# KrishnaswamyLab/MELD

Hardware: AMD Instinct MI355X
Metric: cells/sec through MELD.fit_transform (kNN+Chebyshev) (higher is better)
Workload: dtype f64

## Files before the change

### include/meld_hip.h

```cpp
#ifndef MELD_HIP_H
#define MELD_HIP_H

#include <stddef.h>
#include <stdint.h>

#ifdef __cplusplus
extern "C" {
#endif

#define MELD_OK 0
#define MELD_ERR_INVALID (-1)
#define MELD_ERR_UNSUPPORTED (-2)
#define MELD_ERR_HIP (-3)

typedef void* meld_stream_t;

int meld_abi_version(void);
const char* meld_last_error(void);
int meld_device_count(void);


int meld_knn_padded_dim(int d);
int meld_knn_tile_refs(void);
int meld_knn_block_queries(void);
int meld_knn_row_capacity(int ksel);
double meld_knn_error_coef(int d);

int meld_col_sums_f64(const double* X, int64_t N, int d, double* sums, meld_stream_t stream);
size_t meld_col_stats_temp_bytes(int d);
int meld_col_stats_f64(const double* X, int64_t N, int d, double* sums, double* mins, double* maxs, void* temp, size_t temp_bytes,
                       meld_stream_t stream);

int meld_knn_prepare_refs(const double* X, int64_t N, int d, const double* mean, int KP, float* Rt,
                          float* norm2, float* norm2_max, meld_stream_t stream);
int meld_knn_prepare_queries(const double* X, int64_t N, int d, const double* mean, int KP,
                             int64_t q_begin, int64_t q_count, float* Q, meld_stream_t stream);

int meld_knn_topk(const float* Q, const float* Rt, int64_t n_ref, int KP, int64_t q_count, int ksel,
                  int32_t* cand_idx, float* cand_d2, int32_t* cand_cnt, meld_stream_t stream);

int meld_knn16_kblocks(int d);
int meld_knn16_tile_refs(void);
int meld_knn16_split_dims(int d);
int meld_frame_max_dims(void);
int meld_cov_sample_f64(const double* X, int64_t N, int d, const double* mean, int64_t stride, double* cov, meld_stream_t stream);
int meld_rotate_rows_f64(const double* X, int64_t N, int d, const double* mean, const double* At, double* out, meld_stream_t stream);
int meld_knn16_block_queries(void);
int meld_knn16_row_capacity(int ksel);
double meld_knn16_error_coef(int nprod, int d);
double meld_knn16_error_coef_const(int nprod, int d);
double meld_knn16_error_coef_lin(int nprod);
size_t meld_knn16_tile_bytes(int d);
size_t meld_knn16_query_bytes(int d);
int meld_knn16_prepare(const double* X, int64_t N, int d, const double* mean, int64_t q_begin,
                       int64_t q_count, void* Rt16, void* Q16, float* Qn, float* norm2, float* norm2_max,
                       float* scale_info, meld_stream_t stream);
int meld_knn16_prepare_scaled(const double* X, int64_t N, int d, const double* mean, const double* col_min, const double* col_max,
                              int64_t q_begin, int64_t q_count, void* Rt16, void* Q16, float* Qn, float* norm2, float* norm2_max,
                              float* scale_info, meld_stream_t stream);
size_t meld_knn16_bounds_bytes(int64_t n_ref, int64_t q_count);
size_t meld_knn16_bounds_temp_bytes(int64_t n_ref, int d, int64_t q_count);
int meld_knn16_bounds(const double* X, int64_t N, int d, const double* mean, const float* scale_info,
                      const float* norm2_max, const void* Rt16, int64_t q_begin, int64_t q_count,
                      const float* thr_seed, const float* q_norm2 ,
                      int nprod, void* temp, void* lb2, meld_stream_t stream);
int meld_knn16_tile_spheres(const double* X, int64_t N, int d, const double* mean, const float* scale_info, void* temp,
                            int64_t tile_begin, int64_t tile_count, meld_stream_t stream);
int meld_knn16_sphere_layout(int64_t n_ref, int d, int64_t* rows, int64_t* row_bytes);
int meld_knn16_bounds_from_spheres(const double* X, int64_t N, int d, const double* mean, const float* scale_info,
                      const float* norm2_max, const void* Rt16, int64_t q_begin, int64_t q_count,
                      const float* thr_seed, const float* q_norm2 ,
                      int nprod, void* temp, void* lb2, meld_stream_t stream);
int meld_knn16_prepare_cross(const double* X, int64_t n_refs, int64_t n_total, int d, const double* mean, int64_t q_begin,
                             int64_t q_count, void* Rt16, void* Q16, float* Qn, float* norm2, float* norm2_max,
                             float* scale_info, meld_stream_t stream);
int meld_knn16_prepare_rows(const double* X, int64_t N, int d, const double* mean, const float* scale_info,
                            int64_t q_begin, const int32_t* rows, int64_t n_rows, void* Q16, float* Qn,
                            meld_stream_t stream);
int meld_knn16_research_thresholds(const int32_t* rows, int64_t n_rows, int64_t q_begin, const int32_t* cand_cnt,
                                   const float* cand_d2, int cap, int ksel, const float* norm2, const float* norm2_max,
                                   double err_coef, double err_lin, double err3, const float* scale_info, float* thr,
                                   meld_stream_t stream);
int meld_knn16_seed_thresholds_mfma(const void* Q16, const float* Qn, const void* Rt16, const float* scale_info,
                                    const float* norm2_max, int64_t n_ref, int d, int64_t q_begin, int64_t q_count,
                                    int knn, double radius_factor, int nprod, int side_tiles, float* thr_init,
                                    meld_stream_t stream);
int meld_knn16_topk(const void* Q16, const float* Qn, const void* Rt16, const float* scale_info,
                    int64_t n_ref, int d, int64_t q_count, int ksel, int nprod, int n_slices, const void* lb2,
                    const float* norm2_max, int64_t q_begin, const float* thr_init, int knn, double radius_factor,
                    int32_t* cand_idx, float* cand_d2, int32_t* cand_cnt, float* cand_thr,
                    uint64_t* tiles_done ,
                    const int32_t* block_order ,
                    meld_stream_t stream);
int meld_knn16_block_work(const void* lb2, const float* thr_seed, int64_t n_ref, int d, int64_t q_count, int nprod,
                          const float* norm2_max, const float* scale_info, int32_t* work, meld_stream_t stream);
int meld_knn16_step_lists(const void* lb2, const float* thr_seed, int64_t n_ref, int d, int64_t q_count, int nprod,
                          const float* norm2_max, const float* scale_info, int64_t q_begin, uint32_t* list,
                          int64_t list_stride, int32_t* cnt, meld_stream_t stream);
size_t meld_knn16_list_scratch_bytes(int64_t n_ref);
int meld_knn16_step_lists_direct(const double* X, int64_t N, int d, const double* mean, const float* scale_info, const float* norm2_max,
                                 const void* Rt16, const float* thr_seed, const float* q_norm2, int nprod, void* temp, void* scratch,
                                 uint32_t* list, int64_t list_stride, int32_t* cnt, meld_stream_t stream);
int meld_knn16_step_lists_direct_lead(const double* X, int64_t N, int d, const double* mean, const float* scale_info, const float* norm2_max,
                                 const void* Rt16, const float* thr_seed, const float* q_norm2, int nprod, void* temp, void* scratch,
                                 uint32_t* list, int64_t list_stride, int32_t* cnt, int lead_only, meld_stream_t stream);
int meld_knn16_topk_listed(const void* Q16, const float* Qn, const void* Rt16, const float* scale_info, int64_t n_ref, int d,
                           int64_t q_count, int ksel, const uint32_t* step_list, const int32_t* step_cnt, int64_t list_stride,
                           const float* norm2_max, int64_t q_begin, const float* thr_init, int knn, double radius_factor,
                           int32_t* cand_idx, float* cand_d2, int32_t* cand_cnt, float* cand_thr, uint64_t* tiles_done,
                           const int32_t* block_order, int n_slices , meld_stream_t stream);
int meld_knn16_topk_listed_partial(const void* Q16, const float* Qn, const void* Rt16, const float* scale_info, int64_t n_ref,
                                   int d, int64_t q_count, int ksel, const uint32_t* step_list, const int32_t* step_cnt,
                                   int64_t list_stride, const float* norm2_max, int64_t q_begin, const float* thr_init, int knn,
                                   double radius_factor, int32_t* cand_idx, float* cand_d2, int32_t* cand_cnt, float* cand_thr,
                                   uint64_t* tiles_done, const int32_t* block_order, int n_slices, int partial_test,
                                   meld_stream_t stream);
int meld_knn16_partial_filter(const void* Q16, const float* Qn, const void* Rt16, const float* scale_info, const float* norm2_max, int d,
                              int64_t q_count, const float* thr_init, uint32_t* step_list, const int32_t* step_cnt, int64_t list_stride,
                              int32_t* cnt_out, uint64_t* tested, const int32_t* block_order , meld_stream_t stream);
int meld_knn16_resident_blocks(int d, int nprod);
int meld_knn16_max_slices(int ksel);
int meld_knn16_merge_slices(const int32_t* s_idx, const float* s_d2, const int32_t* s_cnt, int64_t q_count,
                            int ksel, int n_slices, int32_t* out_idx, float* out_d2, int32_t* out_cnt,
                            meld_stream_t stream);


int meld_knn_refine(const double* X, int64_t N, int d, int64_t q_begin, int64_t q_count,
                    const int32_t* cand_idx, const float* cand_d2, const int32_t* cand_cnt,
                    const float* cand_thr ,
                    int ksel, int cap , int knn, double decay, double thresh,
                    const float* norm2_max, double err_coef,
                    const float* norm2 , double err_coef_lin, double* bw,
                    double* cand_val, int32_t* keep_cnt, int32_t* flag_rows, int32_t* n_flag,
                    const int32_t* rows, int out_cap, int32_t* cand_idx_out,
                    double bw_scale ,
                    const double* bw_fixed ,
                    int max_rank ,
                    meld_stream_t stream);

int meld_knn_radius_exact(const double* X, int64_t N, int d, int64_t q_begin, const int32_t* flag_rows,
                          int32_t n_flag, const double* bw, int knn, double decay, double thresh,
                          int mode, int32_t* fb_cnt, const int64_t* fb_off, int32_t* fb_cursor,
                          int32_t* fb_col, double* fb_val, int32_t* err_flag,
                          double bw_scale ,
                          meld_stream_t stream);
int meld_knn_pair_distances(const double* X, int d, const int64_t* rows, const int64_t* cand, int64_t n, int kk, double* out,
                            meld_stream_t stream);

#define MELD_METRIC_L1 1
#define MELD_METRIC_LINF 2
int meld_metric_tile_rows(void);
int meld_metric_tile_boxes(const double* X, int64_t N, int d, double* box_lo, double* box_hi, meld_stream_t stream);
int meld_metric_topk(const double* X, int64_t N, int d, int metric, int ksel, const double* box_lo, const double* box_hi, int prune,
                     double* heap_d, int32_t* heap_i, int32_t* cand_idx, double* cand_d, int32_t* cand_cnt,
                     unsigned long long* tiles_done, meld_stream_t stream);
int meld_metric_refine(const int32_t* cand_idx, const double* cand_d, const int32_t* cand_cnt, int64_t N, int ksel, int knn,
                       double decay, double thresh, double* bw, double* cand_val, int32_t* keep_cnt, int32_t* flag_rows,
                       int32_t* n_flag, meld_stream_t stream);
int meld_metric_radius(const double* X, int64_t N, int d, int metric, const int32_t* flag_rows, int32_t n_flag, const double* bw,
                       double decay, double thresh, int mode, int32_t* fb_cnt, const int64_t* fb_off, int32_t* fb_cursor,
                       int32_t* fb_col, double* fb_val, meld_stream_t stream);


size_t meld_scan_temp_bytes(int64_t n);
int meld_exclusive_scan_i32_i64(const int32_t* in, int64_t* out, int64_t n, void* temp, size_t temp_bytes,
                                meld_stream_t stream);

int meld_coo_emit(int64_t q_begin, int64_t q_count, const int32_t* cand_idx, const double* cand_val,
                  const int32_t* cand_cnt, int ksel, int cap, const int64_t* keep_off, const int32_t* flag_rows,
                  int32_t n_flag, const int64_t* fb_off, const int32_t* fb_col, const double* fb_val,
                  int64_t fb_base, int64_t M, uint64_t* keys, double* vals, meld_stream_t stream);

size_t meld_sort_temp_bytes(int64_t n);
int meld_sort_pairs_u64_f64(const uint64_t* keys_in, uint64_t* keys_out, const double* vals_in,
                            double* vals_out, int64_t n, int end_bit, void* temp, size_t temp_bytes,
                            meld_stream_t stream);

size_t meld_merge_temp_bytes(int64_t n);
int meld_coo_merge(const uint64_t* keys_sorted, const double* vals_sorted, int64_t n, uint64_t* ukeys,
                   double* uvals, int64_t* n_unique, void* temp, size_t temp_bytes, meld_stream_t stream);

int meld_csr_from_keys(const uint64_t* ukeys, int64_t nnz, int64_t row_begin, int64_t n_rows,
                       int64_t* rowptr, int32_t* col, meld_stream_t stream);

int meld_coo_partition_remote(const uint64_t* keys, const double* vals, int64_t n, int64_t rows_per_rank, int world,
                              int self_rank, int64_t cap, int32_t* counts, int64_t* send, meld_stream_t stream);
int meld_coo_emit_scatter(int64_t q_count, const int32_t* cand_idx, const double* cand_val, int ksel, int cap,
                          const int32_t* keep_cnt, const int32_t* flag_rows, int32_t n_flag, const int64_t* fb_off,
                          const int32_t* fb_col, const double* fb_val, int64_t fb_total, int32_t* cursor, int32_t* tcol,
                          double* tval, meld_stream_t stream);
int meld_csr_bucket_slots(void);
int meld_coo_scatter_rows(const uint64_t* keys, const double* vals, int64_t n, int64_t row_begin, int64_t n_rows,
                          int32_t* cursor, int32_t* tcol, double* tval, meld_stream_t stream);
int meld_csr_rows_sort_merge(const int32_t* cursor, int64_t n_rows, int32_t* tcol, double* tval, int32_t* ucnt,
                             int32_t* flags,
                             int symm ,
                             double theta , meld_stream_t stream);
int meld_csr_compact_rows(const int64_t* rowptr, int64_t n_rows, const int32_t* tcol, const double* tval,
                          int32_t* col, double* val, meld_stream_t stream);
int meld_csr_compact_rows_sums(const int64_t* rowptr, int64_t n_rows, const int32_t* tcol, const double* tval, int32_t* col,
                               double* val, double diag, double* sums, meld_stream_t stream);

int meld_csr_row_sums(const int64_t* rowptr, const double* val, int64_t n_rows, double diag,
                      double* out, meld_stream_t stream);
int meld_csr_anisotropy(const int64_t* rowptr, const int32_t* col, double* val, int64_t n_rows,
                        const double* ksum_all, int64_t ksum_row_offset, double anisotropy,
                        meld_stream_t stream);
int meld_csr_anisotropy_degrees(const int64_t* rowptr, const int32_t* col, double* val, int64_t n_rows,
                                const double* ksum_all, int64_t ksum_row_offset, double anisotropy, double* dw,
                                meld_stream_t stream);


int meld_spmm_dot_slots(void);
int meld_cheby_step(const int64_t* rowptr, const int32_t* col, const double* val, const double* dw,
                    int64_t n_rows, int64_t nnz_hint, int p, const double* x_full, int64_t x_row_offset,
                    const double* z, double* y, double* r, double alpha, double beta, double gamma,
                    double coef, double* dots, meld_stream_t stream);

int meld_cheby_step_wide(const int64_t* rowptr, const int32_t* col, const double* val, const double* dw, int64_t n_rows, int p,
                         const double* x_full, int64_t x_row_offset, const double* z, double* y, double alpha, double beta,
                         double gamma, meld_stream_t stream);

int meld_lanczos_steps(const int64_t* rowptr, const int32_t* col, const double* val, const double* dw,
                       int64_t n_rows, int64_t nnz_hint, double* v0, double* v1, double* v2, double* state,
                       double* alphas, double* betas, int it_begin, int n_iter, double* scratch,
                       meld_stream_t stream);
int meld_lanczos_spmv(const int64_t* rowptr, const int32_t* col, const double* val, const double* dw, int64_t n_rows,
                      int64_t nnz_hint, const double* x_full, int64_t x_row_offset, const double* z_local,
                      double* y_local, const double* state, double* dots, meld_stream_t stream);
int meld_lanczos_alpha(double* state, const double* dots, double* nrm2, double* alphas, int it, meld_stream_t stream);
int meld_lanczos_axpy(const double* x_local, double* y_local, int64_t n_rows, const double* state, double* nrm2,
                      meld_stream_t stream);
int meld_lanczos_beta(double* state, const double* nrm2, double* dots, double* betas, int it, meld_stream_t stream);
int meld_lanczos_fold(double* state, double* acc, double* alphas, double* betas, int it, meld_stream_t stream);
int meld_lanczos_axpy3(double* y_local, const double* u_local, const double* u_prev_local, int64_t n_rows,
                       const double* state, double* nrm2, meld_stream_t stream);
int meld_scale_f64(const double* x, double a, double* r, int64_t n, meld_stream_t stream);
int meld_axpby_f64(double a, const double* x, double b, double* y, int64_t n, double* nrm2,
                   meld_stream_t stream);

typedef struct meld_pt_layout {
  const int32_t* blk_row;
  const int32_t* blk_ntile;
  const int32_t* blk_ndist;
  const int32_t* seg;
  const int32_t* list_cols;
  const double* pval;
  const uint32_t* pidx;
  int32_t nb;
  const float* pval32;
  int64_t stream_len;
  const uint16_t* cdesc;
} meld_pt_layout_t;
int meld_pt_geometry(int* consumer_waves, int* rows_max, int* tile_cols, int* tiles_max);
int meld_pt_num_blocks(int64_t n_rows);
int64_t meld_pt_seg_len(int nb);
int64_t meld_pt_stream_len(int64_t nnz, int nb);
int64_t meld_pt_desc_len(int nb);
int meld_pt_debug_ablate(int mask);
int meld_pt_debug_stamps(unsigned long long* buf);
int meld_pt_build(const int64_t* rowptr, const int32_t* col, const double* val, int64_t n_rows, int64_t n_cols,
                  int64_t col_base, int symmetric, const meld_pt_layout_t* layout,
                  uint32_t* codes , int32_t* status, meld_stream_t stream);
int meld_pt_cheby_step(const meld_pt_layout_t* layout, const int64_t* rowptr, const double* dw, int64_t n_rows, int p,
                       const double* x_full, int64_t x_row_offset, const double* z, double* y, double* r,
                       double alpha, double beta, double gamma, double coef, double* dots, meld_stream_t stream);
int meld_pt_cheby_run(const meld_pt_layout_t* layout, const int64_t* rowptr, const double* dw, int64_t n_rows, int p,
                      double* t_prev2, double* t_prev1, double* r, const double* coeffs, int n_coef, double alpha2, double beta2,
                      int* last, meld_stream_t stream);
int meld_pt_lanczos_steps(const meld_pt_layout_t* layout, const int64_t* rowptr, const double* dw, int64_t n_rows,
                          double* v0, double* v1, double* v2, double* state, double* alphas, double* betas,
                          int it_begin, int n_iter, double* scratch, const int32_t* stop, meld_stream_t stream);
int meld_pt_lanczos_spmv(const meld_pt_layout_t* layout, const int64_t* rowptr, const double* dw, int64_t n_rows,
                         const double* x_full, int64_t x_row_offset, const double* z_local, double* y_local,
                         const double* state, double* dots, meld_stream_t stream);

int meld_rccl_available(void);
int meld_rccl_unique_id(void* id_host);
int meld_rccl_comm_create(const void* id_host, int world, int rank, void** comm);
int meld_rccl_comm_destroy(void* comm);
// ... 56 lines not shown
```

### meld_amd/_lib.py

```python
from __future__ import annotations

from ._options import is_set, opt

import ctypes as C
import os

_HERE = os.path.dirname(os.path.abspath(__file__))
LIB_NAME = "libmeld_hip.so"
LIB_PATH = os.path.join(_HERE, LIB_NAME)

_i32, _i64, _f64, _sz, _ptr = C.c_int, C.c_int64, C.c_double, C.c_size_t, C.c_void_p

SIGNATURES = {
    "meld_abi_version": (_i32, []),
    "meld_last_error": (C.c_char_p, []),
    "meld_device_count": (_i32, []),
    "meld_knn_padded_dim": (_i32, [_i32]),
    "meld_knn_tile_refs": (_i32, []),
    "meld_knn_block_queries": (_i32, []),
    "meld_knn_row_capacity": (_i32, [_i32]),
    "meld_col_sums_f64": (_i32, [_ptr, _i64, _i32, _ptr, _ptr]),
    "meld_col_stats_temp_bytes": (_sz, [_i32]),
    "meld_col_stats_f64": (_i32, [_ptr, _i64, _i32, _ptr, _ptr, _ptr, _ptr, _sz, _ptr]),
    "meld_knn_prepare_refs": (_i32, [_ptr, _i64, _i32, _ptr, _i32, _ptr, _ptr, _ptr, _ptr]),
    "meld_knn_prepare_queries": (_i32, [_ptr, _i64, _i32, _ptr, _i32, _i64, _i64, _ptr, _ptr]),
    "meld_knn_topk": (_i32, [_ptr, _ptr, _i64, _i32, _i64, _i32, _ptr, _ptr, _ptr, _ptr]),
    "meld_knn_refine": (
        _i32,
        [_ptr, _i64, _i32, _i64, _i64, _ptr, _ptr, _ptr, _ptr, _i32, _i32, _i32, _f64, _f64, _ptr, _f64, _ptr, _f64, _ptr, _ptr, _ptr,
         _ptr, _ptr, _ptr, _i32, _ptr, _f64, _ptr, _i32, _ptr],
    ),
    "meld_knn_error_coef": (_f64, [_i32]),
    "meld_knn16_kblocks": (_i32, [_i32]),
    "meld_knn16_tile_refs": (_i32, []),
    "meld_knn16_split_dims": (_i32, [_i32]),
    "meld_knn16_block_queries": (_i32, []),
    "meld_knn16_row_capacity": (_i32, [_i32]),
    "meld_knn16_error_coef": (_f64, [_i32, _i32]),
    "meld_knn16_error_coef_const": (_f64, [_i32, _i32]),
    "meld_knn16_error_coef_lin": (_f64, [_i32]),
    "meld_knn16_resident_blocks": (_i32, [_i32, _i32]),
    "meld_knn16_tile_bytes": (_sz, [_i32]),
    "meld_knn16_query_bytes": (_sz, [_i32]),
    "meld_knn16_prepare": (_i32, [_ptr, _i64, _i32, _ptr, _i64, _i64, _ptr, _ptr, _ptr, _ptr, _ptr, _ptr, _ptr]),
    "meld_knn16_prepare_scaled": (_i32, [_ptr, _i64, _i32, _ptr, _ptr, _ptr, _i64, _i64, _ptr, _ptr, _ptr, _ptr, _ptr, _ptr, _ptr]),
    "meld_knn16_prepare_cross": (_i32, [_ptr, _i64, _i64, _i32, _ptr, _i64, _i64, _ptr, _ptr, _ptr, _ptr, _ptr, _ptr, _ptr]),
    "meld_knn16_prepare_rows": (_i32, [_ptr, _i64, _i32, _ptr, _ptr, _i64, _ptr, _i64, _ptr, _ptr, _ptr]),
    "meld_knn16_research_thresholds": (_i32, [_ptr, _i64, _i64, _ptr, _ptr, _i32, _i32, _ptr, _ptr, _f64, _f64, _f64, _ptr, _ptr, _ptr]),
    "meld_knn16_bounds_bytes": (_sz, [_i64, _i64]),
    "meld_knn16_bounds_temp_bytes": (_sz, [_i64, _i32, _i64]),
    "meld_knn16_bounds": (_i32, [_ptr, _i64, _i32, _ptr, _ptr, _ptr, _ptr, _i64, _i64, _ptr, _ptr, _i32, _ptr, _ptr, _ptr]),
    "meld_knn16_bounds_from_spheres": (_i32, [_ptr, _i64, _i32, _ptr, _ptr, _ptr, _ptr, _i64, _i64, _ptr, _ptr, _i32, _ptr, _ptr, _ptr]),
    "meld_knn16_tile_spheres": (_i32, [_ptr, _i64, _i32, _ptr, _ptr, _ptr, _i64, _i64, _ptr]),
    "meld_knn16_sphere_layout": (_i32, [_i64, _i32, _ptr, _ptr]),
    "meld_knn16_topk": (_i32, [_ptr, _ptr, _ptr, _ptr, _i64, _i32, _i64, _i32, _i32, _i32, _ptr, _ptr, _i64, _ptr, _i32, _f64, _ptr, _ptr, _ptr, _ptr, _ptr, _ptr, _ptr]),
    "meld_knn16_block_work": (_i32, [_ptr, _ptr, _i64, _i32, _i64, _i32, _ptr, _ptr, _ptr, _ptr]),
    "meld_knn16_step_lists": (_i32, [_ptr, _ptr, _i64, _i32, _i64, _i32, _ptr, _ptr, _i64, _ptr, _i64, _ptr, _ptr]),
    "meld_knn16_list_scratch_bytes": (_sz, [_i64]),
    "meld_knn16_step_lists_direct": (_i32, [_ptr, _i64, _i32, _ptr, _ptr, _ptr, _ptr, _ptr, _ptr, _i32, _ptr, _ptr, _ptr, _i64, _ptr, _ptr]),
    "meld_knn16_step_lists_direct_lead": (_i32, [_ptr, _i64, _i32, _ptr, _ptr, _ptr, _ptr, _ptr, _ptr, _i32, _ptr, _ptr, _ptr, _i64, _ptr, _i32, _ptr]),
    "meld_knn16_topk_listed": (_i32, [_ptr, _ptr, _ptr, _ptr, _i64, _i32, _i64, _i32, _ptr, _ptr, _i64, _ptr, _i64, _ptr, _i32, _f64, _ptr, _ptr, _ptr, _ptr, _ptr, _ptr, _i32, _ptr]),
    "meld_knn16_topk_listed_partial": (_i32, [_ptr, _ptr, _ptr, _ptr, _i64, _i32, _i64, _i32, _ptr, _ptr, _i64, _ptr, _i64, _ptr, _i32, _f64, _ptr, _ptr, _ptr, _ptr, _ptr, _ptr, _i32, _i32, _ptr]),
    "meld_knn16_partial_filter": (_i32, [_ptr, _ptr, _ptr, _ptr, _ptr, _i32, _i64, _ptr, _ptr, _ptr, _i64, _ptr, _ptr, _ptr, _ptr]),
    "meld_knn16_seed_thresholds_mfma": (_i32, [_ptr, _ptr, _ptr, _ptr, _ptr, _i64, _i32, _i64, _i64, _i32, _f64, _i32, _i32, _ptr, _ptr]),
    "meld_knn16_max_slices": (_i32, [_i32]),
    "meld_knn16_merge_slices": (_i32, [_ptr, _ptr, _ptr, _i64, _i32, _i32, _ptr, _ptr, _ptr, _ptr]),
    "meld_knn_radius_exact": (
        _i32,
        [_ptr, _i64, _i32, _i64, _ptr, _i32, _ptr, _i32, _f64, _f64, _i32, _ptr, _ptr, _ptr, _ptr, _ptr, _ptr, _f64, _ptr],
    ),
    "meld_knn_pair_distances": (_i32, [_ptr, _i32, _ptr, _ptr, _i64, _i32, _ptr, _ptr]),
    "meld_metric_tile_rows": (_i32, []),
    "meld_metric_tile_boxes": (_i32, [_ptr, _i64, _i32, _ptr, _ptr, _ptr]),
    "meld_metric_topk": (_i32, [_ptr, _i64, _i32, _i32, _i32, _ptr, _ptr, _i32, _ptr, _ptr, _ptr, _ptr, _ptr, _ptr, _ptr]),
    "meld_metric_refine": (_i32, [_ptr, _ptr, _ptr, _i64, _i32, _i32, _f64, _f64, _ptr, _ptr, _ptr, _ptr, _ptr, _ptr]),
    "meld_metric_radius": (_i32, [_ptr, _i64, _i32, _i32, _ptr, _i32, _ptr, _f64, _f64, _i32, _ptr, _ptr, _ptr, _ptr, _ptr, _ptr]),
    "meld_scan_temp_bytes": (_sz, [_i64]),
    "meld_exclusive_scan_i32_i64": (_i32, [_ptr, _ptr, _i64, _ptr, _sz, _ptr]),
    "meld_coo_emit": (
        _i32,
        [_i64, _i64, _ptr, _ptr, _ptr, _i32, _i32, _ptr, _ptr, _i32, _ptr, _ptr, _ptr, _i64, _i64, _ptr, _ptr, _ptr],
    ),
    "meld_sort_temp_bytes": (_sz, [_i64]),
    "meld_sort_pairs_u64_f64": (_i32, [_ptr, _ptr, _ptr, _ptr, _i64, _i32, _ptr, _sz, _ptr]),
    "meld_merge_temp_bytes": (_sz, [_i64]),
    "meld_coo_merge": (_i32, [_ptr, _ptr, _i64, _ptr, _ptr, _ptr, _ptr, _sz, _ptr]),
    "meld_csr_from_keys": (_i32, [_ptr, _i64, _i64, _i64, _ptr, _ptr, _ptr]),
    "meld_csr_seg_length": (_i32, []),
    "meld_csr_spmm_f64": (_i32, [_ptr, _ptr, _ptr, _i32, _i64, _ptr, _ptr, _i64, _ptr, _ptr, _i64, _ptr, _ptr, _i64, _i32, _ptr, _i64, _ptr]),
    "meld_csr_transpose_keys": (_i32, [_ptr, _ptr, _ptr, _i32, _i64, _ptr, _ptr, _ptr]),
    "meld_csr_rows_to_dense_f64": (_i32, [_ptr, _ptr, _ptr, _i32, _i64, _i64, _i64, _ptr, _i64, _ptr]),
    "meld_csr_bucket_slots": (_i32, []),
    "meld_coo_scatter_rows": (_i32, [_ptr, _ptr, _i64, _i64, _i64, _ptr, _ptr, _ptr, _ptr]),
    "meld_coo_emit_scatter": (_i32, [_i64, _ptr, _ptr, _i32, _i32, _ptr, _ptr, _i32, _ptr, _ptr, _ptr, _i64, _ptr, _ptr, _ptr, _ptr]),
    "meld_coo_partition_remote": (_i32, [_ptr, _ptr, _i64, _i64, _i32, _i32, _i64, _ptr, _ptr, _ptr]),
    "meld_csr_rows_sort_merge": (_i32, [_ptr, _i64, _ptr, _ptr, _ptr, _ptr, _i32, _f64, _ptr]),
    "meld_csr_compact_rows": (_i32, [_ptr, _i64, _ptr, _ptr, _ptr, _ptr, _ptr]),
    "meld_csr_compact_rows_sums": (_i32, [_ptr, _i64, _ptr, _ptr, _ptr, _ptr, _f64, _ptr, _ptr]),
    "meld_csr_row_sums": (_i32, [_ptr, _ptr, _i64, _f64, _ptr, _ptr]),
    "meld_csr_anisotropy": (_i32, [_ptr, _ptr, _ptr, _i64, _ptr, _i64, _f64, _ptr]),
    "meld_csr_anisotropy_degrees": (_i32, [_ptr, _ptr, _ptr, _i64, _ptr, _i64, _f64, _ptr, _ptr]),
    "meld_spmm_dot_slots": (_i32, []),
    "meld_cheby_step": (
        _i32,
        [_ptr, _ptr, _ptr, _ptr, _i64, _i64, _i32, _ptr, _i64, _ptr, _ptr, _ptr, _f64, _f64, _f64, _f64, _ptr, _ptr],
    ),
    "meld_lanczos_steps": (_i32, [_ptr, _ptr, _ptr, _ptr, _i64, _i64, _ptr, _ptr, _ptr, _ptr, _ptr, _ptr, _i32, _i32, _ptr, _ptr]),
    "meld_lanczos_spmv": (_i32, [_ptr, _ptr, _ptr, _ptr, _i64, _i64, _ptr, _i64, _ptr, _ptr, _ptr, _ptr, _ptr]),
    "meld_lanczos_alpha": (_i32, [_ptr, _ptr, _ptr, _ptr, _i32, _ptr]),
    "meld_lanczos_axpy": (_i32, [_ptr, _ptr, _i64, _ptr, _ptr, _ptr]),
    "meld_lanczos_beta": (_i32, [_ptr, _ptr, _ptr, _ptr, _i32, _ptr]),
    "meld_lanczos_fold": (_i32, [_ptr, _ptr, _ptr, _ptr, _i32, _ptr]),
    "meld_lanczos_axpy3": (_i32, [_ptr, _ptr, _ptr, _i64, _ptr, _ptr, _ptr]),
    "meld_pt_geometry": (_i32, [_ptr, _ptr, _ptr, _ptr]),
    "meld_pt_num_blocks": (_i32, [_i64]),
    "meld_pt_seg_len": (_i64, [_i32]),
    "meld_pt_debug_ablate": (_i32, [_i32]),
    "meld_pt_debug_stamps": (_i32, [_ptr]),
    "meld_pt_stream_len": (_i64, [_i64, _i32]),
    "meld_pt_desc_len": (_i64, [_i32]),
    "meld_pt_build": (_i32, [_ptr, _ptr, _ptr, _i64, _i64, _i64, _i32, _ptr, _ptr, _ptr, _ptr]),
    "meld_cheby_step_wide": (_i32, [_ptr, _ptr, _ptr, _ptr, _i64, _i32, _ptr, _i64, _ptr, _ptr, _f64, _f64, _f64, _ptr]),
    "meld_pt_cheby_step": (_i32, [_ptr, _ptr, _ptr, _i64, _i32, _ptr, _i64, _ptr, _ptr, _ptr, _f64, _f64, _f64, _f64, _ptr, _ptr]),
    "meld_pt_cheby_run": (_i32, [_ptr, _ptr, _ptr, _i64, _i32, _ptr, _ptr, _ptr, _ptr, _i32, _f64, _f64, _ptr, _ptr]),
    "meld_pt_lanczos_steps": (_i32, [_ptr, _ptr, _ptr, _i64, _ptr, _ptr, _ptr, _ptr, _ptr, _ptr, _i32, _i32, _ptr, _ptr, _ptr]),
    "meld_pt_lanczos_spmv": (_i32, [_ptr, _ptr, _ptr, _i64, _ptr, _i64, _ptr, _ptr, _ptr, _ptr, _ptr]),
    "meld_kmeans_max_blocks": (_i32, []),
    "meld_kmeans_assign": (_i32, [_ptr, _i64, _i32, _ptr, _i32, _ptr, _ptr, _ptr, _ptr, _i32, _ptr]),
    "meld_scale_f64": (_i32, [_ptr, _f64, _ptr, _i64, _ptr]),
    "meld_axpby_f64": (_i32, [_f64, _ptr, _f64, _ptr, _i64, _ptr, _ptr]),
    "meld_normalize_rows_l1": (_i32, [_ptr, _ptr, _i64, _i32, _ptr]),
    "meld_assign_nearest": (_i32, [_ptr, _i64, _i32, _ptr, _i32, _ptr, _ptr, _ptr, _ptr]),
    "meld_chain_order": (_i32, [_ptr, _i64, _i32, _i32, _ptr, _ptr]),
    "meld_gather_rows_f64": (_i32, [_ptr, _ptr, _i64, _i32, _ptr, _ptr]),
    "meld_frame_max_dims": (_i32, []),
    "meld_cov_sample_f64": (_i32, [_ptr, _i64, _i32, _ptr, _i64, _ptr, _ptr]),
    "meld_rotate_rows_f64": (_i32, [_ptr, _i64, _i32, _ptr, _ptr, _ptr, _ptr]),
    "meld_argsort_u32_temp_bytes": (_sz, [_i64]),
    "meld_argsort_u32": (_i32, [_ptr, _i64, _i32, _ptr, _ptr, _ptr, _sz, _ptr]),
    "meld_order_starts": (_i32, [_ptr, _i64, _i32, _ptr, _ptr]),
    "meld_order_pick_centroids": (_i32, [_ptr, _i64, _i32, _ptr, _ptr, _i32, _i32, _ptr, _ptr]),
    "meld_order_update_keys": (_i32, [_ptr, _ptr, _ptr, _i64, _i32, _ptr]),
    "meld_rccl_available": (_i32, []),
    "meld_rccl_unique_id": (_i32, [_ptr]),
    "meld_rccl_comm_create": (_i32, [_ptr, _i32, _i32, _ptr]),
    "meld_rccl_comm_destroy": (_i32, [_ptr]),
    "meld_rccl_all_gather": (_i32, [_ptr, _ptr, _ptr, _sz, _ptr]),
    "meld_rccl_all_reduce_sum_f64": (_i32, [_ptr, _ptr, _sz, _ptr]),
    "meld_cheby_run_sharded": (_i32, [_ptr, _ptr, _ptr, _ptr, _ptr, _ptr, _i64, _i64, _i64, _i64, _i32, _ptr, _ptr, _ptr, _ptr, _i32, _f64, _f64, _ptr, _ptr]),
    "meld_lanczos_steps_sharded": (_i32, [_ptr, _ptr, _ptr, _ptr, _ptr, _ptr, _i64, _i64, _i64, _i64, _ptr, _ptr, _ptr, _ptr, _ptr, _ptr, _ptr, _i32, _i32, _ptr]),
    "meld_factorize_max_groups": (_i32, []),
    "meld_factorize_max_words": (_i32, []),
    "meld_factorize_temp_bytes": (_sz, [_i64]),
    "meld_factorize_labels": (_i32, [_ptr, _i64, _i32, _ptr, _sz, _ptr, _ptr]),
    "meld_factorize_codes": (_i32, [_ptr, _i64, _ptr, _ptr, _ptr]),
    "meld_indicator_signal": (_i32, [_ptr, _ptr, _ptr, _i64, _i64, _i32, _ptr, _ptr]),
    "meld_scatter_rows_f64": (_i32, [_ptr, _ptr, _i64, _i32, _ptr, _ptr]),
}



class PtLayout(C.Structure):

    _fields_ = [("blk_row", _ptr), ("blk_ntile", _ptr), ("blk_ndist", _ptr), ("seg", _ptr), ("list_cols", _ptr),
                ("pval", _ptr), ("pidx", _ptr), ("nb", C.c_int32), ("pval32", _ptr), ("stream_len", C.c_int64), ("cdesc", _ptr)]


_lib = None


class MeldHipError(RuntimeError):
    """A libmeld_hip.so entry point returned a non-zero status."""


def get_lib():
    global _lib
    if _lib is not None:
        return _lib
    path = opt("MELD_HIP_LIB") or LIB_PATH
    if not os.path.exists(path):
# ... 23 lines not shown
```

### meld_amd/csrc/assemble.hip

```cpp
#include "common.hpp"

#include <rocprim/rocprim.hpp>

namespace meld {

__global__ __launch_bounds__(256) void coo_emit_rows_kernel(int64_t q_begin, int64_t q_count,
                                                            const int* __restrict__ cand_idx,
                                                            const double* __restrict__ cand_val, int ksel, int cap,
                                                            const int64_t* __restrict__ keep_off, int64_t M,
                                                            unsigned long long* __restrict__ keys,
                                                            double* __restrict__ vals) {
  const int lane = threadIdx.x & 63;
  const int64_t q = (int64_t)blockIdx.x * 4 + (threadIdx.x >> 6);
  if (q >= q_count) return;
  const int64_t base = keep_off[q];
  if (keep_off[q + 1] == base) return;
  const unsigned long long gi = (unsigned long long)(q_begin + q);
  int written = 0;
  for (int c0 = 0; c0 < ksel; c0 += 64) {
    const int c = c0 + lane;
    double v = 0.0;
    int j = 0;
    if (c < ksel) {
      v = cand_val[(size_t)q * ksel + c];
// ... 328 lines not shown
    int j = 0;
    if (c < ksel) {
      v = cand_val[(size_t)q * ksel + c];
      j = cand_idx[(size_t)q * cap + c];
    }
    const bool keep = v > 0.0;
    const unsigned long long b = __ballot(keep);
    if (keep) {
      const int pos = written + __popcll(b & ((1ull << lane) - 1ull));
      const double hv = 0.5 * v;
      tcol[q * CSR_BUCKET + pos] = j;
      tval[q * CSR_BUCKET + pos] = hv;
      const int slot = atomicAdd(cursor + j, 1);
      if (slot < CSR_BUCKET) {
        tcol[(int64_t)j * CSR_BUCKET + slot] = (int)q;
        tval[(int64_t)j * CSR_BUCKET + slot] = hv;
      }
    }
    written += __popcll(b);
  }
}
__global__ __launch_bounds__(256) void coo_emit_scatter_fallback_kernel(const int* __restrict__ flag_rows, int n_flag,
                                                                        const int64_t* __restrict__ fb_off,
                                                                        const int* __restrict__ fb_col,
                                                                        const double* __restrict__ fb_val, int64_t fb_total,
                                                                        int* __restrict__ cursor, int* __restrict__ tcol,
                                                                        double* __restrict__ tval) {
  const int64_t e = (int64_t)blockIdx.x * blockDim.x + threadIdx.x;
  if (e >= fb_total) return;
  int lo = 0, hi = n_flag - 1;
  while (lo < hi) {
    const int mid = (lo + hi + 1) >> 1;
    if (fb_off[mid] <= e) lo = mid; else hi = mid - 1;
  }
  const int64_t q = flag_rows[lo];
  const int64_t pos = e - fb_off[lo];
  const int j = fb_col[e];
  const double hv = 0.5 * fb_val[e];
  if (pos < CSR_BUCKET) {
    tcol[q * CSR_BUCKET + pos] = j;
    tval[q * CSR_BUCKET + pos] = hv;
  }
  const int slot = atomicAdd(cursor + j, 1);
  if (slot < CSR_BUCKET) {
    tcol[(int64_t)j * CSR_BUCKET + slot] = (int)q;
    tval[(int64_t)j * CSR_BUCKET + slot] = hv;
  }
}

template <int SL, typename K>
__device__ __forceinline__ void csr_bitonic_sort(K (&key)[SL], int lane) {
  constexpr int NE = 64 * SL;
#pragma unroll
  for (int k = 2; k <= NE; k <<= 1) {
#pragma unroll
    for (int j = k >> 1; j > 0; j >>= 1) {
      if (j >= 64) {
        const int je = j >> 6;
#pragma unroll
        for (int e = 0; e < SL; ++e) {
          if ((e & je) == 0) {
            const bool asc = ((64 * e + lane) & k) == 0;
            const K a = key[e], b = key[e | je];
            const bool sw = asc ? (b < a) : (a < b);
            key[e] = sw ? b : a;
            key[e | je] = sw ? a : b;
          }
        }
      } else {
#pragma unroll
        for (int e = 0; e < SL; ++e) {
          const int i = 64 * e + lane;
          const K o = __shfl_xor(key[e], j, 64);
          const bool keep_min = ((i & j) == 0) == ((i & k) == 0);
          key[e] = keep_min ? (o < key[e] ? o : key[e]) : (o < key[e] ? key[e] : o);
        }
      }
    }
  }
}

template <int SL>
__device__ __forceinline__ int csr_row_merge(int* __restrict__ tcol, double* __restrict__ tval, int64_t base, int n, int lane,
                                             bool* bad, int symm, double theta) {
  static_assert(CSR_BUCKET <= 256, "the slot shares a 32-bit key with a 24-bit column");
  unsigned cin[SL];
  bool wide = false;
#pragma unroll
  for (int e = 0; e < SL; ++e) {
    const int i = lane + 64 * e;
    cin[e] = i < n ? (unsigned)tcol[base + i] : 0u;
    wide |= cin[e] >= 0xFFFFFFu;
  }
  double v[SL];
  unsigned c[SL];
  if (!__any(wide)) {
    unsigned key[SL];
#pragma unroll
    for (int e = 0; e < SL; ++e) {
      const int i = lane + 64 * e;
      key[e] = i < n ? ((cin[e] << 8) | (unsigned)i) : ~0u;
    }
    csr_bitonic_sort<SL>(key, lane);
#pragma unroll
    for (int e = 0; e < SL; ++e) {
      const int i = lane + 64 * e;
      c[e] = i < n ? (key[e] >> 8) : 0xffffffffu;
      v[e] = i < n ? tval[base + (key[e] & 255u)] : 0.0;
    }
  } else {
    unsigned long long key[SL];
#pragma unroll
    for (int e = 0; e < SL; ++e) {
      const int i = lane + 64 * e;
      key[e] = i < n ? (((unsigned long long)cin[e] << 32) | (unsigned)i) : ~0ull;
    }
    csr_bitonic_sort<SL>(key, lane);
#pragma unroll
    for (int e = 0; e < SL; ++e) {
      const int i = lane + 64 * e;
      c[e] = (unsigned)(key[e] >> 32);
      v[e] = i < n ? tval[base + (unsigned)key[e]] : 0.0;
    }
  }
  int total = 0;
  bool any_bad = false;
  unsigned head_col[SL];
  double head_val[SL];
  int head_pos[SL];
  bool is_head[SL];
#pragma unroll
  for (int e = 0; e < SL; ++e) {
    const int i = lane + 64 * e;
    unsigned prev = __shfl_up(c[e], 1, 64);
    if (lane == 0) prev = 0xffffffffu;
    if (e > 0) {
      const unsigned pl = __shfl(c[e - 1], 63, 64);
      if (lane == 0) prev = pl;
    }
    unsigned n1 = __shfl_down(c[e], 1, 64), n2 = __shfl_down(c[e], 2, 64);
    double v1 = __shfl_down(v[e], 1, 64);
    if (e + 1 < SL) {
      const unsigned f0 = __shfl(c[e + 1], 0, 64), f1 = __shfl(c[e + 1], 1, 64);
      const double w0 = __shfl(v[e + 1], 0, 64);
      if (lane == 63) { n1 = f0; n2 = f1; v1 = w0; }
      if (lane == 62) n2 = f0;
    } else {
      if (lane == 63) { n1 = 0xffffffffu; n2 = 0xffffffffu; }
      if (lane == 62) n2 = 0xffffffffu;
    }
    const bool valid = i < n;
    const bool head = valid && (i == 0 || prev != c[e]);
    const bool pair = valid && (i + 1 < n) && n1 == c[e];
    const bool triple = valid && (i + 2 < n) && n2 == c[e];
    any_bad |= triple;
    double hv = pair ? v[e] + v1 : v[e];
    bool keep_head = head;
    if (symm == 1) {
      hv = pair ? 4.0 * v[e] * v1 : 0.0;
      keep_head = head && pair;
    } else if (symm == 2) {
      hv = pair ? 2.0 * (theta * fmin(v[e], v1) + (1.0 - theta) * fmax(v[e], v1)) : 2.0 * (1.0 - theta) * v[e];
      keep_head = head && hv != 0.0;
    }
    is_head[e] = keep_head;
    head_col[e] = c[e];
    head_val[e] = hv;
    const unsigned long long hb = __ballot(keep_head);
    head_pos[e] = total + __popcll(hb & ((1ull << lane) - 1ull));
    total += __popcll(hb);
  }
#pragma unroll
  for (int e = 0; e < SL; ++e) {
    if (is_head[e]) {
      tcol[base + head_pos[e]] = (int)head_col[e];
      tval[base + head_pos[e]] = head_val[e];
    }
  }
  if (__any(any_bad)) *bad = true;
  return total;
}

__global__ __launch_bounds__(256) void csr_rows_sort_merge_kernel(const int* __restrict__ cursor, int64_t n_rows,
                                                                  int* __restrict__ tcol, double* __restrict__ tval,
                                                                  int* __restrict__ ucnt, int* __restrict__ flags, int symm, double theta) {
  const int lane = threadIdx.x & 63;
  const int64_t r = (int64_t)blockIdx.x * 4 + (threadIdx.x >> 6);
  if (r >= n_rows) return;
  const int64_t base = r * CSR_BUCKET;
  const int n = cursor[r];
  if (n > CSR_BUCKET) {
    if (lane == 0) {
      atomicOr(flags, 1);
      ucnt[r] = 0;
    }
    return;
  }
  bool bad = false;
  int total;
  if (n <= 64)
    total = csr_row_merge<1>(tcol, tval, base, n, lane, &bad, symm, theta);
  else if (n <= 128)
    total = csr_row_merge<2>(tcol, tval, base, n, lane, &bad, symm, theta);
  else
    total = csr_row_merge<4>(tcol, tval, base, n, lane, &bad, symm, theta);
  if (lane == 0) {
    ucnt[r] = total;
    if (bad) atomicOr(flags, 2);
  }
}

__global__ __launch_bounds__(256) void csr_compact_rows_kernel(const int64_t* __restrict__ rowptr, int64_t n_rows,
                                                               const int* __restrict__ tcol, const double* __restrict__ tval,
                                                               int* __restrict__ col, double* __restrict__ val) {
  const int64_t r = ((int64_t)blockIdx.x * blockDim.x + threadIdx.x) >> 4;
  const int g = threadIdx.x & 15;
  if (r >= n_rows) return;
  const int64_t src = r * CSR_BUCKET, dst = rowptr[r];
  const int len = (int)(rowptr[r + 1] - dst);
  for (int k = g; k < len; k += 16) {
    col[dst + k] = tcol[src + k];
    val[dst + k] = tval[src + k];
  }
}

__global__ __launch_bounds__(256) void csr_compact_rows_sums_kernel(const int64_t* __restrict__ rowptr, int64_t n_rows,
                                                                    const int* __restrict__ tcol, const double* __restrict__ tval,
                                                                    int* __restrict__ col, double* __restrict__ val, double diag,
                                                                    double* __restrict__ sums) {
  const int64_t r = ((int64_t)blockIdx.x * blockDim.x + threadIdx.x) >> 3;
  const int g = threadIdx.x & 7;
  double s = 0.0;
  if (r < n_rows) {
    const int64_t src = r * CSR_BUCKET, dst = rowptr[r];
    const int len = (int)(rowptr[r + 1] - dst);
    for (int k = g; k < len; k += 8) {
      const double v = tval[src + k];
      col[dst + k] = tcol[src + k];
      val[dst + k] = v;
      s += v;
    }
  }
  s += __shfl_xor(s, 1, 64);
  s += __shfl_xor(s, 2, 64);
  s += __shfl_xor(s, 4, 64);
  if (r < n_rows && g == 0) sums[r] = diag + s;
}

extern "C" int meld_csr_bucket_slots(void) { return CSR_BUCKET; }

extern "C" int meld_coo_scatter_rows(const uint64_t* keys, const double* vals, int64_t n, int64_t row_begin, int64_t n_rows,
                                     int32_t* cursor, int32_t* tcol, double* tval, meld_stream_t stream) {
  MELD_CHECK_ARG(cursor && n_rows > 0 && n >= 0 && (n == 0 || (keys && vals && tcol && tval)),
                 "meld_coo_scatter_rows: bad arguments");
  MELD_HIP_CALL(hipMemsetAsync(cursor, 0, sizeof(int32_t) * (size_t)n_rows, S(stream)));
  if (n == 0) return MELD_OK;
  hipLaunchKernelGGL(coo_scatter_rows_kernel, dim3((unsigned)ceil_div(n, 256)), dim3(256), 0, S(stream),
                     reinterpret_cast<const unsigned long long*>(keys), vals, n, row_begin, n_rows, cursor, tcol, tval);
  MELD_LAUNCH_CHECK("coo_scatter_rows_kernel");
  return MELD_OK;
}

extern "C" int meld_coo_partition_remote(const uint64_t* keys, const double* vals, int64_t n, int64_t rows_per_rank, int world,
                                         int self_rank, int64_t cap, int32_t* counts, int64_t* send, meld_stream_t stream) {
  MELD_CHECK_ARG(counts && send && n >= 0 && (n == 0 || (keys && vals)) && rows_per_rank > 0 && world >= 1 && self_rank >= 0 &&
                     self_rank < world && cap >= 0,
                 "meld_coo_partition_remote: bad arguments");
  MELD_HIP_CALL(hipMemsetAsync(counts, 0, sizeof(int32_t) * (size_t)world, S(stream)));
  if (cap > 0) MELD_HIP_CALL(hipMemsetAsync(send, 0xFF, sizeof(int64_t) * 2 * (size_t)world * (size_t)cap, S(stream)));
  if (n == 0) return MELD_OK;
  MELD_CHECK_ARG(world <= PR_WORLD_MAX, "meld_coo_partition_remote: %d ranks (at most %d)", world, PR_WORLD_MAX);
  hipLaunchKernelGGL(coo_partition_remote_kernel, dim3((unsigned)ceil_div(n, 256 * PR_PER)), dim3(256), 0, S(stream),
                     reinterpret_cast<const unsigned long long*>(keys), vals, n, rows_per_rank, world, self_rank, cap, counts,
                     reinterpret_cast<long long*>(send));
  MELD_LAUNCH_CHECK("coo_partition_remote_kernel");
  return MELD_OK;
}

extern "C" int meld_coo_emit_scatter(int64_t q_count, const int32_t* cand_idx, const double* cand_val, int ksel, int cap,
                                     const int32_t* keep_cnt, const int32_t* flag_rows, int32_t n_flag, const int64_t* fb_off,
                                     const int32_t* fb_col, const double* fb_val, int64_t fb_total, int32_t* cursor, int32_t* tcol,
                                     double* tval, meld_stream_t stream) {
  MELD_CHECK_ARG(cand_idx && cand_val && keep_cnt && cursor && tcol && tval && q_count > 0, "meld_coo_emit_scatter: bad arguments");
  MELD_CHECK_ARG(cap >= ksel && ksel <= CSR_BUCKET, "meld_coo_emit_scatter: ksel=%d must fit a row bucket (%d) and the row stride cap=%d",
                 ksel, CSR_BUCKET, cap);
  hipLaunchKernelGGL(coo_emit_scatter_rows_kernel, dim3((unsigned)ceil_div(q_count, 4)), dim3(256), 0, S(stream), q_count, cand_idx,
                     cand_val, ksel, cap, keep_cnt, cursor, tcol, tval);
  MELD_LAUNCH_CHECK("coo_emit_scatter_rows_kernel");
  if (n_flag > 0 && fb_total > 0) {
    MELD_CHECK_ARG(flag_rows && fb_off && fb_col && fb_val, "meld_coo_emit_scatter: missing fallback arrays");
    hipLaunchKernelGGL(coo_emit_scatter_fallback_kernel, dim3((unsigned)ceil_div(fb_total, 256)), dim3(256), 0, S(stream), flag_rows,
                       n_flag, fb_off, fb_col, fb_val, fb_total, cursor, tcol, tval);
    MELD_LAUNCH_CHECK("coo_emit_scatter_fallback_kernel");
  }
  return MELD_OK;
}

extern "C" int meld_csr_rows_sort_merge(const int32_t* cursor, int64_t n_rows, int32_t* tcol, double* tval, int32_t* ucnt,
                                        int32_t* flags, int symm, double theta, meld_stream_t stream) {
  MELD_CHECK_ARG(cursor && tcol && tval && ucnt && flags && n_rows > 0, "meld_csr_rows_sort_merge: bad arguments");
  MELD_CHECK_ARG(symm >= 0 && symm <= 2 && (symm != 2 || (theta >= 0.0 && theta <= 1.0)),
                 "meld_csr_rows_sort_merge: symm must be 0 (+), 1 (*) or 2 (mnn, theta in [0, 1])");
  MELD_HIP_CALL(hipMemsetAsync(flags, 0, sizeof(int32_t), S(stream)));
  hipLaunchKernelGGL(csr_rows_sort_merge_kernel, dim3((unsigned)ceil_div(n_rows, 4)), dim3(256), 0, S(stream), cursor, n_rows,
                     tcol, tval, ucnt, flags, symm, theta);
  MELD_LAUNCH_CHECK("csr_rows_sort_merge_kernel");
  return MELD_OK;
}

extern "C" int meld_csr_compact_rows(const int64_t* rowptr, int64_t n_rows, const int32_t* tcol, const double* tval,
                                     int32_t* col, double* val, meld_stream_t stream) {
  MELD_CHECK_ARG(rowptr && n_rows > 0 && tcol && tval && col && val, "meld_csr_compact_rows: bad arguments");
  hipLaunchKernelGGL(csr_compact_rows_kernel, dim3((unsigned)ceil_div(n_rows * 16, 256)), dim3(256), 0, S(stream), rowptr,
                     n_rows, tcol, tval, col, val);
  MELD_LAUNCH_CHECK("csr_compact_rows_kernel");
  return MELD_OK;
}

extern "C" int meld_csr_compact_rows_sums(const int64_t* rowptr, int64_t n_rows, const int32_t* tcol, const double* tval, int32_t* col,
                                          double* val, double diag, double* sums, meld_stream_t stream) {
  MELD_CHECK_ARG(rowptr && n_rows > 0 && tcol && tval && col && val && sums, "meld_csr_compact_rows_sums: bad arguments");
  hipLaunchKernelGGL(csr_compact_rows_sums_kernel, dim3((unsigned)ceil_div(n_rows * 8, 256)), dim3(256), 0, S(stream), rowptr, n_rows, tcol,
                     tval, col, val, diag, sums);
  MELD_LAUNCH_CHECK("csr_compact_rows_sums_kernel");
  return MELD_OK;
}

extern "C" int meld_csr_row_sums(const int64_t* rowptr, const double* val, int64_t n_rows, double diag, double* out,
                                 meld_stream_t stream) {
  MELD_CHECK_ARG(rowptr && out && n_rows > 0, "meld_csr_row_sums: bad arguments");
  hipLaunchKernelGGL(csr_row_sums_kernel, dim3((unsigned)ceil_div(n_rows * 8, 256)), dim3(256), 0, S(stream), rowptr,
                     val, n_rows, diag, out);
  MELD_LAUNCH_CHECK("csr_row_sums_kernel");
  return MELD_OK;
}

extern "C" int meld_csr_anisotropy(const int64_t* rowptr, const int32_t* col, double* val, int64_t n_rows,
                                   const double* ksum_all, int64_t ksum_row_offset, double anisotropy,
                                   meld_stream_t stream) {
  MELD_CHECK_ARG(rowptr && ksum_all && n_rows > 0, "meld_csr_anisotropy: bad arguments");
  if (anisotropy == 0.0) return MELD_OK;
  hipLaunchKernelGGL(csr_anisotropy_kernel, dim3((unsigned)ceil_div(n_rows * 8, 256)), dim3(256), 0, S(stream),
                     rowptr, col, val, n_rows, ksum_all, ksum_row_offset, anisotropy, (double*)nullptr);
  MELD_LAUNCH_CHECK("csr_anisotropy_kernel");
  return MELD_OK;
}

extern "C" int meld_csr_anisotropy_degrees(const int64_t* rowptr, const int32_t* col, double* val, int64_t n_rows,
                                           const double* ksum_all, int64_t ksum_row_offset, double anisotropy, double* dw,
                                           meld_stream_t stream) {
  MELD_CHECK_ARG(rowptr && ksum_all && dw && n_rows > 0, "meld_csr_anisotropy_degrees: bad arguments");
  if (anisotropy == 0.0) return meld_csr_row_sums(rowptr, val, n_rows, 0.0, dw, stream);
  hipLaunchKernelGGL(csr_anisotropy_kernel, dim3((unsigned)ceil_div(n_rows * 8, 256)), dim3(256), 0, S(stream),
                     rowptr, col, val, n_rows, ksum_all, ksum_row_offset, anisotropy, dw);
  MELD_LAUNCH_CHECK("csr_anisotropy_kernel");
  return MELD_OK;
}
```

### meld_amd/csrc/knn16.hip

```cpp
#include "common.hpp"

#include <hip/hip_fp16.h>

#include <algorithm>

namespace meld {

constexpr int K16_TS = 64;
constexpr int K16_BQ = 256;
constexpr int K16_THREADS = 256;
constexpr int K16_NWAVE = K16_THREADS / 64;
constexpr int K16_SLACK = 128;
constexpr int K16_CAPMAX = 256;
constexpr int K16_BOUNDS_THREADS = 1024;
constexpr int K16_SLOTS = K16_CAPMAX / 64;
constexpr int K16_DMAX = 16 * 9 - 3;

constexpr int K16_SPLIT_DA = 13;
__host__ __device__ inline void k16_slot(int c, int d, int dA, int* coord, int* piece) {
  *coord = -1;
  *piece = -1;
  if (dA == 0) {
    if (c < d) *coord = c;
    else if (c < d + 3) *piece = 3 + (c - d);
// ... 984 lines not shown
}
template <int SL>
__device__ __forceinline__ void k16_finish_row(float* __restrict__ drow, int* __restrict__ irow, int n0, int half, int n_all, int n,
                                               float add, float out_scale, int lane) {
  unsigned long long key[SL];
#pragma unroll
  for (int e = 0; e < SL; ++e) {
    const int i = lane + 64 * e;
    const int p = i < n0 ? i : half + (i - n0);
    key[e] = ~0ull;
    if (i < n_all) key[e] = ((unsigned long long)ordered_bits(drow[p] + 0.0f) << 32) | (unsigned)irow[p];
  }
  k16_bitonic_sort<SL>(key, lane);
#pragma unroll
  for (int e = 0; e < SL; ++e) {
    const int i = 64 * e + lane;
    if (i < n) {
      drow[i] = (from_ordered_bits((unsigned)(key[e] >> 32)) + add) * out_scale;
      irow[i] = (int)(unsigned)key[e];
    }
  }
}
__global__ __launch_bounds__(256) void knn16_finish_rows_kernel(float* __restrict__ d2, int* __restrict__ idx,
                                                                int* __restrict__ cnt, const float* __restrict__ Qn,
                                                                const float* __restrict__ scale_info, int64_t n_rows,
                                                                int64_t q_pad, int cap, int ksel) {
  const int lane = threadIdx.x & 63;
  const int64_t row = (int64_t)blockIdx.x * 4 + (threadIdx.x >> 6);
  if (row >= n_rows) return;
  const int packed = cnt[row];
  const int n0 = packed & 0xffff, n1 = (packed >> 16) & 0xffff, half = cap >> 1;
  float* drow = d2 + (size_t)row * cap;
  int* irow = idx + (size_t)row * cap;
  const int n_all = n0 + n1, n = min(n_all, ksel);
  const float add = Qn[row % q_pad], out_scale = scale_info[1];
  if (n_all <= 64)
    k16_finish_row<1>(drow, irow, n0, half, n_all, n, add, out_scale, lane);
  else if (n_all <= 128)
    k16_finish_row<2>(drow, irow, n0, half, n_all, n, add, out_scale, lane);
  else
    k16_finish_row<K16_SLOTS>(drow, irow, n0, half, n_all, n, add, out_scale, lane);
  if (lane == 0) cnt[row] = n;
}

constexpr int K16_MERGE_MAX = 4096;
constexpr int K16_MERGE_SLOTS = K16_MERGE_MAX / 64;

__global__ __launch_bounds__(64) void knn16_merge_slices_kernel(const int* __restrict__ s_idx,
                                                                const float* __restrict__ s_d2,
                                                                const int* __restrict__ s_cnt, int q_count, int q_pad,
                                                                int ksel, int cap, int n_slices,
                                                                int* __restrict__ out_idx, float* __restrict__ out_d2,
                                                                int* __restrict__ out_cnt) {
  extern __shared__ __attribute__((aligned(16))) unsigned char merge_lds[];
  float* sd = reinterpret_cast<float*>(merge_lds);
  int* si = reinterpret_cast<int*>(merge_lds) + n_slices * ksel;
  const int lane = threadIdx.x;
  const int q = blockIdx.x;
  if (q >= q_count) return;
  int n = 0;
  for (int s = 0; s < n_slices; ++s) {
    const int row = s * q_pad + q;
    const int c = min(s_cnt[row], ksel);
    for (int e = lane; e < c; e += 64) {
      sd[n + e] = s_d2[(size_t)row * cap + e];
      si[n + e] = s_idx[(size_t)row * cap + e];
    }
    n += c;
  }
  __syncthreads();
  for (int p = lane; p < n; p += 64) {
    const float dp = sd[p];
    const int ip = si[p];
    int rk = 0;
    for (int e = 0; e < n; ++e) rk += (sd[e] < dp || (sd[e] == dp && si[e] < ip)) ? 1 : 0;
    if (rk < ksel) {
      out_d2[(size_t)q * cap + rk] = dp;
      out_idx[(size_t)q * cap + rk] = ip;
    }
  }
  if (lane == 0) out_cnt[q] = min(n, ksel);
}

__global__ __launch_bounds__(256) void tile_spheres_kernel(const double* __restrict__ X, int64_t N, int d,
                                                           const double* __restrict__ mean,
                                                           const float* __restrict__ scale_info, int KB,
                                                           _Float16* __restrict__ cent16, float* __restrict__ cent_n,
                                                           float* __restrict__ cent_r, int tile0, int dA) {
  extern __shared__ float xs_dyn[];
  const int ld = d | 1;
#define XS(r, k) xs_dyn[(r) * ld + (k)]
  __shared__ float cs[K16_DMAX + 19];
  const int tid = threadIdx.x;
  const int tile = tile0 + (int)blockIdx.x;
  const int64_t row0 = (int64_t)tile * K16_TS;
  const int cnt = (int)min((int64_t)K16_TS, N - row0);
  const float s = scale_info[0];
  for (int u = tid; u < K16_TS * d; u += 256) {
    const int r = u / d, k = u - r * d;
    const int64_t i = row0 + r;
    XS(r, k) = i < N ? s * (float)(X[i * d + k] - mean[k]) : 0.0f;
  }
  __syncthreads();
  if (tid < KB * 16) {
    float acc = 0.0f;
    if (tid < d)
      for (int r = 0; r < cnt; ++r) acc += XS(r, tid);
    cs[tid] = tid < d ? acc / (float)cnt : 0.0f;
  }
  __syncthreads();
  __shared__ float cb[K16_DMAX + 19];
  __shared__ float s_best_r2;
  if (tid < 64) {
    const int lane = tid;
    auto far2 = [&](int* who) {
      float r2 = -1.0f;
      if (lane < cnt) {
        r2 = 0.0f;
        int k = 0;
        for (; k + 8 <= d; k += 8) {
          float t[8];
#pragma unroll
          for (int u = 0; u < 8; ++u) t[u] = XS(lane, k + u) - cs[k + u];
#pragma unroll
          for (int u = 0; u < 8; ++u) r2 = fmaf(t[u], t[u], r2);
        }
        for (; k < d; ++k) {
          const float t = XS(lane, k) - cs[k];
          r2 = fmaf(t, t, r2);
        }
      }
      auto dppf = [](float old, float v, auto ctrl, auto rows) __attribute__((always_inline)) {
        return __int_as_float(__builtin_amdgcn_update_dpp(__float_as_int(old), __float_as_int(v), decltype(ctrl)::value, decltype(rows)::value, 0xF, false));
      };
      using std::integral_constant;
      float m = r2;
      m = fmaxf(m, dppf(m, m, integral_constant<int, 0xB1>{}, integral_constant<int, 0xF>{}));
      m = fmaxf(m, dppf(m, m, integral_constant<int, 0x4E>{}, integral_constant<int, 0xF>{}));
      m = fmaxf(m, dppf(m, m, integral_constant<int, 0x141>{}, integral_constant<int, 0xF>{}));
      m = fmaxf(m, dppf(m, m, integral_constant<int, 0x140>{}, integral_constant<int, 0xF>{}));
      m = fmaxf(m, dppf(m, m, integral_constant<int, 0x142>{}, integral_constant<int, 0xA>{}));
      m = fmaxf(m, dppf(m, m, integral_constant<int, 0x143>{}, integral_constant<int, 0xC>{}));
      m = __int_as_float(__builtin_amdgcn_readlane(__float_as_int(m), 63));
      *who = __ffsll((long long)__ballot(r2 == m)) - 1;
      return m;
    };
    float best = INFINITY;
    constexpr int MEB_STEPS = 24;
    for (int it = 1; it <= MEB_STEPS + 1; ++it) {
      int who;
      const float r2 = far2(&who);
      if (r2 < best) {
        best = r2;
        for (int k = lane; k < KB * 16; k += 64) cb[k] = cs[k];
      }
      if (it <= MEB_STEPS) {
        const float wgt = 1.0f / (float)(it + 1);
        for (int k = lane; k < d; k += 64) cs[k] = fmaf(wgt, XS(who, k) - cs[k], cs[k]);
      }
      __builtin_amdgcn_s_waitcnt(0xC07F);
      asm volatile("" ::: "memory");
    }
    for (int k = lane; k < KB * 16; k += 64) cs[k] = cb[k];
    if (lane == 0) s_best_r2 = best;
  }
  __syncthreads();
  if (tid < 64) {
    const float r2 = s_best_r2;
    float n = 0.0f;
    for (int k = 0; k < d; ++k) n = fmaf(cs[k], cs[k], n);
    if (tid == 0) {
      cent_r[tile] = sqrtf(r2) * 1.0001f + 1e-30f;
      cent_n[tile] = n;
    }
  } else if (tid - 64 < KB * 2) {
    const int g = tid - 64;
    f16x8 hi, lo;
#pragma unroll
    for (int e = 0; e < 8; ++e) {
      int cc, pc;
      k16_slot(g * 8 + e, d, dA, &cc, &pc);
      _Float16 h16 = (_Float16)0.0f, l16 = (_Float16)0.0f;
      if (cc >= 0) {
        h16 = (_Float16)cs[cc];
        l16 = (_Float16)(cs[cc] - (float)h16);
      } else if (pc >= 0) {
        h16 = (_Float16)1.0f;
      }
      hi[e] = h16;
      lo[e] = l16;
    }
    f16x8* qrow = reinterpret_cast<f16x8*>(cent16) + (size_t)tile * ((size_t)KB * 4);
    qrow[g * 2 + 0] = hi;
    qrow[g * 2 + 1] = lo;
  }
#undef XS
}

template <int KB, bool SEEDED, int BT, bool BITS = false, int KU = KB>
__global__ __launch_bounds__(BT) void knn16_tile_bounds_kernel(const _Float16* __restrict__ C16, const float* __restrict__ Cn,
                                                                const float* __restrict__ Cr,
                                                                const _Float16* __restrict__ Rt16, int n_tiles,
                                                                int first_tile, int n_blocks, float err_coef,
                                                                const float* __restrict__ norm2_max,
                                                                const float* __restrict__ scale_info,
                                                                const float* __restrict__ thr_seed, int64_t n_seed,
                                                                float seed_err_coef, int mark_sign,
                                                                const float* __restrict__ q_norm2, float err_c, float err_l,
                                                                __half* __restrict__ lb2, const float* __restrict__ wthr = nullptr,
                                                                unsigned long long* __restrict__ bits_a = nullptr,
                                                                unsigned long long* __restrict__ bits_b = nullptr, int wpr = 0, int dA = 0) {
  constexpr int TPB = 1;
  constexpr int HV = KU * 2 * K16_TS;
  constexpr int NS = (HV + BT - 1) / BT;
  __shared__ __attribute__((aligned(16))) float4 lds_a[2][HV];
  __shared__ __attribute__((aligned(16))) f16x8 lds_x[2][2 * K16_TS];
  const int tid = threadIdx.x, lane = tid & 63, wave = tid >> 6, jq = lane & 31, h = lane >> 5;
  const int c_base = blockIdx.x * BT + wave * 64;
  f16x8 bhi[2][KU];
  float cn[2], cr[2];
#pragma unroll
  for (int g = 0; g < 2; ++g) {
    const f16x8* qrow = reinterpret_cast<const f16x8*>(C16 + (size_t)(c_base + g * 32 + jq) * (KB * 32));
#pragma unroll
    for (int kb = 0; kb < KU; ++kb) bhi[g][kb] = qrow[(kb * 2 + h) * 2 + 0];
    cn[g] = Cn[c_base + g * 32 + jq];
    cr[g] = Cr[c_base + g * 32 + jq];
    if (KU < KB) {
      const f16x8 lo = qrow[(0 * 2 + h) * 2 + 1];
      float n = 0.0f;
#pragma unroll
      for (int e = 0; e < 8; ++e) {
        const float v = (8 * h + e < dA) ? (float)bhi[g][0][e] + (float)lo[e] : 0.0f;
        n = fmaf(v, v, n);
      }
      cn[g] = n + __shfl_xor(n, 32, 64);
    }
  }
  float wcol[2] = {-INFINITY, -INFINITY};
  if (BITS) {
#pragma unroll
    for (int g = 0; g < 2; ++g)
      if (c_base + g * 32 + jq < n_tiles) wcol[g] = wthr[c_base + g * 32 + jq];
  }
  const int c_l = c_base + lane;
  const float cn_l = h == 0 ? cn[0] : cn[1], cr_l = h == 0 ? cr[0] : cr[1], wcol_l = h == 0 ? wcol[0] : wcol[1];
  f16x8 bx[2];
#pragma unroll
  for (int g = 0; g < 2; ++g) {
#pragma unroll
    for (int e = 0; e < 8; ++e) bx[g][e] = (_Float16)0.0f;
    if (h == 0) {
      bx[g][0] = (_Float16)(-1.0f);
      bx[g][1] = (_Float16)(-__half2float(__float2half_ru(2.0f * cr[g])));
    }
  }
  const float err_abs = (err_coef + (KU < KB ? 1.9073486328125e-06f : 0.0f)) * norm2_max[0] * scale_info[0] * scale_info[0];
  const int b_lo = (int)((long long)n_blocks * blockIdx.y / gridDim.y);
  const int b_hi = (int)((long long)n_blocks * (blockIdx.y + 1) / gridDim.y);
  const int n_steps = (b_hi - b_lo) * TPB;
  const float4* R4 = reinterpret_cast<const float4*>(Rt16);
  float4 p[NS];
  float seed_v = 0.0f;
  const float nmax_s = norm2_max[0] * scale_info[0] * scale_info[0];
  const float seed_margin = seed_err_coef * nmax_s;
  float seed_nq = -1.0f;
  auto load = [&](int step) __attribute__((always_inline)) {
    const int t = first_tile + (b_lo * TPB + step);
#pragma unroll
    for (int u = 0; u < NS; ++u) {
      const int j = tid + BT * u;
      if (j < HV) p[u] = t < n_tiles ? R4[(size_t)t * (KB * 256) + ((j >> 6) << 7) + (j & 63)] : make_float4(0.f, 0.f, 0.f, 0.f);
    }
    if (SEEDED && tid < K16_TS) {
      const int64_t q = (int64_t)(b_lo * TPB + step) * K16_TS + tid;
      seed_v = q < n_seed ? thr_seed[q] : -1.0f;
      seed_nq = (q_norm2 != nullptr && q < n_seed) ? q_norm2[q] : -1.0f;
    }
  };
  auto store = [&](int buf) __attribute__((always_inline)) {
#pragma unroll
// ... 130 lines not shown
    if (IS_REF) {
      if (i < N) v = s * (float)(X[i * d + k] - mean[k]);
    } else {
      const int64_t qq = i < n_rows ? i : n_rows - 1;
      const int64_t src = q_begin + (rows ? (int64_t)rows[qq] : qq);
      v = s * (float)(X[src * d + k] - mean[k]);
    }
    xs[r][k] = v;
  }
  __syncthreads();
  const int r = tid & 63, part = tid >> 6;
  const int64_t i = row0 + r;
  const bool real = !IS_REF || i < N;
  float n = 0.0f;
  for (int k = 0; k < d; ++k) n = fmaf(xs[r][k], xs[r][k], n);
  if (!real) n = INFINITY;
  float nA = 0.0f, nB = n;
  if (IS_REF && dA > 0) {
    nB = 0.0f;
    for (int k = 0; k < dA; ++k) nA = fmaf(xs[r][k], xs[r][k], nA);
    for (int k = dA; k < d; ++k) nB = fmaf(xs[r][k], xs[r][k], nB);
    const float m_r = 1.03f * 0.0009765625f * nB + (float)d * 2.384185791015625e-07f;
    nA -= m_r;
    nB += m_r;
    if (!real) {
      nA = INFINITY;
      nB = 0.0f;
    }
  }
  _Float16 npc[6];
  {
    const float src2[2] = {nA, nB};
#pragma unroll
    for (int q = 0; q < 2; ++q) {
      const float nn = src2[q];
      const _Float16 n1 = (_Float16)nn;
      const float r1 = isinf(nn) ? 0.0f : nn - (float)n1;
      const _Float16 n2 = (_Float16)r1;
      npc[3 * q + 0] = n1;
      npc[3 * q + 1] = n2;
      npc[3 * q + 2] = (_Float16)(r1 - (float)n2);
    }
  }
  for (int g = part; g < KB * 2; g += 4) {
    f16x8 hi, lo;
#pragma unroll
    for (int e = 0; e < 8; ++e) {
      int cc, pc;
      k16_slot(g * 8 + e, d, dA, &cc, &pc);
      _Float16 h16 = (_Float16)0.0f, l16 = (_Float16)0.0f;
      if (cc >= 0) {
        const float v = IS_REF ? -2.0f * xs[r][cc] : xs[r][cc];
        h16 = (_Float16)v;
        l16 = (_Float16)(v - (float)h16);
      } else if (pc >= 0) {
        h16 = IS_REF ? npc[pc] : (_Float16)1.0f;
      }
      hi[e] = h16;
      lo[e] = l16;
    }
    if (IS_REF) {
      f16x8* tile = reinterpret_cast<f16x8*>(out16) + (size_t)blockIdx.x * ((size_t)KB * 2 * 2 * K16_TS);
      tile[(size_t)(g * 2 + 0) * K16_TS + r] = hi;
      tile[(size_t)(g * 2 + 1) * K16_TS + r] = lo;
    } else {
      f16x8* qrow = reinterpret_cast<f16x8*>(out16) + (size_t)i * ((size_t)KB * 4);
      qrow[g * 2 + 0] = hi;
      qrow[g * 2 + 1] = lo;
    }
  }
  if (part == 0) {
    if (IS_REF) {
      float n_orig = 0.0f;
      if (real) {
        n_orig = n * scale_info[1];
        out_norm[i] = n_orig;
      }
#pragma unroll
      for (int off = 32; off > 0; off >>= 1) n_orig = fmaxf(n_orig, __shfl_xor(n_orig, off, 64));
      if (r == 0) atomicMax(reinterpret_cast<int*>(norm2_max), __float_as_int(n_orig));
    } else {
      out_norm[i] = n;
    }
  }
}

constexpr int SEED_KMAX = 64;

constexpr int SEED_WAVES = 8;
template <int KB, int SEED_K>
__global__ __launch_bounds__(64 * SEED_WAVES) void knn16_seed_mfma_kernel(const _Float16* __restrict__ Q16, const float* __restrict__ Qn,
                                                              const _Float16* __restrict__ Rt16,
                                                              const float* __restrict__ scale_info,
                                                              const float* __restrict__ norm2_max, int n_tiles,
                                                              int first_tile, int side, int n_qwaves, int knn1, float rf2, float err_c, float err_l,
                                                              float* __restrict__ thr_init) {
  constexpr int HV = KB * 2 * K16_TS;
  constexpr int ST = 64 * SEED_WAVES;
  constexpr int NS = (HV + ST - 1) / ST;
  __shared__ __attribute__((aligned(16))) float4 lds_a[HV];
  const int tid = threadIdx.x, lane = tid & 63, wave = tid >> 6, jq = lane & 31, h = lane >> 5;
  const int q_base = (blockIdx.x * SEED_WAVES + wave) * 64;
  const bool has_q = blockIdx.x * SEED_WAVES + wave < n_qwaves;
  f16x8 bhi[2][KB];
  float nq[2];
#pragma unroll
  for (int g = 0; g < 2; ++g) {
    const f16x8* qrow = reinterpret_cast<const f16x8*>(Q16 + (size_t)((has_q ? q_base : 0) + g * 32 + jq) * (KB * 32));
#pragma unroll
    for (int kb = 0; kb < KB; ++kb) bhi[g][kb] = qrow[(kb * 2 + h) * 2 + 0];
    nq[g] = Qn[(has_q ? q_base : 0) + g * 32 + jq];
  }
  float best0[SEED_K], best1[SEED_K];
#pragma unroll
  for (int e = 0; e < SEED_K; ++e) best0[e] = best1[e] = INFINITY;
  auto insert = [&](float (&best)[SEED_K], float v) __attribute__((always_inline)) {
    if (v < best[SEED_K - 1]) {
#pragma unroll
      for (int e = SEED_K - 1; e > 0; --e) best[e] = __builtin_amdgcn_fmed3f(best[e - 1], v, best[e]);
      best[0] = fminf(best[0], v);
    }
  };
  const float4* R4 = reinterpret_cast<const float4*>(Rt16);
  const int t_own = first_tile + blockIdx.x * SEED_WAVES;
  const int t_lo = max(t_own - side, 0), t_hi = min(t_own + SEED_WAVES + side, n_tiles);
  float4 stage[NS];
  auto fetch = [&](int t) __attribute__((always_inline)) {
#pragma unroll
    for (int u = 0; u < NS; ++u) {
      const int j = tid + ST * u;
      if (j < HV) stage[u] = R4[(size_t)t * (KB * 256) + ((j >> 6) << 7) + (j & 63)];
    }
  };
  const int own_hi = min(t_own + SEED_WAVES, t_hi);
  int n_below = 0, n_above = 0, t_next;
  auto advance = [&](int t) __attribute__((always_inline)) {
    if (t >= t_own && t + 1 < own_hi) return t + 1;
    const bool more_below = t_own - 1 - n_below >= t_lo, more_above = own_hi + n_above < t_hi;
    if (more_below && (n_below <= n_above || !more_above)) return t_own - 1 - n_below++;
    if (more_above) return own_hi + n_above++;
    return t_hi;
  };
  t_next = t_own < own_hi ? t_own : advance(t_hi);
  if (t_next < t_hi) fetch(t_next);
  for (int t = t_next; t < t_hi; t = t_next) {
    __syncthreads();
#pragma unroll
    for (int u = 0; u < NS; ++u) {
      const int j = tid + ST * u;
      if (j < HV) lds_a[j] = stage[u];
    }
    __syncthreads();
    t_next = advance(t);
    if (t_next < t_hi) fetch(t_next);
    const f16x8* a8 = reinterpret_cast<const f16x8*>(lds_a);
#pragma unroll
    for (int sub = 0; sub < 2; ++sub) {
      f32x16 c0, c1;
#pragma unroll
      for (int r = 0; r < 16; ++r) c0[r] = c1[r] = 0.0f;
#pragma unroll
      for (int kb = 0; kb < KB; ++kb) {
        const f16x8 ahi = a8[(kb * 2 + h) * K16_TS + sub * 32 + jq];
        c0 = __builtin_amdgcn_mfma_f32_32x32x16_f16(ahi, bhi[0][kb], c0, 0, 0, 0);
        c1 = __builtin_amdgcn_mfma_f32_32x32x16_f16(ahi, bhi[1][kb], c1, 0, 0, 0);
      }
// ... 47 lines not shown
static int k16_dA(int d, int KB) { return (d > K16_SPLIT_DA && d + 6 <= 16 * KB) ? K16_SPLIT_DA : 0; }
extern "C" int meld_knn16_kblocks(int d);
extern "C" int meld_knn16_split_dims(int d) {
  const int kb = meld_knn16_kblocks(d);
  return kb < 0 ? 0 : k16_dA(d, kb);
}
extern "C" int meld_knn16_kblocks(int d) {
  if (d < 1) return MELD_ERR_INVALID;
  const int kb = (d + 3 + 15) / 16;
  if (kb > 9) {
    set_err("meld_knn16_kblocks: d=%d exceeds the largest instantiated distance kernel (d <= 141)", d);
    return MELD_ERR_UNSUPPORTED;
  }
  return kb;
}
extern "C" size_t meld_knn16_tile_bytes(int d) {
  const int kb = meld_knn16_kblocks(d);
  return kb < 0 ? 0 : (size_t)kb * 2 * 2 * K16_TS * 16;
}
extern "C" size_t meld_knn16_query_bytes(int d) {
  const int kb = meld_knn16_kblocks(d);
  return kb < 0 ? 0 : (size_t)kb * 64;
}
extern "C" int meld_knn16_tile_refs(void) { return K16_TS; }
extern "C" int meld_knn16_block_queries(void) { return K16_BQ; }
extern "C" int meld_knn16_row_capacity(int ksel) {
  if (ksel < 1 || ksel > K16_CAPMAX - K16_SLACK) {
    set_err("meld_knn16_row_capacity: ksel=%d outside [1, %d]", ksel, K16_CAPMAX - K16_SLACK);
    return MELD_ERR_UNSUPPORTED;
  }
  return ksel + K16_SLACK;
}
static double k16_const_coef(int nprod, int d) {
  const double T = (double)(nprod == 3 ? 3 * d : d) + 6.0;
  double c = 1.01 * T * 1.1920928955078125e-07 * 3.0
             + 4.76837158203125e-07
             + (double)(d + 2) * 5.9604644775390625e-08
             + 5.9604644775390625e-08
             + 2.98023223876953125e-07;
  if (nprod == 3) c += 9.5367431640625e-07 + 3.0 * 2.98023223876953125e-08 * sqrt((double)d) + 4.76837158203125e-07;
  return c;
}
extern "C" double meld_knn16_error_coef(int nprod, int d) {
  return k16_const_coef(nprod, d) + (nprod == 1 ? 0.001953125 : 0.0);
}
extern "C" double meld_knn16_error_coef_const(int nprod, int d) { return k16_const_coef(nprod, d); }
extern "C" double meld_knn16_error_coef_lin(int nprod) { return nprod == 1 ? 0.001953125 : 0.0; }

static int k16_prepare_impl(const double* X, int64_t N, int d, const double* mean, int64_t q_begin,
                                  int64_t q_count, void* Rt16, void* Q16, float* Qn, float* norm2, float* norm2_max,
                                  float* scale_info, meld_stream_t stream, const double* col_min, const double* col_max) {
  MELD_CHECK_ARG(X && mean && Rt16 && Q16 && Qn && norm2 && norm2_max && scale_info && N > 0,
                 "meld_knn16_prepare: null/empty argument");
  MELD_CHECK_ARG(q_count > 0 && q_begin >= 0 && q_begin + q_count <= N, "meld_knn16_prepare: bad query range");
  const int KB = meld_knn16_kblocks(d);
  if (KB < 0) return KB;
  hipStream_t st = S(stream);
  MELD_HIP_CALL(hipMemsetAsync(scale_info, 0, 4 * sizeof(float), st));
  MELD_HIP_CALL(hipMemsetAsync(norm2_max, 0, sizeof(float), st));
  if (col_min != nullptr && col_max != nullptr)
    hipLaunchKernelGGL(absmax_from_extremes_kernel, dim3(1), dim3(256), 0, st, mean, col_min, col_max, d, scale_info);
  else
    hipLaunchKernelGGL(absmax_centered_kernel, dim3(2048), dim3(256), 0, st, X, N * (int64_t)d, d, mean, scale_info);
  hipLaunchKernelGGL(finish_scale_kernel, dim3(1), dim3(1), 0, st, scale_info);
  const int64_t n_pad = ceil_div(N, K16_TS) * K16_TS;
  hipLaunchKernelGGL((prepare16_kernel<true>), dim3((unsigned)(n_pad / K16_TS)), dim3(256), 0, st, X, N, d, mean, scale_info,
                     KB, (int64_t)0, N, (const int*)nullptr, reinterpret_cast<_Float16*>(Rt16), norm2, norm2_max, k16_dA(d, KB));
  const int64_t q_pad = ceil_div(q_count, K16_BQ) * K16_BQ;
  hipLaunchKernelGGL((prepare16_kernel<false>), dim3((unsigned)(q_pad / K16_TS)), dim3(256), 0, st, X, N, d, mean, scale_info,
                     KB, q_begin, q_count, (const int*)nullptr, reinterpret_cast<_Float16*>(Q16), Qn, (float*)nullptr, k16_dA(d, KB));
  MELD_LAUNCH_CHECK("meld_knn16_prepare");
  return MELD_OK;
}
extern "C" int meld_knn16_prepare(const double* X, int64_t N, int d, const double* mean, int64_t q_begin,
                                  int64_t q_count, void* Rt16, void* Q16, float* Qn, float* norm2, float* norm2_max,
                                  float* scale_info, meld_stream_t stream) {
  return k16_prepare_impl(X, N, d, mean, q_begin, q_count, Rt16, Q16, Qn, norm2, norm2_max, scale_info, stream, nullptr, nullptr);
}
extern "C" int meld_knn16_prepare_scaled(const double* X, int64_t N, int d, const double* mean, const double* col_min, const double* col_max,
                                         int64_t q_begin, int64_t q_count, void* Rt16, void* Q16, float* Qn, float* norm2, float* norm2_max,
                                         float* scale_info, meld_stream_t stream) {
  MELD_CHECK_ARG(col_min && col_max, "meld_knn16_prepare_scaled: null column extremes");
  return k16_prepare_impl(X, N, d, mean, q_begin, q_count, Rt16, Q16, Qn, norm2, norm2_max, scale_info, stream, col_min, col_max);
}

extern "C" int meld_knn16_prepare_cross(const double* X, int64_t n_refs, int64_t n_total, int d, const double* mean,
                                        int64_t q_begin, int64_t q_count, void* Rt16, void* Q16, float* Qn, float* norm2,
                                        float* norm2_max, float* scale_info, meld_stream_t stream) {
  MELD_CHECK_ARG(X && mean && Rt16 && Q16 && Qn && norm2 && norm2_max && scale_info && n_refs > 0 && n_total >= n_refs,
                 "meld_knn16_prepare_cross: null/empty argument");
  MELD_CHECK_ARG(q_count > 0 && q_begin >= 0 && q_begin + q_count <= n_total, "meld_knn16_prepare_cross: bad query range");
  const int KB = meld_knn16_kblocks(d);
  if (KB < 0) return KB;
  hipStream_t st = S(stream);
  MELD_HIP_CALL(hipMemsetAsync(scale_info, 0, 4 * sizeof(float), st));
  MELD_HIP_CALL(hipMemsetAsync(norm2_max, 0, sizeof(float), st));
  hipLaunchKernelGGL(absmax_centered_kernel, dim3(2048), dim3(256), 0, st, X, n_total * (int64_t)d, d, mean, scale_info);
  hipLaunchKernelGGL(finish_scale_kernel, dim3(1), dim3(1), 0, st, scale_info);
  const int64_t n_pad = ceil_div(n_refs, K16_TS) * K16_TS;
  hipLaunchKernelGGL((prepare16_kernel<true>), dim3((unsigned)(n_pad / K16_TS)), dim3(256), 0, st, X, n_refs, d, mean, scale_info,
                     KB, (int64_t)0, n_refs, (const int*)nullptr, reinterpret_cast<_Float16*>(Rt16), norm2, norm2_max, k16_dA(d, KB));
  const int64_t q_pad = ceil_div(q_count, K16_BQ) * K16_BQ;
  hipLaunchKernelGGL((prepare16_kernel<false>), dim3((unsigned)(q_pad / K16_TS)), dim3(256), 0, st, X, n_total, d, mean, scale_info,
                     KB, q_begin, q_count, (const int*)nullptr, reinterpret_cast<_Float16*>(Q16), Qn, (float*)nullptr, k16_dA(d, KB));
  MELD_LAUNCH_CHECK("meld_knn16_prepare_cross");
  return MELD_OK;
}

extern "C" int meld_knn16_prepare_rows(const double* X, int64_t N, int d, const double* mean, const float* scale_info,
                                       int64_t q_begin, const int32_t* rows, int64_t n_rows, void* Q16, float* Qn,
                                       meld_stream_t stream) {
  MELD_CHECK_ARG(X && mean && scale_info && rows && Q16 && Qn && n_rows > 0 && N > 0,
                 "meld_knn16_prepare_rows: bad arguments");
  const int KB = meld_knn16_kblocks(d);
  if (KB < 0) return KB;
  const int64_t q_pad = ceil_div(n_rows, K16_BQ) * K16_BQ;
  hipLaunchKernelGGL((prepare16_kernel<false>), dim3((unsigned)(q_pad / K16_TS)), dim3(256), 0, S(stream), X, N, d, mean,
                     scale_info, KB, q_begin, n_rows, rows, reinterpret_cast<_Float16*>(Q16), Qn, (float*)nullptr, k16_dA(d, KB));
  MELD_LAUNCH_CHECK("meld_knn16_prepare_rows");
  return MELD_OK;
}

namespace meld {
__global__ __launch_bounds__(256) void knn16_research_thr_kernel(const int* __restrict__ rows, long long n_rows, long long q_pad,
                                                                 long long q_begin, const int* __restrict__ cand_cnt,
                                                                 const float* __restrict__ cand_d2, int cap, int ksel,
                                                                 const float* __restrict__ norm2, const float* __restrict__ nmax,
                                                                 double err_coef, double err_lin, double err3,
                                                                 const float* __restrict__ scale_info, float* __restrict__ thr) {
  const long long i = (long long)blockIdx.x * 256 + threadIdx.x;
  if (i >= q_pad) return;
  const long long r = rows[i < n_rows ? i : n_rows - 1];
  const int c = cand_cnt[r];
  const double tau = (double)cand_d2[r * cap + (c > 0 ? c - 1 : 0)];
  const double nmx = (double)nmax[0];
  const double e1 = err_coef * nmx + err_lin * sqrt((double)norm2[q_begin + r] * nmx);
  const double e3 = err3 * nmx;
  const double s = (double)scale_info[0];
  const float b = (float)((tau + e1 + e3) * (s * s) * (1.0 + 1e-5));
  thr[i] = c >= ksel ? b : INFINITY;
}
}

extern "C" int meld_knn16_research_thresholds(const int32_t* rows, int64_t n_rows, int64_t q_begin, const int32_t* cand_cnt,
                                              const float* cand_d2, int cap, int ksel, const float* norm2, const float* norm2_max,
                                              double err_coef, double err_lin, double err3, const float* scale_info, float* thr,
                                              meld_stream_t stream) {
  MELD_CHECK_ARG(rows && cand_cnt && cand_d2 && norm2 && norm2_max && scale_info && thr && n_rows > 0 && cap > 0,
                 "meld_knn16_research_thresholds: bad arguments");
  const int64_t q_pad = ceil_div(n_rows, K16_BQ) * K16_BQ;
  knn16_research_thr_kernel<<<(unsigned)ceil_div(q_pad, 256), 256, 0, S(stream)>>>(rows, n_rows, q_pad, q_begin, cand_cnt, cand_d2, cap, ksel,
                                                                                   norm2, norm2_max, err_coef, err_lin, err3, scale_info, thr);
  MELD_LAUNCH_CHECK("meld_knn16_research_thresholds");
  return MELD_OK;
}

namespace meld {
__global__ __launch_bounds__(256) void knn16_bounds_symmetrize_kernel(unsigned short* __restrict__ lb, int n, int ld) {
  __shared__ unsigned short ta[64][66], tb[64][66];
  const int nb = (n + 63) / 64;
  int bi = 0, rem = blockIdx.x;
  while (rem >= nb - bi) {
    rem -= nb - bi;
    ++bi;
  }
  const int bj = bi + rem;
// ... 221 lines not shown
  if (w >= n_rows) return;
  const int64_t q = (int64_t)w * 64 + lane;
  float sd = q < n_seed ? thr_seed[q] : -INFINITY;
#pragma unroll
  for (int off = 32; off > 0; off >>= 1) sd = fmaxf(sd, __shfl_xor(sd, off, 64));
  if (lane == 0) wthr[w] = sd + err_coef * norm2_max[0] * scale_info[0] * scale_info[0];
}

__global__ __launch_bounds__(256) void knn16_bits_transpose_and_kernel(const unsigned long long* __restrict__ bits_a,
                                                                       const unsigned long long* __restrict__ bits_b, int n_rows, int wpr,
                                                                       unsigned long long* __restrict__ live) {
  const int lane = threadIdx.x & 63;
  const int tile = blockIdx.x * 4 + (threadIdx.x >> 6);
  const int R = tile / wpr, C = tile % wpr;
  if (R >= (n_rows + 63) / 64) return;
  const int src_row = C * 64 + lane;
  const unsigned long long x = (src_row < n_rows && R < wpr) ? bits_b[(size_t)src_row * wpr + R] : 0ull;
  unsigned long long mine = 0ull;
#pragma unroll 8
  for (int j = 0; j < 64; ++j) {
    const unsigned long long t = __ballot((x >> j) & 1ull);
    if (lane == j) mine = t;
  }
  const int out_row = R * 64 + lane;
  if (out_row < n_rows) live[(size_t)out_row * wpr + C] = mine & bits_a[(size_t)out_row * wpr + C];
}

__global__ __launch_bounds__(256) void knn16_step_list_bits_kernel(const unsigned long long* __restrict__ live, int wpr, int n_tiles,
                                                                   int tile_origin, int two_sided, unsigned* __restrict__ list,
                                                                   long long stride, int* __restrict__ cnt) {
  __shared__ int wtot[2][K16_NWAVE];
  const int tid = threadIdx.x, lane = tid & 63, wave = tid >> 6;
  const int bx = blockIdx.x;
  const unsigned long long* row = live + (size_t)bx * K16_NWAVE * wpr;
  unsigned* out = list + (size_t)bx * (size_t)stride;
  const int t0 = (int)(((long long)tile_origin + (long long)bx * (K16_BQ / K16_TS)) % n_tiles);
  int base = 0, par = 0;
  for (int s0 = 0; s0 < n_tiles; s0 += 256, par ^= 1) {
    const int sidx = s0 + tid;
    unsigned mask = 0u;
    int t = 0;
    if (sidx < n_tiles) {
      t = k16_scan_tile(sidx, t0, n_tiles, two_sided);
      const int wd = t >> 6, bt = t & 63;
#pragma unroll
      for (int w = 0; w < K16_NWAVE; ++w) mask |= (unsigned)((row[(size_t)w * wpr + wd] >> bt) & 1ull) << w;
    }
    const bool keep = mask != 0u || sidx == 0;
    const unsigned long long bal = __ballot(keep);
    if (lane == 0) wtot[par][wave] = __popcll(bal);
    __syncthreads();
    int before = base;
    for (int w = 0; w < wave; ++w) before += wtot[par][w];
    if (keep) out[before + __popcll(bal & (((unsigned long long)1 << lane) - 1ull))] = (unsigned)t | (mask << 24);
    base += wtot[par][0] + wtot[par][1] + wtot[par][2] + wtot[par][3];
  }
  if (tid == 0) cnt[bx] = base;
}

extern "C" int meld_knn16_step_lists(const void* lb2, const float* thr_seed, int64_t n_ref, int d, int64_t q_count, int nprod,
                                     const float* norm2_max, const float* scale_info, int64_t q_begin, uint32_t* list,
                                     int64_t list_stride, int32_t* cnt, meld_stream_t stream) {
  MELD_CHECK_ARG(lb2 && norm2_max && scale_info && list && cnt && n_ref > 0 && q_count > 0 && (nprod == 1 || nprod == 3) && q_begin >= 0,
                 "meld_knn16_step_lists: bad arguments");
  static_assert(K16_NWAVE == 4 && K16_BQ == 256, "knn16_step_list_kernel is written for 4 waves of 64 queries");
  const int n_tiles = (int)ceil_div(n_ref, K16_TS);
  MELD_CHECK_ARG(n_tiles < (1 << 24) && list_stride >= n_tiles, "meld_knn16_step_lists: list_stride must hold the %d tiles of a block", n_tiles);
  const int tile_origin = (int)((q_begin / K16_TS) % n_tiles);
  hipLaunchKernelGGL(knn16_step_list_kernel, dim3((unsigned)ceil_div(q_count, K16_BQ)), dim3(256), 0, S(stream),
                     reinterpret_cast<const __half*>(lb2), thr_seed, n_tiles, (float)meld_knn16_error_coef(nprod, d), norm2_max, scale_info,
                     tile_origin, 1, list, (long long)list_stride, cnt);
  MELD_LAUNCH_CHECK("knn16_step_list_kernel");
  return MELD_OK;
}

extern "C" size_t meld_knn16_list_scratch_bytes(int64_t n_ref) {
  const size_t n_q = (size_t)ceil_div(n_ref, K16_BQ) * K16_NWAVE, wpr = (size_t)ceil_div(ceil_div(n_ref, K16_TS), 64);
  return ((n_q * sizeof(float) + 255) / 256) * 256 + 3 * n_q * wpr * sizeof(unsigned long long);
}

static int k16_step_lists_direct_impl(const double* X, int64_t N, int d, const double* mean, const float* scale_info,
                                      const float* norm2_max, const void* Rt16, const float* thr_seed, const float* q_norm2,
                                      int nprod, void* temp, void* scratch, uint32_t* list, int64_t list_stride, int32_t* cnt,
                                      int lead_only, meld_stream_t stream) {
  MELD_CHECK_ARG(nprod == 1 || nprod == 3, "meld_knn16_step_lists_direct: nprod must be 1 or 3");
  MELD_CHECK_ARG(X && mean && scale_info && norm2_max && Rt16 && thr_seed && q_norm2 && temp && scratch && list && cnt && N > 0,
                 "meld_knn16_step_lists_direct: bad arguments");
  const int KB = meld_knn16_kblocks(d);
  if (KB < 0) return KB;
  const int n_t = (int)ceil_div(N, K16_TS), n_q = (int)ceil_div(N, K16_BQ) * K16_NWAVE;
  MELD_CHECK_ARG(n_t < (1 << 24) && list_stride >= n_t, "meld_knn16_step_lists_direct: list_stride must hold the %d tiles of a block", n_t);
  const int wpr = (int)ceil_div(n_t, 64);
  const size_t n_c = (size_t)ceil_div(n_t, K16_BOUNDS_THREADS) * K16_BOUNDS_THREADS;
  hipStream_t st = S(stream);
  _Float16* c16 = reinterpret_cast<_Float16*>(temp);
  float* cn = reinterpret_cast<float*>(reinterpret_cast<char*>(temp) + n_c * (size_t)KB * 64);
  float* cr = cn + n_c;
  float* wthr = reinterpret_cast<float*>(scratch);
  unsigned long long* bits_a = reinterpret_cast<unsigned long long*>(reinterpret_cast<char*>(scratch) + (((size_t)n_q * sizeof(float) + 255) / 256) * 256);
  unsigned long long* bits_b = bits_a + (size_t)n_q * wpr;
  unsigned long long* live = bits_b + (size_t)n_q * wpr;
  MELD_HIP_CALL(hipMemsetAsync(temp, 0, n_c * ((size_t)KB * 64 + 2 * sizeof(float)), st));
  hipLaunchKernelGGL(tile_spheres_kernel, dim3(n_t), dim3(256), sizeof(float) * K16_TS * (size_t)(d | 1), st, X, N, d, mean, scale_info, KB, c16, cn, cr, 0, k16_dA(d, KB));
  const float es = (float)meld_knn16_error_coef(nprod, d);
  hipLaunchKernelGGL(knn16_wave_thresholds_kernel, dim3((unsigned)ceil_div(n_q, 4)), dim3(256), 0, st, thr_seed, N, n_q, es, norm2_max,
                     scale_info, wthr);
  MELD_HIP_CALL(hipMemsetAsync(bits_a, 0, 2 * (size_t)n_q * wpr * sizeof(unsigned long long), st));
  const int bt = KB <= 4 ? K16_BOUNDS_THREADS : K16_BOUNDS_THREADS / 2;
  const int gx = (int)(n_c / bt);
  const int gy = std::max(1, std::min(n_q, (int)ceil_div(2048, gx)));
  const float ec = (float)meld_knn16_error_coef(1, d);
  const int dA = k16_dA(d, KB);
  const bool lead = lead_only != 0 && dA > 0 && KB >= 2;
#define K16_BITS_LAUNCH(KBV, BTV)                                                                                          \
  if (lead)                                                                                                                \
    hipLaunchKernelGGL((knn16_tile_bounds_kernel<KBV, true, BTV, true, (KBV >= 2 ? 1 : KBV)>), dim3(gx, gy), dim3(BTV), 0, st, c16, cn, cr, \
                       reinterpret_cast<const _Float16*>(Rt16), n_t, 0, n_q, ec, norm2_max, scale_info, thr_seed, N, es, 1, q_norm2, \
                       (float)meld_knn16_error_coef_const(nprod, d), (float)meld_knn16_error_coef_lin(nprod), (__half*)nullptr, wthr,  \
                       bits_a, bits_b, wpr, dA);                                                                          \
  else                                                                                                                     \
  hipLaunchKernelGGL((knn16_tile_bounds_kernel<KBV, true, BTV, true>), dim3(gx, gy), dim3(BTV), 0, st, c16, cn, cr,        \
                     reinterpret_cast<const _Float16*>(Rt16), n_t, 0, n_q, ec, norm2_max, scale_info, thr_seed, N, es, 1, q_norm2, \
                     (float)meld_knn16_error_coef_const(nprod, d), (float)meld_knn16_error_coef_lin(nprod), (__half*)nullptr, wthr,  \
                     bits_a, bits_b, wpr)
#define K16_BITS_CASE(KBV) \
  case KBV:                \
    K16_BITS_LAUNCH(KBV, (KBV <= 4 ? K16_BOUNDS_THREADS : K16_BOUNDS_THREADS / 2)); \
    break;
  switch (KB) {
    K16_BITS_CASE(1)
    K16_BITS_CASE(2)
    K16_BITS_CASE(3)
    K16_BITS_CASE(4)
    K16_BITS_CASE(5)
    K16_BITS_CASE(6)
    K16_BITS_CASE(7)
    K16_BITS_CASE(8)
    K16_BITS_CASE(9)
    default:
      set_err("meld_knn16_step_lists_direct: no kernel for %d K blocks", KB);
      return MELD_ERR_UNSUPPORTED;
  }
#undef K16_BITS_CASE
#undef K16_BITS_LAUNCH
  MELD_LAUNCH_CHECK("knn16_tile_bounds_kernel(bits)");
  const int64_t n_tiles64 = (int64_t)ceil_div(n_q, 64) * wpr;
  hipLaunchKernelGGL(knn16_bits_transpose_and_kernel, dim3((unsigned)ceil_div(n_tiles64, 4)), dim3(256), 0, st, bits_a, bits_b, n_q, wpr, live);
  hipLaunchKernelGGL(knn16_step_list_bits_kernel, dim3((unsigned)ceil_div(N, K16_BQ)), dim3(256), 0, st, live, wpr, n_t, 0, 1, list,
                     (long long)list_stride, cnt);
  MELD_LAUNCH_CHECK("knn16_step_list_bits_kernel");
  return MELD_OK;
}

extern "C" int meld_knn16_step_lists_direct(const double* X, int64_t N, int d, const double* mean, const float* scale_info,
                                            const float* norm2_max, const void* Rt16, const float* thr_seed, const float* q_norm2,
                                            int nprod, void* temp, void* scratch, uint32_t* list, int64_t list_stride, int32_t* cnt,
                                            meld_stream_t stream) {
  return k16_step_lists_direct_impl(X, N, d, mean, scale_info, norm2_max, Rt16, thr_seed, q_norm2, nprod, temp, scratch, list, list_stride, cnt, 0,
                                    stream);
}
extern "C" int meld_knn16_step_lists_direct_lead(const double* X, int64_t N, int d, const double* mean, const float* scale_info,
                                                 const float* norm2_max, const void* Rt16, const float* thr_seed, const float* q_norm2,
                                                 int nprod, void* temp, void* scratch, uint32_t* list, int64_t list_stride, int32_t* cnt,
                                                 int lead_only, meld_stream_t stream) {
  return k16_step_lists_direct_impl(X, N, d, mean, scale_info, norm2_max, Rt16, thr_seed, q_norm2, nprod, temp, scratch, list, list_stride, cnt,
                                    lead_only, stream);
}

extern "C" int meld_knn16_seed_thresholds_mfma(const void* Q16, const float* Qn, const void* Rt16, const float* scale_info,
                                               const float* norm2_max, int64_t n_ref, int d, int64_t q_begin,
                                               int64_t q_count, int knn, double radius_factor, int nprod, int side_tiles,
                                               float* thr_init, meld_stream_t stream) {
  const int side = side_tiles > 0 ? side_tiles : (int)std::min<double>(64.0, std::max<double>(8.0, (double)n_ref / 12500.0));
  MELD_CHECK_ARG(Q16 && Qn && Rt16 && scale_info && norm2_max && thr_init && n_ref > 0 && q_count > 0 && q_begin >= 0,
                 "meld_knn16_seed_thresholds_mfma: bad arguments");
  MELD_CHECK_ARG(q_begin % K16_BQ == 0, "meld_knn16_seed_thresholds_mfma: q_begin must be a multiple of the query block (%d)", K16_BQ);
  MELD_CHECK_ARG(knn >= 1 && radius_factor >= 1.0 && (nprod == 1 || nprod == 3), "meld_knn16_seed_thresholds_mfma: bad kernel parameters");
  const int KB = meld_knn16_kblocks(d);
  if (KB < 0) return KB;
  const int n_b = (int)ceil_div(q_count, K16_BQ);
  hipStream_t st = S(stream);
  if (knn + 1 > SEED_KMAX) {
    MELD_HIP_CALL(hipMemsetD32Async(reinterpret_cast<hipDeviceptr_t>(thr_init), 0x7f800000, (size_t)n_b * K16_BQ, st));
    return MELD_OK;
  }
  const float rf2 = (float)(radius_factor * radius_factor * (1.0 + 1e-6));
  const int n_tiles = (int)ceil_div(n_ref, K16_TS);
  const float ec = (float)meld_knn16_error_coef_const(1, d), el = (float)meld_knn16_error_coef_lin(1);
  (void)nprod;
#define K16_SEEDM_LAUNCH(KBV, KV)                                                                                       \
  hipLaunchKernelGGL((knn16_seed_mfma_kernel<KBV, KV>), dim3((unsigned)ceil_div(n_b * K16_NWAVE, SEED_WAVES)),            \
                     dim3(64 * SEED_WAVES), 0, st, reinterpret_cast<const _Float16*>(Q16), Qn,                            \
                     reinterpret_cast<const _Float16*>(Rt16), scale_info, norm2_max, n_tiles, (int)(q_begin / K16_TS),   \
                     side, n_b * K16_NWAVE, knn + 1, rf2, ec, el, thr_init)
#define K16_SEEDM_CASE(KBV)          \
  case KBV:                          \
    if (knn + 1 <= 16)               \
      K16_SEEDM_LAUNCH(KBV, 16);     \
    else                             \
      K16_SEEDM_LAUNCH(KBV, 64);     \
    break;
  switch (KB) {
    K16_SEEDM_CASE(1)
    K16_SEEDM_CASE(2)
    K16_SEEDM_CASE(3)
    K16_SEEDM_CASE(4)
    K16_SEEDM_CASE(5)
    K16_SEEDM_CASE(6)
    K16_SEEDM_CASE(7)
    K16_SEEDM_CASE(8)
    K16_SEEDM_CASE(9)
    default:
      set_err("meld_knn16_seed_thresholds_mfma: no kernel for %d K blocks", KB);
      return MELD_ERR_UNSUPPORTED;
  }
#undef K16_SEEDM_CASE
#undef K16_SEEDM_LAUNCH
  MELD_LAUNCH_CHECK("knn16_seed_mfma_kernel");
  return MELD_OK;
}

template <int KB, int STATS>
static void k16_launch_topk(dim3 grid, hipStream_t st, const K16Args& ka, bool listed, bool ee, int nprod) {
  if (listed) {
    if constexpr (KB >= 2 && KB <= 7) {
      if (ee) {
        hipLaunchKernelGGL((knn16_topk_kernel<KB, STATS, 1, true, true>), grid, dim3(K16_THREADS), 0, st, ka);
        return;
      }
    }
    hipLaunchKernelGGL((knn16_topk_kernel<KB, STATS, 1, true>), grid, dim3(K16_THREADS), 0, st, ka);
  } else if (nprod == 1) {
    hipLaunchKernelGGL((knn16_topk_kernel<KB, STATS, 1>), grid, dim3(K16_THREADS), 0, st, ka);
  } else {
    hipLaunchKernelGGL((knn16_topk_kernel<KB, STATS, 3>), grid, dim3(K16_THREADS), 0, st, ka);
  }
}

static int k16_topk_impl(const void* Q16, const float* Qn, const void* Rt16, const float* scale_info,
                         int64_t n_ref, int d,
                         int64_t q_count, int ksel, int nprod, int n_slices, const void* lb2,
                         const float* norm2_max, int64_t q_begin, const float* thr_init, int knn,
                         double radius_factor, int32_t* cand_idx, float* cand_d2, int32_t* cand_cnt,
                         float* cand_thr, uint64_t* tiles_done, const int32_t* block_order, const uint32_t* step_list,
                         const int32_t* step_cnt, int64_t list_stride, meld_stream_t stream, int partial_test = 0, int two_counters = 0) {
  MELD_CHECK_ARG(nprod == 1 || nprod == 3, "meld_knn16_topk: nprod must be 1 or 3");
  MELD_CHECK_ARG(step_list == nullptr || (step_cnt != nullptr && nprod == 1 && lb2 == nullptr && thr_init != nullptr),
                 "meld_knn16_topk_listed: step lists go with the hi-only pass, start thresholds and no table");
  MELD_CHECK_ARG(n_slices >= 1 && n_slices * ksel <= K16_MERGE_MAX, "meld_knn16_topk: n_slices=%d must satisfy n_slices * ksel <= %d",
// ... 211 lines not shown
```

### meld_amd/graph.py

```python
from __future__ import annotations

from ._options import opt

import math
import time

from types import SimpleNamespace

import numpy as np
import torch

from ._lib import check, get_lib, ptr
from .knn_plan import SearchOptions, plan_knn_search, search_nprod, sphere_layout

__all__ = ["DeviceGraph", "build_knn_graph", "default_ksel", "EVENTS", "record_events"]

EVENTS = {"enabled": False, "pairs": []}


def record_events(enabled=True):
    EVENTS["enabled"] = bool(enabled)
    EVENTS["pairs"] = []


# ... 350 lines not shown

    def __init__(self, device=None, search=None, prune=None, nprod=None, spmm=None):
        self.lib = get_lib()
        self.spmm = spmm
        o = SearchOptions.from_env(search=search, prune=prune, nprod=nprod)
        self.search, self.nprod, self.prune, self.rotate, self.rotate_min_cells = o.search, o.nprod, o.prune, o.rotate, o.rotate_min_cells
        self.radius_cut, self.seed, self.seeded_bounds, self.block_order = o.radius_cut, o.seed, o.seeded_bounds, o.block_order
        if not torch.cuda.is_available():
            raise RuntimeError("meld_amd needs a ROCm GPU (MI355X); there is no CPU fallback")
        self.device = torch.device("cuda", torch.cuda.current_device()) if device is None else torch.device(device)

    def col_stats(self, X):
        N, d = int(X.shape[0]), int(X.shape[1])
        out = torch.empty(3, d, dtype=torch.float64, device=X.device)
        tb = self.lib.meld_col_stats_temp_bytes(d)
        tmp = torch.empty(tb, dtype=torch.uint8, device=X.device)
        check(self.lib.meld_col_stats_f64(ptr(X), N, d, ptr(out[0]), ptr(out[1]), ptr(out[2]), ptr(tmp), tb, _stream()), "meld_col_stats_f64")
        return out[0], out[1], out[2]

    def frame_axes_async(self, X, col_stats):
        lib = self.lib
        N, d = int(X.shape[0]), int(X.shape[1])
        if col_stats is None or d > int(lib.meld_frame_max_dims()) or not plan_knn_search(lib, N, d, 0, N, 1, 2, options=self).frame:
            return None
        st = _stream()
        mean = col_stats[0] / N
        cov = torch.zeros(d, d, dtype=torch.float64, device=X.device)
        check(lib.meld_cov_sample_f64(ptr(X), N, d, ptr(mean), max(1, N // 32768), ptr(cov), st), "meld_cov_sample_f64")
        host = torch.empty(d, d, dtype=torch.float64, pin_memory=True)
        host.copy_(cov, non_blocking=True)
        done = torch.cuda.Event()
        done.record()

        def finish(lead):
            done.synchronize()
            evals, evecs = _eigh_one_thread(host.numpy())
            tot = float(evals.sum())
            if not np.isfinite(tot) or tot <= 0.0 or float(evals[-lead:].sum()) < 0.5 * tot:
                return False
            At = np.zeros((d, int(lib.meld_frame_max_dims())))
            At[:, :d] = evecs[:, ::-1].T
            return torch.from_numpy(At).to(X.device, non_blocking=True)

        return finish

    def principal_frame(self, X, mean, lead, comm=None, axes=None):
        lib, st = self.lib, _stream()
        N, d = int(X.shape[0]), int(X.shape[1])
        if axes is not None and (comm is None or getattr(comm, "world", 1) == 1):
            At = axes(lead)
            if At is False:
                return None
            out = torch.empty_like(X)
            check(lib.meld_rotate_rows_f64(ptr(X), N, d, ptr(mean), ptr(At), ptr(out), st), "meld_rotate_rows_f64")
            return out
        wide = d > int(lib.meld_frame_max_dims())
        stride = max(1, N // 32768)
        if wide:
            Xs = X[::stride] - mean
            cov = torch.triu(Xs.T @ Xs)
            del Xs
        else:
            cov = torch.zeros(d, d, dtype=torch.float64, device=X.device)
            check(lib.meld_cov_sample_f64(ptr(X), N, d, ptr(mean), stride, ptr(cov), st), "meld_cov_sample_f64")
        if comm is not None and getattr(comm, "world", 1) > 1:
            if comm.rank != 0:
                cov.zero_()
            comm.all_reduce_sum(cov)
        evals, evecs = _eigh_one_thread(cov.cpu().numpy())
        tot = float(evals.sum())
        if not np.isfinite(tot) or tot <= 0.0 or float(evals[-lead:].sum()) < 0.5 * tot:
            return None
        if wide:
            V = torch.from_numpy(np.ascontiguousarray(evecs[:, ::-1])).to(X.device)
            return torch.addmm(-(mean @ V), X, V)
        At = np.zeros((d, int(lib.meld_frame_max_dims())))
        At[:, :d] = evecs[:, ::-1].T
        At = torch.from_numpy(At).to(X.device)
        out = torch.empty_like(X)
        check(lib.meld_rotate_rows_f64(ptr(X), N, d, ptr(mean), ptr(At), ptr(out), st), "meld_rotate_rows_f64")
        return out

    def directed_kernel_coo(self, X, q_begin, q_count, knn, decay, thresh, ksel, tm=None, force_fallback=False, n_refs=None, assemble=False, comm=None,
                            bw_scale=1.0, bw_fixed=None, col_stats=None, knn_max=None, symm=(0, 0.0), count_rows_ge=None, frame_axes=None):
        N = int(X.shape[0])
        NR = int(n_refs) if n_refs is not None else N
        if n_refs is not None and not (0 < NR <= q_begin and q_begin + q_count <= N):
            raise ValueError("cross search: the queries must lie behind the n_refs references")
        a = SimpleNamespace(X=X, N=N, d=int(X.shape[1]), NR=NR, cross=n_refs is not None, q_begin=q_begin, q_count=q_count, knn=knn, decay=decay,
                            thresh=thresh, bw_scale=bw_scale, bw_fixed=bw_fixed, knn_max=knn_max, force_fallback=force_fallback,
                            col_stats=col_stats, frame_axes=frame_axes, tm=tm or _Timer(False))
        r = self._search_and_refine(a, ksel, comm)
        retry_from = None
        if r.n_flag > max(1024, q_count // 100) and ksel < 128 and r.plan.search == "f16x3" and not force_fallback:
            retry_from, ksel = (ksel, r.n_flag), 128
            r = self._search_and_refine(a, ksel, None)
        s = self._exact_sweep(a, r, count_rows_ge)
        keys, vals, assembled = self._emit(a, r, s, ksel, assemble, symm)
        p, c = r.plan, r.cands
        info = dict(ksel=int(ksel), KP=int(c.KP), search=p.search, nprod=p.nprod, n_flagged_rows=r.n_flag,
                    prune=p.prune, radius_cut=p.radius_cut, seed=p.seed != "none", seeded_bounds=p.seeded_bounds, block_order=p.block_order != "none",
                    step_lists=p.lists != "none", principal_frame=p.frame, two_phase=p.two_pass, n_rows_bandwidth_recomputed=s.n_rebandwidth,
                    n_researched_rows=r.n_flag_stage1 if p.stage2 else 0, nnz_directed=r.m_main + s.fb_total,
                    wave_tiles_done=r.tiles_done_h, blocks_past_partial_test=r.blocks_on_h, pairs_past_filter=r.pairs_kept_h)
        if s.rows_at_least is not None:
            info["rows_with_at_least"] = s.rows_at_least
        if assembled is not None:
            info["assembled"] = assembled
        if retry_from is not None:
            info["ksel_retry_from"], info["n_flagged_rows_first_try"] = int(retry_from[0]), int(retry_from[1])
        return keys, vals, r.bw, info

    def _search_and_refine(self, a, ksel, comm):
        lib, dev = self.lib, a.X.device
        nprod = search_nprod(self.nprod, a.d)
        resident = lib.meld_knn16_resident_blocks(a.d, nprod) if lib.meld_knn16_kblocks(a.d) > 0 and nprod in (1, 3) else 0
        plan = plan_knn_search(lib, a.N, a.d, a.q_begin, a.q_count, a.knn, ksel, options=self, cross=a.cross, bandwidth=a.bw_fixed is not None,
                               world=getattr(comm, "world", 1) if comm is not None else 1, resident=resident)
        a.tm.start()
        col_min = col_max = None
        if a.col_stats is not None:
            sums, col_min, col_max = a.col_stats
            mean = sums / a.N
        elif a.d <= 256:
            sums, col_min, col_max = self.col_stats(a.X)
            mean = sums / a.N
        else:
            mean = a.X.mean(dim=0)
        norm2 = torch.empty(a.N, dtype=torch.float32, device=dev)
        nmax = torch.zeros(1, dtype=torch.float32, device=dev)
        if plan.search == "wide":
            c = self._candidates_wide(a, plan, ksel, mean, norm2, nmax)
        elif plan.search == "f32":
            c = self._candidates_f32(a, plan, ksel, mean, norm2, nmax)
        else:
            c = self._candidates_f16x3(a, plan, ksel, comm, mean, col_min, col_max, norm2, nmax)
        a.tm.stop("knn_topk")
        return self._refine(a, c, ksel)

    def _candidates_wide(self, a, plan, ksel, mean, norm2, nmax):
        dev, N, q_begin, q_count = a.X.device, a.N, a.q_begin, a.q_count
        cap = int(ksel)
        Xc = a.X - mean
        n2 = (Xc * Xc).sum(dim=1)
        norm2.copy_(n2.to(torch.float32))
        nmax.copy_(n2.max().to(torch.float32).reshape(1))
        a.tm.stop("prepare")
        kk = min(int(ksel), N)
        cand_idx = torch.zeros(q_count * cap, dtype=torch.int32, device=dev)
        cand_d2 = torch.full((q_count * cap,), float("inf"), dtype=torch.float32, device=dev)
        cand_cnt = torch.full((q_count,), kk, dtype=torch.int32, device=dev)
        QC, RC = 4096, 32768
        with _EventSpan("knn_topk", N=N, d=a.d, q=q_count):
            for q0 in range(0, q_count, QC):
                q1 = min(q_count, q0 + QC)
                Xq = Xc[q_begin + q0 : q_begin + q1]
                nq = n2[q_begin + q0 : q_begin + q1]
                best_d = torch.full((q1 - q0, 0), 0.0, dtype=torch.float64, device=dev)
                best_i = torch.zeros((q1 - q0, 0), dtype=torch.int64, device=dev)
                for r0 in range(0, N, RC):
                    r1 = min(N, r0 + RC)
                    D = nq[:, None] + n2[None, r0:r1] - 2.0 * (Xq @ Xc[r0:r1].T)
                    ids = torch.arange(r0, r1, device=dev, dtype=torch.int64)[None, :].expand(q1 - q0, -1)
                    D = torch.cat([best_d, D], dim=1)
                    ids = torch.cat([best_i, ids], dim=1)
                    best_d, sel = torch.topk(D, min(kk, D.shape[1]), dim=1, largest=False, sorted=True)
                    best_i = torch.gather(ids, 1, sel)
                rows = torch.arange(q0, q1, device=dev, dtype=torch.int64)[:, None] * cap + torch.arange(kk, device=dev)[None, :]
                cand_d2[rows.reshape(-1)] = best_d.clamp_(min=0.0).to(torch.float32).reshape(-1)
                cand_idx[rows.reshape(-1)] = best_i.to(torch.int32).reshape(-1)
        return SimpleNamespace(plan=plan, idx=cand_idx, d2=cand_d2, cnt=cand_cnt, thr=None, cap=cap, err_coef=1e-6, err_lin=0.0, KP=a.d,
                               norm2=norm2, nmax=nmax, tiles_done=None, research=None)

    def _candidates_f32(self, a, plan, ksel, mean, norm2, nmax):
        lib, st, dev, X, N, d = self.lib, _stream(), a.X.device, a.X, a.N, a.d
        KP = lib.meld_knn_padded_dim(d)
        if KP < 0:
            check(KP, "meld_knn_padded_dim")
        TS, BQ = lib.meld_knn_tile_refs(), lib.meld_knn_block_queries()
        cap = lib.meld_knn_row_capacity(ksel)
        if cap < 0:
            check(cap, "meld_knn_row_capacity")
        n_tiles = (N + TS - 1) // TS
        Rt = torch.empty(n_tiles * KP * TS, dtype=torch.float32, device=dev)
        check(lib.meld_knn_prepare_refs(ptr(X), N, d, ptr(mean), KP, ptr(Rt), ptr(norm2), ptr(nmax), st), "meld_knn_prepare_refs")
        q_pad = ((a.q_count + BQ - 1) // BQ) * BQ
        Q = torch.empty(q_pad * KP, dtype=torch.float32, device=dev)
        check(lib.meld_knn_prepare_queries(ptr(X), N, d, ptr(mean), KP, a.q_begin, a.q_count, ptr(Q), st), "meld_knn_prepare_queries")
        a.tm.stop("prepare")
        cand_idx = torch.empty(q_pad * cap, dtype=torch.int32, device=dev)
        cand_d2 = torch.empty(q_pad * cap, dtype=torch.float32, device=dev)
        cand_cnt = torch.empty(q_pad, dtype=torch.int32, device=dev)
        with _EventSpan("knn_topk", N=N, d=d, q=a.q_count):
            check(lib.meld_knn_topk(ptr(Q), ptr(Rt), N, KP, a.q_count, ksel, ptr(cand_idx), ptr(cand_d2), ptr(cand_cnt), st), "meld_knn_topk")
        return SimpleNamespace(plan=plan, idx=cand_idx, d2=cand_d2, cnt=cand_cnt, thr=None, cap=cap, err_coef=lib.meld_knn_error_coef(d), err_lin=0.0,
                               KP=KP, norm2=norm2, nmax=nmax, tiles_done=None, research=None)

    def _candidates_f16x3(self, a, plan, ksel, comm, mean, col_min, col_max, norm2, nmax):
        lib, dev = self.lib, a.X.device
        cap = lib.meld_knn16_row_capacity(ksel)
        if cap < 0:
            check(cap, "meld_knn16_row_capacity")
        plan, o, nmax = self._operands16(a, plan, comm, mean, col_min, col_max, norm2, nmax)
        c = SimpleNamespace(plan=plan, cap=cap, err_coef=lib.meld_knn16_error_coef_const(plan.nprod, a.d), err_lin=lib.meld_knn16_error_coef_lin(plan.nprod),
                            KP=16 * o.KB, norm2=norm2, nmax=nmax, research=o if plan.stage2 else None)
        c.idx = torch.empty(o.q_pad * cap, dtype=torch.int32, device=dev)
        c.d2 = torch.empty(o.q_pad * cap, dtype=torch.float32, device=dev)
        c.cnt = torch.empty(o.q_pad, dtype=torch.int32, device=dev)
        c.thr, rfac = None, 1.0
        if plan.radius_cut:
            c.thr = torch.full((o.q_pad,), float("inf"), dtype=torch.float32, device=dev)
            rfac = max(_radius_factor(a.decay, a.thresh) * float(a.bw_scale), 1.0)
        c.tiles_done = torch.zeros(4, dtype=torch.int64, device=dev)
        seeds = self._start_thresholds(a, plan, o, c, rfac)
        lists = self._step_lists(a, plan, o, seeds, nmax, comm)
        self._search16(a, plan, o, c, ksel, seeds, rfac, lists)
        return c

    def _operands16(self, a, plan, comm, mean, col_min, col_max, norm2, nmax):
        lib, st, dev, X, N, d = self.lib, _stream(), a.X.device, a.X, a.N, a.d
        KB, TS, BQ = lib.meld_knn16_kblocks(d), lib.meld_knn16_tile_refs(), lib.meld_knn16_block_queries()
        o = SimpleNamespace(X_s=X, mean_s=mean, KB=KB, BQ=BQ, n_tiles=(a.NR + TS - 1) // TS, q_pad=((a.q_count + BQ - 1) // BQ) * BQ)
        if plan.frame:
            X_s = self.principal_frame(X, mean, int(lib.meld_knn16_split_dims(d)), comm, axes=a.frame_axes)
            if X_s is None:
                plan = plan.without_frame()
            else:
                sums_s, col_min, col_max = self.col_stats(X_s)
                o.X_s, o.mean_s = X_s, sums_s / N
        o.Rt = torch.empty(o.n_tiles * lib.meld_knn16_tile_bytes(d), dtype=torch.uint8, device=dev)
        o.Q = torch.empty(o.q_pad * lib.meld_knn16_query_bytes(d), dtype=torch.uint8, device=dev)
        o.Qn = torch.empty(o.q_pad, dtype=torch.float32, device=dev)
        o.scale_info = torch.empty(4, dtype=torch.float32, device=dev)
        tail = (a.q_begin, a.q_count, ptr(o.Rt), ptr(o.Q), ptr(o.Qn), ptr(norm2), ptr(nmax), ptr(o.scale_info), st)
        if a.cross:
            check(lib.meld_knn16_prepare_cross(ptr(X), a.NR, N, d, ptr(mean), *tail), "meld_knn16_prepare_cross")
            norm2[a.q_begin : a.q_begin + a.q_count] = o.Qn[: a.q_count]
            nmax = torch.maximum(nmax, o.Qn[: a.q_count].max().reshape(1))
        elif col_min is not None:
            check(lib.meld_knn16_prepare_scaled(ptr(o.X_s), N, d, ptr(o.mean_s), ptr(col_min), ptr(col_max), *tail), "meld_knn16_prepare_scaled")
        else:
            check(lib.meld_knn16_prepare(ptr(o.X_s), N, d, ptr(o.mean_s), *tail), "meld_knn16_prepare")
        a.tm.stop("prepare")
        return plan, o, nmax

    def _start_thresholds(self, a, plan, o, c, rfac):
        lib, st, dev = self.lib, _stream(), a.X.device
        if plan.seed == "bandwidth":
            rad = (a.bw_fixed[a.q_begin : a.q_begin + a.q_count] * float(a.bw_scale)).clamp_(min=float(np.finfo(float).eps)) * _radius_factor(a.decay, a.thresh)
            nmx = c.nmax.to(torch.float64)
            e_row = float(c.err_coef) * nmx + float(c.err_lin) * torch.sqrt(c.norm2[a.q_begin : a.q_begin + a.q_count].to(torch.float64) * nmx)
            seeds = torch.full((o.q_pad,), float("inf"), dtype=torch.float32, device=dev)
            seeds[: a.q_count] = ((rad * rad + 1.01 * e_row) * o.scale_info[0].to(torch.float64) ** 2 * (1.0 + 1e-5)).to(torch.float32)
            if o.q_pad > a.q_count:
                seeds[a.q_count :] = seeds[a.q_count - 1]
            return seeds
        if plan.seed == "mfma":
            seeds = torch.empty(o.q_pad, dtype=torch.float32, device=dev)
            check(lib.meld_knn16_seed_thresholds_mfma(ptr(o.Q), ptr(o.Qn), ptr(o.Rt), ptr(o.scale_info), ptr(c.nmax), a.N, a.d, a.q_begin, a.q_count, a.knn,
                                                      rfac, plan.nprod, 0, ptr(seeds), st), "meld_knn16_seed_thresholds_mfma")
            a.tm.stop("seed")
            return seeds
        return None

    def _step_lists(self, a, plan, o, seeds, nmax, comm):
        if not plan.prune:
            return None, None, None, None
        lib, st, dev, N, d = self.lib, _stream(), a.X.device, a.N, a.d
        X_s, mean_s, n_tiles, n_blocks = o.X_s, o.mean_s, o.n_tiles, o.q_pad // o.BQ
        tmpb = torch.empty(lib.meld_knn16_bounds_temp_bytes(N, d, a.q_count), dtype=torch.uint8, device=dev)
        if plan.bounds == "bounds_from_spheres":
            rows_c, row_b = sphere_layout(lib, N, d)
            per = rows_c // comm.world
            t0s = min(comm.rank * per, n_tiles)
            t1s = min(t0s + per, n_tiles)
            tmpb.zero_()
            check(lib.meld_knn16_tile_spheres(ptr(X_s), N, d, ptr(mean_s), ptr(o.scale_info), ptr(tmpb), t0s, max(t1s - t0s, 0), st), "meld_knn16_tile_spheres")
            parts = (tmpb[: rows_c * row_b], tmpb[rows_c * row_b : rows_c * (row_b + 4)], tmpb[rows_c * (row_b + 4) : rows_c * (row_b + 8)])
            for arr, width in zip(parts, (row_b, 4, 4)):
                mine = arr[comm.rank * per * width : (comm.rank + 1) * per * width].clone()
                comm.all_gather_rows(arr, mine)
        lb2 = step_list = step_cnt = None
        if plan.lists == "direct":
            step_list = torch.empty(n_blocks * n_tiles, dtype=torch.int32, device=dev)
            step_cnt = torch.empty(n_blocks, dtype=torch.int32, device=dev)
            scratch = torch.empty(lib.meld_knn16_list_scratch_bytes(N), dtype=torch.uint8, device=dev)
            check(lib.meld_knn16_step_lists_direct_lead(ptr(X_s), N, d, ptr(mean_s), ptr(o.scale_info), ptr(nmax), ptr(o.Rt), ptr(seeds), ptr(o.Qn), plan.nprod,
                                                        ptr(tmpb), ptr(scratch), ptr(step_list), n_tiles, ptr(step_cnt), int(plan.lead_bounds), st),
                  "meld_knn16_step_lists_direct")
            del scratch
        else:
            sb = plan.seeded_bounds
            lb2 = torch.empty(lib.meld_knn16_bounds_bytes(N, a.q_count), dtype=torch.uint8, device=dev)
            check((lib.meld_knn16_bounds_from_spheres if plan.bounds == "bounds_from_spheres" else lib.meld_knn16_bounds)(
                ptr(X_s), N, d, ptr(mean_s), ptr(o.scale_info), ptr(nmax), ptr(o.Rt), a.q_begin, a.q_count, ptr(seeds) if sb else None,
                ptr(o.Qn) if sb else None, plan.nprod, ptr(tmpb), ptr(lb2), st), "meld_knn16_bounds")
            if plan.lists == "table":
                step_list = torch.empty(n_blocks * n_tiles, dtype=torch.int32, device=dev)
                step_cnt = torch.empty(n_blocks, dtype=torch.int32, device=dev)
                check(lib.meld_knn16_step_lists(ptr(lb2), ptr(seeds), N, d, a.q_count, plan.nprod, ptr(nmax), ptr(o.scale_info), a.q_begin,
                                                ptr(step_list), n_tiles, ptr(step_cnt), st), "meld_knn16_step_lists")
        work = step_cnt
        if plan.block_order == "work":
            work = torch.empty(n_blocks, dtype=torch.int32, device=dev)
            check(lib.meld_knn16_block_work(ptr(lb2), ptr(seeds), N, d, a.q_count, plan.nprod, ptr(nmax), ptr(o.scale_info), ptr(work), st), "meld_knn16_block_work")
        block_order = torch.argsort(work, descending=True, stable=True).to(torch.int32) if plan.block_order != "none" else None
        a.tm.stop("bounds")
        return lb2, step_list, step_cnt, block_order

    def _search16(self, a, plan, o, c, ksel, seeds, rfac, lists):
        lib, st, dev, d, q_count, q_pad, cap = self.lib, _stream(), a.X.device, a.d, a.q_count, o.q_pad, c.cap
        lb2, step_list, step_cnt, block_order = lists
        q0 = 0 if a.cross else a.q_begin
        tiles_b = c.tiles_done
        if plan.two_pass:
            with _EventSpan("knn_filter", N=a.N, d=d, q=q_count):
                check(lib.meld_knn16_partial_filter(ptr(o.Q), ptr(o.Qn), ptr(o.Rt), ptr(o.scale_info), ptr(c.nmax), d, q_count, ptr(seeds), ptr(step_list),
                                                    ptr(step_cnt), o.n_tiles, ptr(step_cnt), ptr(c.tiles_done), ptr(block_order), st), "meld_knn16_partial_filter")
                if block_order is not None:
                    block_order = torch.argsort(step_cnt, descending=True, stable=True).to(torch.int32)
            tiles_b = c.tiles_done[1:]
            a.tm.stop("knn_filter")
        S = plan.main_slices
        with _EventSpan("knn_topk", N=a.N, d=d, q=q_count):
            if S > 1:
                out = (torch.empty(S * q_pad * cap, dtype=torch.int32, device=dev), torch.empty(S * q_pad * cap, dtype=torch.float32, device=dev),
                       torch.empty(S * q_pad, dtype=torch.int32, device=dev), torch.full((S, q_pad), float("inf"), dtype=torch.float32, device=dev))
            else:
                out = (c.idx, c.d2, c.cnt, c.thr)
            if step_list is not None:
                check(lib.meld_knn16_topk_listed_partial(ptr(o.Q), ptr(o.Qn), ptr(o.Rt), ptr(o.scale_info), a.NR, d, q_count, ksel, ptr(step_list), ptr(step_cnt),
                                                         o.n_tiles, ptr(c.nmax), q0, ptr(seeds), plan.knn_cut, rfac, *map(ptr, out), ptr(tiles_b), ptr(block_order),
                                                         S, int(plan.partial_in_search), st), "meld_knn16_topk_listed")
            else:
                check(lib.meld_knn16_topk(ptr(o.Q), ptr(o.Qn), ptr(o.Rt), ptr(o.scale_info), a.NR, d, q_count, ksel, plan.nprod, S, ptr(lb2), ptr(c.nmax), q0,
                                          ptr(seeds), plan.knn_cut, rfac, *map(ptr, out), ptr(c.tiles_done), ptr(block_order), st), "meld_knn16_topk")
            if S > 1:
                check(lib.meld_knn16_merge_slices(*map(ptr, out[:3]), q_count, ksel, S, ptr(c.idx), ptr(c.d2), ptr(c.cnt), st), "meld_knn16_merge_slices")
                c.thr.copy_(out[3].amin(0))
            del out
            while _WHILE_SEARCHING:
                _WHILE_SEARCHING.pop()()
        del o.Q

    def _refine(self, a, c, ksel):
        lib, st, dev, q_count = self.lib, _stream(), a.X.device, a.q_count
        r = SimpleNamespace(plan=c.plan, cands=c)
        max_rank = 0 if a.knn_max is None else int(a.knn_max) + 1
        r.bw = torch.empty(q_count, dtype=torch.float64, device=dev)
        r.cand_val = torch.empty(q_count * ksel, dtype=torch.float64, device=dev)
        r.keep_cnt = torch.empty(q_count, dtype=torch.int32, device=dev)
        r.flag_rows = torch.empty(q_count, dtype=torch.int32, device=dev)
        n_flag = torch.zeros(1, dtype=torch.int32, device=dev)
        nmax_used = c.nmax
        if a.force_fallback:
            nmax_used = torch.full((1,), float("inf"), dtype=torch.float32, device=dev)
        check(
            lib.meld_knn_refine(
                ptr(a.X), a.N, a.d, a.q_begin, q_count, ptr(c.idx), ptr(c.d2), ptr(c.cnt), ptr(c.thr), ksel, c.cap, a.knn, float(a.decay),
                float(a.thresh), ptr(nmax_used), float(c.err_coef), ptr(c.norm2), float(c.err_lin), ptr(r.bw), ptr(r.cand_val), ptr(r.keep_cnt),
                ptr(r.flag_rows), ptr(n_flag), None, 0, None, float(a.bw_scale), ptr(a.bw_fixed), max_rank, st,
            ),
            "meld_knn_refine",
        )
        r.n_flag = r.n_flag_stage1 = int(n_flag.item())
        a.tm.stop("refine")
        stage2 = c.research is not None and r.n_flag > 0 and not a.force_fallback
        if stage2:
            self._stage2(a, c, r, ksel, n_flag, max_rank)
        c.research = None
        r.keep_off = _scan_i32(lib, r.keep_cnt, st)
        td, p = c.tiles_done, c.plan
        heads = [n_flag[0].to(torch.int64), r.keep_off[q_count]] + ([td[0], td[2] if p.two_pass else td[1], td[1]] if td is not None else [])
        heads_h = torch.stack(heads).tolist()
        if stage2:
            r.n_flag = int(heads_h[0])
        r.m_main = int(heads_h[1])
# ... 23 lines not shown
                                                 ptr(o.scale_info), ptr(thr2), st), "meld_knn16_research_thresholds")
        c2_idx = torch.empty(n_slices * q2_pad * cap, dtype=torch.int32, device=dev)
        c2_d2 = torch.empty(n_slices * q2_pad * cap, dtype=torch.float32, device=dev)
        c2_cnt = torch.empty(n_slices * q2_pad, dtype=torch.int32, device=dev)
        with _EventSpan("knn_topk_stage2", N=a.N, d=d, q=n_flag_h):
            check(lib.meld_knn16_topk(ptr(Q2), ptr(Qn2), ptr(o.Rt), ptr(o.scale_info), a.NR, d, n_flag_h, ksel, 3, n_slices, None, ptr(c.nmax), 0, ptr(thr2), 0, 1.0,
                                      ptr(c2_idx), ptr(c2_d2), ptr(c2_cnt), None, None, None, st), "meld_knn16_topk(stage 2)")
            if n_slices > 1:
                m_idx = torch.empty(q2_pad * cap, dtype=torch.int32, device=dev)
                m_d2 = torch.empty(q2_pad * cap, dtype=torch.float32, device=dev)
                m_cnt = torch.empty(q2_pad, dtype=torch.int32, device=dev)
                check(lib.meld_knn16_merge_slices(ptr(c2_idx), ptr(c2_d2), ptr(c2_cnt), n_flag_h, ksel, n_slices, ptr(m_idx), ptr(m_d2), ptr(m_cnt), st), "meld_knn16_merge_slices")
                c2_idx, c2_d2, c2_cnt = m_idx, m_d2, m_cnt
        n_flag.zero_()
        check(
            lib.meld_knn_refine(
                ptr(a.X), a.N, d, a.q_begin, n_flag_h, ptr(c2_idx), ptr(c2_d2), ptr(c2_cnt), None, ksel, cap, a.knn, float(a.decay),
                float(a.thresh), ptr(c.nmax), float(lib.meld_knn16_error_coef(3, d)), None, 0.0, ptr(r.bw), ptr(r.cand_val), ptr(r.keep_cnt),
                ptr(r.flag_rows), ptr(n_flag), ptr(rows2), cap, ptr(c.idx), float(a.bw_scale), ptr(a.bw_fixed), max_rank, st,
            ),
            "meld_knn_refine(stage 2)",
        )
        a.tm.stop("knn_stage2")

    def _exact_sweep(self, a, r, count_rows_ge):
        lib, st, dev, q_count, n_flag_h = self.lib, _stream(), a.X.device, a.q_count, r.n_flag
        knn_chk = a.knn if a.bw_fixed is None else 2**31 - 1
        s = SimpleNamespace(n_rebandwidth=0, fb_total=0, fb_off=None, fb_col=None, fb_val=None, fb_cnt=None, rows_at_least=None)
        if n_flag_h > 0:
            r.flag_rows = flag_rows = torch.sort(r.flag_rows[:n_flag_h]).values.contiguous()
            fb_cnt = torch.empty(n_flag_h, dtype=torch.int32, device=dev)
            err = torch.zeros(1, dtype=torch.int32, device=dev)
            cursor = torch.zeros(n_flag_h, dtype=torch.int32, device=dev)

            def sweep(fill, what, fb_cnt=None, fb_off=None, fb_col=None, fb_val=None, err=None):
                check(lib.meld_knn_radius_exact(ptr(a.X), a.NR, a.d, a.q_begin, ptr(flag_rows), n_flag_h, ptr(r.bw), knn_chk, float(a.decay), float(a.thresh), fill,
                                                ptr(fb_cnt), ptr(fb_off), ptr(cursor), ptr(fb_col), ptr(fb_val), ptr(err), float(a.bw_scale), st), what)

            sweep(0, "meld_knn_radius_exact(count)", fb_cnt=fb_cnt, err=err)
            if int(err.item()) != 0:
                bad = torch.nonzero(fb_cnt < 0).reshape(-1)
                rows_bad = flag_rows[bad].to(torch.int64)
                r.bw[rows_bad] = _exact_bandwidth(a.X, a.q_begin + rows_bad, a.knn, n_refs=a.NR)
                fb_cnt.zero_()
                cursor.zero_()
                err.zero_()
                sweep(0, "meld_knn_radius_exact(recount)", fb_cnt=fb_cnt, err=err)
                if int(err.item()) != 0:
                    raise NotImplementedError(
                        "degenerate neighbourhoods: the exact sweep could not settle the bandwidth of {} rows".format(int((fb_cnt < 0).sum())))
                s.n_rebandwidth = int(bad.shape[0])
            fb_off = _scan_i32(lib, fb_cnt, st)
            fb_total = int(fb_off[n_flag_h].item())
            need = 12 * fb_total + 32 * (r.m_main + fb_total)
            if need > torch.cuda.get_device_properties(dev).total_memory:
                raise MemoryError(
                    "the kernel radius covers {:.3g} neighbours per cell on average: the graph would hold {:.3g} entries ({:.0f} GB to "
                    "assemble) -- raise decay or thresh".format((r.m_main + fb_total) / max(q_count, 1), float(r.m_main + fb_total), need / 1e9))
            fb_col = torch.empty(max(fb_total, 1), dtype=torch.int32, device=dev)
            fb_val = torch.empty(max(fb_total, 1), dtype=torch.float64, device=dev)
            sweep(1, "meld_knn_radius_exact(fill)", fb_off=fb_off, fb_col=fb_col, fb_val=fb_val)
            if a.knn_max is not None and fb_total > 0 and int(fb_cnt.max()) > int(a.knn_max):
                rows_e = torch.repeat_interleave(torch.arange(n_flag_h, device=dev), fb_cnt.to(torch.int64))
                o = torch.argsort(fb_col[:fb_total].to(torch.int64), stable=True)
                o = o[torch.argsort(-fb_val[:fb_total][o], stable=True)]
                o = o[torch.argsort(rows_e[o], stable=True)]
                rank = torch.arange(fb_total, device=dev) - fb_off[:n_flag_h][rows_e[o]]
                keep = o[rank < int(a.knn_max)]
                keep = keep[torch.argsort(rows_e[keep], stable=True)]
                fb_col, fb_val = fb_col[keep].contiguous(), fb_val[keep].contiguous()
                fb_cnt = torch.clamp(fb_cnt, max=int(a.knn_max))
                fb_off = _scan_i32(lib, fb_cnt, st)
                fb_total = int(fb_off[n_flag_h].item())
            s.fb_total, s.fb_off, s.fb_col, s.fb_val, s.fb_cnt = fb_total, fb_off, fb_col, fb_val, fb_cnt
        a.tm.stop("radius_exact")
        if count_rows_ge is not None:
            tot = r.keep_cnt.to(torch.int64)
            if n_flag_h > 0 and s.fb_total > 0:
                tot = tot.clone()
                tot[r.flag_rows[:n_flag_h].to(torch.int64)] = s.fb_cnt.to(torch.int64)
            s.rows_at_least = int(((tot + 1) >= int(count_rows_ge)).sum())
        return s

    def _emit(self, a, r, s, ksel, assemble, symm):
        lib, st, dev, q_count, n_flag_h, c = self.lib, _stream(), a.X.device, a.q_count, r.n_flag, r.cands
        M = r.m_main + s.fb_total
        assembled = None
        if assemble and M > 0 and a.q_begin == 0 and q_count == a.NR and not a.cross and opt("MELD_ASSEMBLE", "bucket") == "bucket" \
                and opt("MELD_ASSEMBLE_FUSED", "1") != "0":
            B = int(lib.meld_csr_bucket_slots())
            if ksel <= B and q_count * B * 12 <= torch.cuda.mem_get_info(dev)[0] // 4:
                cursor = r.keep_cnt.clone()
                if n_flag_h > 0 and s.fb_total > 0:
                    cursor[r.flag_rows[:n_flag_h].to(torch.int64)] = s.fb_cnt
                tcol = torch.empty(q_count * B, dtype=torch.int32, device=dev)
                tval = torch.empty(q_count * B, dtype=torch.float64, device=dev)
                check(lib.meld_coo_emit_scatter(q_count, ptr(c.idx), ptr(r.cand_val), ksel, c.cap, ptr(r.keep_cnt), ptr(r.flag_rows), n_flag_h,
                                                ptr(s.fb_off), ptr(s.fb_col), ptr(s.fb_val), s.fb_total, ptr(cursor), ptr(tcol), ptr(tval), st),
                      "meld_coo_emit_scatter")
                a.tm.stop("coo_emit")
                assembled = self._finish_buckets(cursor, tcol, tval, q_count, sums_diag=1.0, symm=symm)
                if assembled is not None and self.last_row_sums is not None:
                    assembled = assembled + (self.last_row_sums[1],)
                a.tm.stop("symmetrize")
                del cursor, tcol, tval
        keys = vals = None
        if assembled is None:
            keys = torch.empty(2 * M, dtype=torch.int64, device=dev)
            vals = torch.empty(2 * M, dtype=torch.float64, device=dev)
            if M > 0:
                check(
                    lib.meld_coo_emit(
                        a.q_begin, q_count, ptr(c.idx), ptr(r.cand_val), ptr(c.cnt), ksel, c.cap, ptr(r.keep_off), ptr(r.flag_rows),
                        n_flag_h, ptr(s.fb_off), ptr(s.fb_col), ptr(s.fb_val), r.m_main, M, ptr(keys), ptr(vals), st,
                    ),
                    "meld_coo_emit",
                )
        a.tm.stop("coo_emit")
        return keys, vals, assembled

    def sort_pairs(self, keys, vals, N):
        lib, st = self.lib, _stream()
        n = int(keys.shape[0])
        keys2 = torch.empty_like(keys)
        vals2 = torch.empty_like(vals)
        if n == 0:
            return keys2, vals2
        tb = lib.meld_sort_temp_bytes(n)
        tmp = torch.empty(tb, dtype=torch.uint8, device=keys.device)
        end_bit = 32 + max(1, int(N - 1).bit_length())
        check(lib.meld_sort_pairs_u64_f64(ptr(keys), ptr(keys2), ptr(vals), ptr(vals2), n, end_bit, ptr(tmp), tb, st), "meld_sort_pairs_u64_f64")
        return keys2, vals2

    def partition_remote(self, keys, vals, rows_per_rank, world, rank, cap):
        dev = keys.device
        counts = torch.empty(world, dtype=torch.int32, device=dev)
        send = torch.empty(world * 2 * cap, dtype=torch.int64, device=dev)
        check(self.lib.meld_coo_partition_remote(ptr(keys), ptr(vals), int(keys.shape[0]), int(rows_per_rank), int(world), int(rank),
                                                 int(cap), ptr(counts), ptr(send), _stream()), "meld_coo_partition_remote")
        return send, counts

    def _finish_buckets(self, cursor, tcol, tval, n_rows, sums_diag=None, symm=(0, 0.0)):
        lib, st, dev = self.lib, _stream(), cursor.device
        i32 = dict(dtype=torch.int32, device=dev)
        ucnt = torch.empty(n_rows, **i32)
        flags = torch.empty(1, **i32)
        check(lib.meld_csr_rows_sort_merge(ptr(cursor), n_rows, ptr(tcol), ptr(tval), ptr(ucnt), ptr(flags), int(symm[0]), float(symm[1]), st), "meld_csr_rows_sort_merge")
        rowptr = _scan_i32(lib, ucnt, st)
        nnz, flag = (int(v) for v in torch.stack([rowptr[n_rows], flags[0].to(torch.int64)]).tolist())
        if flag != 0:
            return None
        col = torch.empty(nnz, **i32)
        val = torch.empty(nnz, dtype=torch.float64, device=dev)
        self.last_row_sums = None
        if nnz > 0 and sums_diag is not None:
            sums = torch.empty(n_rows, dtype=torch.float64, device=dev)
            check(lib.meld_csr_compact_rows_sums(ptr(rowptr), n_rows, ptr(tcol), ptr(tval), ptr(col), ptr(val), float(sums_diag), ptr(sums), st),
                  "meld_csr_compact_rows_sums")
            self.last_row_sums = (sums_diag, sums)
        elif nnz > 0:
            check(lib.meld_csr_compact_rows(ptr(rowptr), n_rows, ptr(tcol), ptr(tval), ptr(col), ptr(val), st), "meld_csr_compact_rows")
        self.last_assemble = "bucket"
        return rowptr, col, val

    def assemble_rows(self, keys, vals, row_begin, n_rows, N, foreign=False, symm=(0, 0.0)):
        lib, st, dev = self.lib, _stream(), keys.device
        n = int(keys.shape[0])
        B = int(lib.meld_csr_bucket_slots())
        bucket_bytes = n_rows * B * 12
        fits = bucket_bytes <= torch.cuda.mem_get_info(dev)[0] // 4 if n_rows > 0 else True
        if n > 0 and n_rows > 0 and fits and opt("MELD_ASSEMBLE", "bucket") != "sort":
            i32 = dict(dtype=torch.int32, device=dev)
            cursor = torch.empty(n_rows, **i32)
            tcol = torch.empty(n_rows * B, **i32)
            tval = torch.empty(n_rows * B, dtype=torch.float64, device=dev)
            check(lib.meld_coo_scatter_rows(ptr(keys), ptr(vals), n, row_begin, n_rows, ptr(cursor), ptr(tcol), ptr(tval), st), "meld_coo_scatter_rows")
            done = self._finish_buckets(cursor, tcol, tval, n_rows, symm=symm)
            if done is not None:
                return done
            del cursor, tcol, tval
        self.last_assemble = "sort" if n > 0 else "empty"
        if foreign and n > 0:
            rows = keys >> 32
            own = (rows >= row_begin) & (rows < row_begin + n_rows)
            keys, vals = keys[own].contiguous(), vals[own].contiguous()
            n = int(keys.shape[0])
        keys2, vals2 = self.sort_pairs(keys, vals, N)
        if symm[0] != 0 and n > 0:
            first = torch.ones(n, dtype=torch.bool, device=dev)
            first[1:] = keys2[1:] != keys2[:-1]
            seg = torch.cumsum(first, 0) - 1
            nseg = int(seg[-1].item()) + 1
            cnt = torch.bincount(seg, minlength=nseg)
            if int(cnt.max().item()) > 2:
                raise NotImplementedError("kernel_symm other than '+': an entry of the kernel occurs more than once per direction")
            hi = torch.zeros(nseg, dtype=torch.float64, device=dev).scatter_reduce_(0, seg, vals2, "amax", include_self=False)
            lo = torch.zeros(nseg, dtype=torch.float64, device=dev).scatter_reduce_(0, seg, vals2, "amin", include_self=False)
            lo = torch.where(cnt == 2, lo, torch.zeros_like(lo))
            if symm[0] == 1:
                v, keep = 4.0 * hi * lo, cnt == 2
            else:
                v = 2.0 * (float(symm[1]) * lo + (1.0 - float(symm[1])) * hi)
                keep = v != 0.0
            ukeys, uvals = keys2[first][keep].contiguous(), v[keep].contiguous()
            nnz = int(ukeys.shape[0])
        else:
            tb = lib.meld_merge_temp_bytes(max(n, 1))
            tmp = torch.empty(tb, dtype=torch.uint8, device=dev)
            n_unique = torch.zeros(1, dtype=torch.int64, device=dev)
            ukeys = torch.empty_like(keys2)
            uvals = torch.empty_like(vals2)
            check(lib.meld_coo_merge(ptr(keys2), ptr(vals2), n, ptr(ukeys), ptr(uvals), ptr(n_unique), ptr(tmp), tb, st), "meld_coo_merge")
            nnz = int(n_unique.item())
        rowptr = torch.empty(n_rows + 1, dtype=torch.int64, device=dev)
        col = torch.empty(nnz, dtype=torch.int32, device=dev)
        check(lib.meld_csr_from_keys(ptr(ukeys), nnz, row_begin, n_rows, ptr(rowptr), ptr(col), st), "meld_csr_from_keys")
        return rowptr, col, uvals[:nnz].clone()

    def gather_rows(self, X, perm):
        X = X.contiguous()
        perm = perm.to(torch.int64).contiguous()
        out = torch.empty((int(perm.shape[0]), int(X.shape[1])), dtype=torch.float64, device=X.device)
        check(self.lib.meld_gather_rows_f64(ptr(X), ptr(perm), int(perm.shape[0]), int(X.shape[1]), ptr(out), _stream()), "meld_gather_rows_f64")
        return out

    def row_sums(self, rowptr, val, n_rows, diag):
        out = torch.empty(n_rows, dtype=torch.float64, device=rowptr.device)
        check(self.lib.meld_csr_row_sums(ptr(rowptr), ptr(val), n_rows, float(diag), ptr(out), _stream()), "meld_csr_row_sums")
        return out

    def anisotropy(self, rowptr, col, val, n_rows, ksum_all, row_off, a):
        check(self.lib.meld_csr_anisotropy(ptr(rowptr), ptr(col), ptr(val), n_rows, ptr(ksum_all), row_off, float(a), _stream()), "meld_csr_anisotropy")

    def anisotropy_degrees(self, rowptr, col, val, n_rows, ksum_all, row_off, a):
        dw = torch.empty(n_rows, dtype=torch.float64, device=val.device)
        check(self.lib.meld_csr_anisotropy_degrees(ptr(rowptr), ptr(col), ptr(val), n_rows, ptr(ksum_all), row_off, float(a), ptr(dw), _stream()),
              "meld_csr_anisotropy_degrees")
        return dw
# ... 272 lines not shown
def resolve_graph_params(N, knn, thresh, ksel):
    if N < 3:
        raise ValueError("need at least 3 points to build a kNN graph, got {}".format(N))
    if knn > N - 2:
        knn = N - 2
    thresh = float(max(thresh, np.finfo(float).eps))
    if ksel is None:
        ksel = default_ksel(knn)
    if ksel < knn + 2:
        raise NotImplementedError(
            "knn={} needs a candidate list of at least knn+2 entries but the search kernel holds at most 128".format(knn)
        )
    return int(knn), thresh, int(ksel)


def symm_code(kernel_symm, theta):
    if kernel_symm == "+":
        return (0, 0.0)
    if kernel_symm == "*":
        return (1, 0.0)
    if kernel_symm == "mnn":
        if theta is None:
            theta = 1.0
        if not isinstance(theta, (int, float)) or theta < 0 or theta > 1:
            raise ValueError("theta {} not recognized. Expected a float between 0 and 1".format(theta))
        return (2, float(theta))
    if kernel_symm is None:
        raise NotImplementedError("kernel_symm=None (a directed kernel) is not implemented: the filter needs a symmetric Laplacian")
    raise ValueError("kernel_symm '{}' not recognized. Choose from '+', '*', 'mnn', or 'none'.".format(kernel_symm))


def build_knn_graph(X, knn=5, decay=40, thresh=1e-4, anisotropy=1, ksel=None, profile=False, force_fallback=False,
                    reorder=True, bandwidth=None, bandwidth_scale=1.0, col_stats=None, knn_max=None, kernel_symm="+", theta=None, ops=None):
    if not (isinstance(X, torch.Tensor) and X.is_cuda and X.dtype == torch.float64 and X.dim() == 2):
        raise TypeError("build_knn_graph expects a CUDA float64 tensor [N, d]")
    X = X.contiguous()
    N, d = int(X.shape[0]), int(X.shape[1])
    ops = ops if ops is not None else HipOps(X.device)
    tm = _Timer(profile)
    knn, thresh, ksel = resolve_graph_params(N, knn, thresh, ksel)
    bw_scale = float(bandwidth_scale)
    if not (bw_scale > 0 and math.isfinite(bw_scale)):
        raise ValueError("bandwidth_scale must be positive and finite, got {!r}".format(bandwidth_scale))
    symm = symm_code(kernel_symm, theta)
    if knn_max is not None:
        knn_max = int(knn_max)
        if knn_max < knn:
            raise ValueError("`knn_max` must be greater than or equal to `knn`")
        if knn_max + 2 > ksel:
            ksel = min(128, ((knn_max + 2 + 31) // 32) * 32)
            if knn_max + 2 > ksel:
                raise NotImplementedError("knn_max={} needs a candidate list beyond the 128 entries the search kernel holds".format(knn_max))
    bw_fixed = None
    if bandwidth is not None:
        if callable(bandwidth):
            raise NotImplementedError("a callable bandwidth is not implemented by the MI355X graph builder")
        b = torch.as_tensor(np.asarray(bandwidth, dtype=np.float64)).to(X.device)
        if b.dim() == 0:
            b = b.expand(N)
        if tuple(b.shape) != (N,):
            raise ValueError("bandwidth must be a number or have one entry per cell ({}), got shape {}".format(N, tuple(b.shape)))
        if not bool(torch.isfinite(b).all()) or bool((b < 0).any()):
            raise ValueError("bandwidth must be finite and non-negative")
        bw_fixed = b.contiguous().clone()

    frame_axes = ops.frame_axes_async(X, col_stats) if (bw_fixed is None and hasattr(ops, "frame_axes_async")) else None
    perm = None
    if reorder:
        from .reorder import locality_permutation

        tm.start()
        perm = locality_permutation(X)
        if perm is not None:
            X = ops.gather_rows(X, perm)
            if bw_fixed is not None:
                bw_fixed = bw_fixed.index_select(0, perm).contiguous()
        tm.stop("reorder")

    k1 = knn + 1
    info = None
    if knn_max is not None and decay is not None and math.isfinite(decay) and 36 * k1 < min(knn_max + 1, N):
        trial = ops.directed_kernel_coo(X, 0, N, knn, decay, thresh, ksel, tm=tm, force_fallback=force_fallback, assemble=True,
                                        bw_scale=bw_scale, bw_fixed=bw_fixed, col_stats=col_stats, knn_max=None, symm=symm, count_rows_ge=6 * k1,
                                        frame_axes=frame_axes)
        if trial[3]["rows_with_at_least"] <= N // 10 or 36 * k1 >= N / 2:
            keys, vals, bw, info = trial
            info["knn_max_uncapped_as_upstream"] = True
            knn_max = None
        del trial
    if info is None:
        keys, vals, bw, info = ops.directed_kernel_coo(X, 0, N, knn, decay, thresh, ksel, tm=tm, force_fallback=force_fallback, assemble=True,
                                                       bw_scale=bw_scale, bw_fixed=bw_fixed, col_stats=col_stats, knn_max=knn_max, symm=symm,
                                                       frame_axes=frame_axes)
    if bw_scale != 1.0:
        bw = (bw * bw_scale).clamp_(min=float(np.finfo(float).eps))
    if info.get("nnz_directed", 0) == 0:
        raise ValueError("the kernel has no off-diagonal entries; cannot build a graph")
    tm.start()
    ksum = None
    if info.get("assembled") is not None:
        asm = info.pop("assembled")
        rowptr, col, val = asm[:3]
        ksum = asm[3] if len(asm) > 3 else None
    else:
        rowptr, col, val = ops.assemble_rows(keys, vals, 0, N, N, symm=symm)
    del keys, vals
    tm.stop("symmetrize")
    if ksum is None:
        ksum = ops.row_sums(rowptr, val, N, 1.0)
    dw = ops.anisotropy_degrees(rowptr, col, val, N, ksum, 0, anisotropy)
    tm.stop("anisotropy_degree")

    nnz = int(col.shape[0])
    info.update(N=N, d=d, knn=knn, nnz=nnz, mean_degree=nnz / N, stage_seconds=dict(tm.t), assemble=getattr(ops, "last_assemble", None))
    G = DeviceGraph(rowptr, col, val, dw, ksum=ksum, anisotropy=anisotropy, info=info)
    G.bandwidth = bw
    G.perm = perm
    G.ops = ops
    return G
```

### meld_amd/knn_plan.py

```python
from __future__ import annotations

import ctypes
import dataclasses
from dataclasses import dataclass
from typing import Optional

from ._lib import check
from ._options import opt


@dataclass(frozen=True)
class SearchOptions:

    search: str = "f16x3"
    nprod: int = 1
    prune: bool = True
    radius_cut: bool = True
    seed: bool = True
    seeded_bounds: bool = True
    block_order: bool = True
    rotate: bool = True
    rotate_min_cells: int = 262144

    @classmethod
    def from_env(cls, search=None, prune=None, nprod=None):
        out = cls(search=search or opt("MELD_KNN_SEARCH", "f16x3"), nprod=1 if nprod is None else int(nprod),
                  prune=(opt("MELD_KNN_PRUNE", "1") != "0") if prune is None else bool(prune),
                  rotate=opt("MELD_KNN_ROTATE", "1") != "0", rotate_min_cells=int(opt("MELD_KNN_ROTATE_MIN", "262144")))
        if out.search not in ("f16x3", "f32"):
            raise ValueError("unknown search kernel {!r}".format(out.search))
        return out


@dataclass(frozen=True)
class KnnPlan:
    search: str
    nprod: int
    frame: bool
    radius_cut: bool
    prune: bool
    seed: str
    knn_cut: int
    bounds: str
    seeded_bounds: bool
    lists: str
    block_order: str
    main_slices: int
    two_pass: bool
    partial_in_search: bool
    stage2: bool
    lead_bounds: Optional[bool] = None
    partial_forced: bool = False

    def __post_init__(self):
        if self.lead_bounds is None:
            object.__setattr__(self, "lead_bounds", self.lists == "direct" and self.frame)

    def without_frame(self):
        return dataclasses.replace(self, frame=False, two_pass=False, lead_bounds=False,
                                   partial_in_search=self.partial_in_search and self.partial_forced)


def search_nprod(nprod, d):
    return 3 if (nprod == 1 and d <= 6) else nprod


def sphere_layout(lib, N, d):
    rows, row_bytes = ctypes.c_int64(0), ctypes.c_int64(0)
    check(lib.meld_knn16_sphere_layout(N, d, ctypes.byref(rows), ctypes.byref(row_bytes)), "meld_knn16_sphere_layout")
    return int(rows.value), int(row_bytes.value)


def plan_knn_search(lib, N, d, q_begin, q_count, knn, ksel, *, options, cross=False, bandwidth=False, world=1, resident=0):
    search = options.search
    if search == "f16x3" and lib.meld_knn16_kblocks(d) < 0:
        search = "wide"
    if cross and search != "f16x3":
        raise NotImplementedError("the search between two point sets runs on the split-fp16 MFMA kernel only (d <= 141)")
    if search != "f16x3":
        return KnnPlan(search, options.nprod, False, False, False, "none", knn, "none", False, "none", "none", 1, False, False, False)
    nprod = search_nprod(options.nprod, d)
    TS, BQ = lib.meld_knn16_tile_refs(), lib.meld_knn16_block_queries()
    n_blocks, n_tiles = -(-q_count // BQ), -(-N // TS)
    radius_cut = bool(options.radius_cut) and knn < ksel
    frame = bool(options.rotate and lib.meld_knn16_split_dims(d) > 0 and nprod == 1 and not cross and options.prune and options.seed
                 and N >= max(16384, options.rotate_min_cells) and q_begin % BQ == 0 and not bandwidth)
    prune = bool(options.prune) and q_begin % TS == 0 and N >= 16384 and not cross
    seed = "none"
    if bandwidth and radius_cut:
        seed = "bandwidth"
    elif options.seed and radius_cut and q_begin % BQ == 0 and not cross:
        seed = "mfma"
    bounds, lists, block_order, seeded_bounds, main_slices = "none", "none", "none", False, 1
    if prune:
        seeded_bounds = seed != "none" and bool(options.seeded_bounds)
        shared = world > 1 and sphere_layout(lib, N, d)[0] % world == 0
        want_lists = seed != "none" and radius_cut and nprod == 1
        if want_lists and seeded_bounds and not shared and q_begin == 0 and q_count == N and opt("MELD_KNN_LIST_DIRECT", "1") != "0":
            lists = "direct"
        else:
            bounds = "bounds_from_spheres" if shared else "bounds"
            lists = "table" if want_lists else "none"
        if options.block_order and n_blocks > 1:
            block_order = "lists" if lists != "none" else "work"
        if radius_cut and resident > 0 and n_blocks < 2 * resident:
            main_slices = int(max(1, min(4, lib.meld_knn16_max_slices(ksel), -(-2 * resident // n_blocks), n_tiles // 64)))
    ee = opt("MELD_KNN16_EE")
    partial = frame if ee is None else ee != "0"
    two = opt("MELD_KNN_TWO_PHASE", "1")
    two_pass = lists != "none" and frame and (main_slices == 1 or two == "2") and two != "0" and ee is None
    lead_bounds = lists == "direct" and frame and opt("MELD_KNN16_LEAD_BOUNDS", "1") != "0"
    return KnnPlan(search, nprod, frame, radius_cut, prune, seed, 0 if seed == "bandwidth" else knn, bounds, seeded_bounds, lists,
                   block_order, main_slices, two_pass, partial, nprod == 1, lead_bounds, ee is not None)
```

Baseline: 27.99 million.

## Fuse kNN operand prep with tile spheres and fold anisotropy into CSR assembly

```diff
diff --git a/include/meld_hip.h b/include/meld_hip.h
--- a/include/meld_hip.h
+++ b/include/meld_hip.h
@@ -58,6 +58,9 @@
 int meld_knn16_prepare_scaled(const double* X, int64_t N, int d, const double* mean, const double* col_min, const double* col_max,
                               int64_t q_begin, int64_t q_count, void* Rt16, void* Q16, float* Qn, float* norm2, float* norm2_max,
                               float* scale_info, meld_stream_t stream);
+int meld_knn16_prepare_fused(const double* X, int64_t N, int d, const double* mean, const double* col_min, const double* col_max,
+                             void* Rt16, void* Q16, float* Qn, float* norm2, float* norm2_max, float* scale_info, void* temp,
+                             meld_stream_t stream);
 size_t meld_knn16_bounds_bytes(int64_t n_ref, int64_t q_count);
 size_t meld_knn16_bounds_temp_bytes(int64_t n_ref, int d, int64_t q_count);
 int meld_knn16_bounds(const double* X, int64_t N, int d, const double* mean, const float* scale_info,
@@ -104,6 +107,9 @@
 int meld_knn16_step_lists_direct_lead(const double* X, int64_t N, int d, const double* mean, const float* scale_info, const float* norm2_max,
                                  const void* Rt16, const float* thr_seed, const float* q_norm2, int nprod, void* temp, void* scratch,
                                  uint32_t* list, int64_t list_stride, int32_t* cnt, int lead_only, meld_stream_t stream);
+int meld_knn16_step_lists_direct_spheres(const double* X, int64_t N, int d, const double* mean, const float* scale_info, const float* norm2_max,
+                                 const void* Rt16, const float* thr_seed, const float* q_norm2, int nprod, void* temp, void* scratch,
+                                 uint32_t* list, int64_t list_stride, int32_t* cnt, int lead_only, meld_stream_t stream);
 int meld_knn16_topk_listed(const void* Q16, const float* Qn, const void* Rt16, const float* scale_info, int64_t n_ref, int d,
                            int64_t q_count, int ksel, const uint32_t* step_list, const int32_t* step_cnt, int64_t list_stride,
                            const float* norm2_max, int64_t q_begin, const float* thr_init, int knn, double radius_factor,
@@ -196,6 +202,10 @@
                              int32_t* flags,
                              int symm ,
                              double theta , meld_stream_t stream);
+int meld_csr_rows_sort_merge_sums(const int32_t* cursor, int64_t n_rows, int32_t* tcol, double* tval, int32_t* ucnt, int32_t* flags,
+                                  int symm, double theta, double diag, double* sums, meld_stream_t stream);
+int meld_csr_compact_rows_anisotropy(const int64_t* rowptr, int64_t n_rows, const int32_t* tcol, const double* tval, int32_t* col,
+                                     double* val, const double* ksum, double anisotropy, double* dw, meld_stream_t stream);
 int meld_csr_compact_rows(const int64_t* rowptr, int64_t n_rows, const int32_t* tcol, const double* tval,
                           int32_t* col, double* val, meld_stream_t stream);
 int meld_csr_compact_rows_sums(const int64_t* rowptr, int64_t n_rows, const int32_t* tcol, const double* tval, int32_t* col,
diff --git a/meld_amd/_lib.py b/meld_amd/_lib.py
--- a/meld_amd/_lib.py
+++ b/meld_amd/_lib.py
@@ -58,6 +58,8 @@
     "meld_knn16_step_lists": (_i32, [_ptr, _ptr, _i64, _i32, _i64, _i32, _ptr, _ptr, _i64, _ptr, _i64, _ptr, _ptr]),
     "meld_knn16_list_scratch_bytes": (_sz, [_i64]),
     "meld_knn16_step_lists_direct": (_i32, [_ptr, _i64, _i32, _ptr, _ptr, _ptr, _ptr, _ptr, _ptr, _i32, _ptr, _ptr, _ptr, _i64, _ptr, _ptr]),
+    "meld_knn16_prepare_fused": (_i32, [_ptr, _i64, _i32, _ptr, _ptr, _ptr, _ptr, _ptr, _ptr, _ptr, _ptr, _ptr, _ptr, _ptr]),
+    "meld_knn16_step_lists_direct_spheres": (_i32, [_ptr, _i64, _i32, _ptr, _ptr, _ptr, _ptr, _ptr, _ptr, _i32, _ptr, _ptr, _ptr, _i64, _ptr, _i32, _ptr]),
     "meld_knn16_step_lists_direct_lead": (_i32, [_ptr, _i64, _i32, _ptr, _ptr, _ptr, _ptr, _ptr, _ptr, _i32, _ptr, _ptr, _ptr, _i64, _ptr, _i32, _ptr]),
     "meld_knn16_topk_listed": (_i32, [_ptr, _ptr, _ptr, _ptr, _i64, _i32, _i64, _i32, _ptr, _ptr, _i64, _ptr, _i64, _ptr, _i32, _f64, _ptr, _ptr, _ptr, _ptr, _ptr, _ptr, _i32, _ptr]),
     "meld_knn16_topk_listed_partial": (_i32, [_ptr, _ptr, _ptr, _ptr, _i64, _i32, _i64, _i32, _ptr, _ptr, _i64, _ptr, _i64, _ptr, _i32, _f64, _ptr, _ptr, _ptr, _ptr, _ptr, _ptr, _i32, _i32, _ptr]),
@@ -96,6 +98,8 @@
     "meld_coo_partition_remote": (_i32, [_ptr, _ptr, _i64, _i64, _i32, _i32, _i64, _ptr, _ptr, _ptr]),
     "meld_csr_rows_sort_merge": (_i32, [_ptr, _i64, _ptr, _ptr, _ptr, _ptr, _i32, _f64, _ptr]),
     "meld_csr_compact_rows": (_i32, [_ptr, _i64, _ptr, _ptr, _ptr, _ptr, _ptr]),
+    "meld_csr_rows_sort_merge_sums": (_i32, [_ptr, _i64, _ptr, _ptr, _ptr, _ptr, _i32, _f64, _f64, _ptr, _ptr]),
+    "meld_csr_compact_rows_anisotropy": (_i32, [_ptr, _i64, _ptr, _ptr, _ptr, _ptr, _ptr, _f64, _ptr, _ptr]),
     "meld_csr_compact_rows_sums": (_i32, [_ptr, _i64, _ptr, _ptr, _ptr, _ptr, _f64, _ptr, _ptr]),
     "meld_csr_row_sums": (_i32, [_ptr, _ptr, _i64, _f64, _ptr, _ptr]),
     "meld_csr_anisotropy": (_i32, [_ptr, _ptr, _ptr, _i64, _ptr, _i64, _f64, _ptr]),
diff --git a/meld_amd/csrc/assemble.hip b/meld_amd/csrc/assemble.hip
--- a/meld_amd/csrc/assemble.hip
+++ b/meld_amd/csrc/assemble.hip
@@ -434,7 +434,7 @@
 
 template <int SL>
 __device__ __forceinline__ int csr_row_merge(int* __restrict__ tcol, double* __restrict__ tval, int64_t base, int n, int lane,
-                                             bool* bad, int symm, double theta) {
+                                             bool* bad, int symm, double theta, double* srow) {
   static_assert(CSR_BUCKET <= 256, "the slot shares a 32-bit key with a 24-bit column");
   unsigned cin[SL];
   bool wide = false;
@@ -527,6 +527,7 @@
     if (is_head[e]) {
       tcol[base + head_pos[e]] = (int)head_col[e];
       tval[base + head_pos[e]] = head_val[e];
+      if (srow != nullptr) srow[head_pos[e]] = head_val[e];
     }
   }
   if (__any(any_bad)) *bad = true;
@@ -535,7 +536,10 @@
 
 __global__ __launch_bounds__(256) void csr_rows_sort_merge_kernel(const int* __restrict__ cursor, int64_t n_rows,
                                                                   int* __restrict__ tcol, double* __restrict__ tval,
-                                                                  int* __restrict__ ucnt, int* __restrict__ flags, int symm, double theta) {
+                                                                  int* __restrict__ ucnt, int* __restrict__ flags, int symm, double theta,
+                                                                  double diag, double* __restrict__ sums) {
+  __shared__ double s_rows[4][CSR_BUCKET];
+  double* srow = sums != nullptr ? s_rows[threadIdx.x >> 6] : nullptr;
   const int lane = threadIdx.x & 63;
   const int64_t r = (int64_t)blockIdx.x * 4 + (threadIdx.x >> 6);
   if (r >= n_rows) return;
@@ -551,14 +555,24 @@
   bool bad = false;
   int total;
   if (n <= 64)
-    total = csr_row_merge<1>(tcol, tval, base, n, lane, &bad, symm, theta);
+    total = csr_row_merge<1>(tcol, tval, base, n, lane, &bad, symm, theta, srow);
   else if (n <= 128)
-    total = csr_row_merge<2>(tcol, tval, base, n, lane, &bad, symm, theta);
+    total = csr_row_merge<2>(tcol, tval, base, n, lane, &bad, symm, theta, srow);
   else
-    total = csr_row_merge<4>(tcol, tval, base, n, lane, &bad, symm, theta);
+    total = csr_row_merge<4>(tcol, tval, base, n, lane, &bad, symm, theta, srow);
   if (lane == 0) {
     ucnt[r] = total;
     if (bad) atomicOr(flags, 2);
+  }
+  if (sums != nullptr) {
+    __builtin_amdgcn_fence(__ATOMIC_ACQ_REL, "workgroup");
+    double s = 0.0;
+    if (lane < 8)
+      for (int k = lane; k < total; k += 8) s += srow[k];
+    s += __shfl_xor(s, 1, 64);
+    s += __shfl_xor(s, 2, 64);
+    s += __shfl_xor(s, 4, 64);
+    if (lane == 0) sums[r] = diag + s;
   }
 }
 
@@ -599,6 +613,49 @@
   if (r < n_rows && g == 0) sums[r] = diag + s;
 }
 
+__global__ __launch_bounds__(256) void csr_compact_rows_anisotropy_kernel(const int64_t* __restrict__ rowptr, int64_t n_rows,
+                                                                          const int* __restrict__ tcol, const double* __restrict__ tval,
+                                                                          int* __restrict__ col, double* __restrict__ val,
+                                                                          const double* __restrict__ ksum, double anisotropy,
+                                                                          double* __restrict__ dw) {
+  const int64_t r = ((int64_t)blockIdx.x * blockDim.x + threadIdx.x) >> 3;
+  const int g = threadIdx.x & 7;
+  double s = 0.0;
+  if (r < n_rows) {
+    const double di = ksum[r];
+    const int64_t src = r * CSR_BUCKET, dst = rowptr[r];
+    const int len = (int)(rowptr[r + 1] - dst);
+    constexpr int U = 4;
+    for (int k0 = g; k0 < len; k0 += 8 * U) {
+      int c[U];
+      double v[U], kj[U];
+#pragma unroll
+      for (int u = 0; u < U; ++u) {
+        const int k = k0 + 8 * u;
+        c[u] = k < len ? tcol[src + k] : 0;
+        v[u] = k < len ? tval[src + k] : 0.0;
+      }
+#pragma unroll
+      for (int u = 0; u < U; ++u) kj[u] = ksum[c[u]];
+#pragma unroll
+      for (int u = 0; u < U; ++u) {
+        const int k = k0 + 8 * u;
+        if (k < len) {
+          const double dd = di * kj[u];
+          const double w = (anisotropy == 0.0) ? v[u] : (anisotropy == 1.0) ? v[u] / dd : v[u] / pow(dd, anisotropy);
+          col[dst + k] = c[u];
+          val[dst + k] = w;
+          s += w;
+        }
+      }
+    }
+  }
+  s += __shfl_xor(s, 1, 64);
+  s += __shfl_xor(s, 2, 64);
+  s += __shfl_xor(s, 4, 64);
+  if (r < n_rows && g == 0) dw[r] = 0.0 + s;
+}
+
 extern "C" int meld_csr_bucket_slots(void) { return CSR_BUCKET; }
 
 extern "C" int meld_coo_scatter_rows(const uint64_t* keys, const double* vals, int64_t n, int64_t row_begin, int64_t n_rows,
@@ -655,8 +712,30 @@
                  "meld_csr_rows_sort_merge: symm must be 0 (+), 1 (*) or 2 (mnn, theta in [0, 1])");
   MELD_HIP_CALL(hipMemsetAsync(flags, 0, sizeof(int32_t), S(stream)));
   hipLaunchKernelGGL(csr_rows_sort_merge_kernel, dim3((unsigned)ceil_div(n_rows, 4)), dim3(256), 0, S(stream), cursor, n_rows,
-                     tcol, tval, ucnt, flags, symm, theta);
+                     tcol, tval, ucnt, flags, symm, theta, 0.0, (double*)nullptr);
   MELD_LAUNCH_CHECK("csr_rows_sort_merge_kernel");
+  return MELD_OK;
+}
+
+extern "C" int meld_csr_rows_sort_merge_sums(const int32_t* cursor, int64_t n_rows, int32_t* tcol, double* tval, int32_t* ucnt,
+                                             int32_t* flags, int symm, double theta, double diag, double* sums, meld_stream_t stream) {
+  MELD_CHECK_ARG(cursor && tcol && tval && ucnt && flags && sums && n_rows > 0, "meld_csr_rows_sort_merge_sums: bad arguments");
+  MELD_CHECK_ARG(symm >= 0 && symm <= 2 && (symm != 2 || (theta >= 0.0 && theta <= 1.0)),
+                 "meld_csr_rows_sort_merge_sums: symm must be 0 (+), 1 (*) or 2 (mnn, theta in [0, 1])");
+  MELD_HIP_CALL(hipMemsetAsync(flags, 0, sizeof(int32_t), S(stream)));
+  hipLaunchKernelGGL(csr_rows_sort_merge_kernel, dim3((unsigned)ceil_div(n_rows, 4)), dim3(256), 0, S(stream), cursor, n_rows,
+                     tcol, tval, ucnt, flags, symm, theta, diag, sums);
+  MELD_LAUNCH_CHECK("csr_rows_sort_merge_kernel");
+  return MELD_OK;
+}
+
+extern "C" int meld_csr_compact_rows_anisotropy(const int64_t* rowptr, int64_t n_rows, const int32_t* tcol, const double* tval,
+                                                int32_t* col, double* val, const double* ksum, double anisotropy, double* dw,
+                                                meld_stream_t stream) {
+  MELD_CHECK_ARG(rowptr && n_rows > 0 && tcol && tval && col && val && ksum && dw, "meld_csr_compact_rows_anisotropy: bad arguments");
+  hipLaunchKernelGGL(csr_compact_rows_anisotropy_kernel, dim3((unsigned)ceil_div(n_rows * 8, 256)), dim3(256), 0, S(stream), rowptr, n_rows,
+                     tcol, tval, col, val, ksum, anisotropy, dw);
+  MELD_LAUNCH_CHECK("csr_compact_rows_anisotropy_kernel");
   return MELD_OK;
 }
 
diff --git a/meld_amd/csrc/knn16.hip b/meld_amd/csrc/knn16.hip
--- a/meld_amd/csrc/knn16.hip
+++ b/meld_amd/csrc/knn16.hip
@@ -1090,26 +1090,11 @@
   if (lane == 0) out_cnt[q] = min(n, ksel);
 }
 
-__global__ __launch_bounds__(256) void tile_spheres_kernel(const double* __restrict__ X, int64_t N, int d,
-                                                           const double* __restrict__ mean,
-                                                           const float* __restrict__ scale_info, int KB,
-                                                           _Float16* __restrict__ cent16, float* __restrict__ cent_n,
-                                                           float* __restrict__ cent_r, int tile0, int dA) {
-  extern __shared__ float xs_dyn[];
-  const int ld = d | 1;
+__device__ __forceinline__ void k16_tile_sphere(const float* xs_dyn, int ld, int cnt, int d, int KB, int dA, int tile,
+                                                _Float16* __restrict__ cent16, float* __restrict__ cent_n, float* __restrict__ cent_r) {
 #define XS(r, k) xs_dyn[(r) * ld + (k)]
   __shared__ float cs[K16_DMAX + 19];
   const int tid = threadIdx.x;
-  const int tile = tile0 + (int)blockIdx.x;
-  const int64_t row0 = (int64_t)tile * K16_TS;
-  const int cnt = (int)min((int64_t)K16_TS, N - row0);
-  const float s = scale_info[0];
-  for (int u = tid; u < K16_TS * d; u += 256) {
-    const int r = u / d, k = u - r * d;
-    const int64_t i = row0 + r;
-    XS(r, k) = i < N ? s * (float)(X[i * d + k] - mean[k]) : 0.0f;
-  }
-  __syncthreads();
   if (tid < KB * 16) {
     float acc = 0.0f;
     if (tid < d)
@@ -1205,6 +1190,27 @@
 #undef XS
 }
 
+__global__ __launch_bounds__(256) void tile_spheres_kernel(const double* __restrict__ X, int64_t N, int d,
+                                                           const double* __restrict__ mean,
+                                                           const float* __restrict__ scale_info, int KB,
+                                                           _Float16* __restrict__ cent16, float* __restrict__ cent_n,
+                                                           float* __restrict__ cent_r, int tile0, int dA) {
+  extern __shared__ float xs_dyn[];
+  const int ld = d | 1;
+  const int tid = threadIdx.x;
+  const int tile = tile0 + (int)blockIdx.x;
+  const int64_t row0 = (int64_t)tile * K16_TS;
+  const int cnt = (int)min((int64_t)K16_TS, N - row0);
+  const float s = scale_info[0];
+  for (int u = tid; u < K16_TS * d; u += 256) {
+    const int r = u / d, k = u - r * d;
+    const int64_t i = row0 + r;
+    xs_dyn[r * ld + k] = i < N ? s * (float)(X[i * d + k] - mean[k]) : 0.0f;
+  }
+  __syncthreads();
+  k16_tile_sphere(xs_dyn, ld, cnt, d, KB, dA, tile, cent16, cent_n, cent_r);
+}
+
 template <int KB, bool SEEDED, int BT, bool BITS = false, int KU = KB>
 __global__ __launch_bounds__(BT) void knn16_tile_bounds_kernel(const _Float16* __restrict__ C16, const float* __restrict__ Cn,
                                                                 const float* __restrict__ Cr,
@@ -1501,6 +1507,112 @@
     } else {
       out_norm[i] = n;
     }
+  }
+}
+
+__global__ __launch_bounds__(256) void prepare16_fused_kernel(const double* __restrict__ X, int64_t N, int d,
+                                                              const double* __restrict__ mean,
+                                                              const float* __restrict__ scale_info, int KB,
+                                                              _Float16* __restrict__ Rt16, _Float16* __restrict__ Q16,
+                                                              float* __restrict__ Qn, float* __restrict__ norm2,
+                                                              float* __restrict__ norm2_max, _Float16* __restrict__ cent16,
+                                                              float* __restrict__ cent_n, float* __restrict__ cent_r, int n_t, int dA) {
+  extern __shared__ float xs_dyn[];
+  const int ld = d | 1;
+#define XS(r, k) xs_dyn[(r) * ld + (k)]
+  const int tid = threadIdx.x;
+  const int64_t row0 = (int64_t)blockIdx.x * K16_TS;
+  const float s = scale_info[0];
+  for (int u = tid; u < K16_TS * d; u += 256) {
+    const int r = u / d, k = u - r * d;
+    const int64_t src = row0 + r < N ? row0 + r : N - 1;
+    XS(r, k) = s * (float)(X[src * d + k] - mean[k]);
+  }
+  __syncthreads();
+  const int r = tid & 63, part = tid >> 6;
+  const int64_t i = row0 + r;
+  const bool is_tile = (int)blockIdx.x < n_t;
+  const bool real = i < N;
+  float n = 0.0f;
+  for (int k = 0; k < d; ++k) n = fmaf(XS(r, k), XS(r, k), n);
+  float nA = 0.0f, nB = real ? n : INFINITY;
+  if (is_tile && dA > 0) {
+    nB = 0.0f;
+    for (int k = 0; k < dA; ++k) nA = fmaf(XS(r, k), XS(r, k), nA);
+    for (int k = dA; k < d; ++k) nB = fmaf(XS(r, k), XS(r, k), nB);
+    const float m_r = 1.03f * 0.0009765625f * nB + (float)d * 2.384185791015625e-07f;
+    nA -= m_r;
+    nB += m_r;
+    if (!real) {
+      nA = INFINITY;
+      nB = 0.0f;
+    }
+  }
+  _Float16 npc[6];
+  {
+    const float src2[2] = {nA, nB};
+#pragma unroll
+    for (int q = 0; q < 2; ++q) {
+      const float nn = src2[q];
+      const _Float16 n1 = (_Float16)nn;
+      const float r1 = isinf(nn) ? 0.0f : nn - (float)n1;
+      const _Float16 n2 = (_Float16)r1;
+      npc[3 * q + 0] = n1;
+      npc[3 * q + 1] = n2;
+      npc[3 * q + 2] = (_Float16)(r1 - (float)n2);
+    }
+  }
+  for (int g = part; g < KB * 2; g += 4) {
+    f16x8 qhi, qlo, rhi, rlo;
+#pragma unroll
+    for (int e = 0; e < 8; ++e) {
+      int cc, pc;
+      k16_slot(g * 8 + e, d, dA, &cc, &pc);
+      _Float16 qh = (_Float16)0.0f, ql = (_Float16)0.0f, rh = (_Float16)0.0f, rl = (_Float16)0.0f;
+      if (cc >= 0) {
+        const float vq = XS(r, cc);
+        qh = (_Float16)vq;
+        ql = (_Float16)(vq - (float)qh);
+        float xr = real ? vq : 0.0f;
+        asm volatile("" : "+v"(xr));
+        const float vr = -2.0f * xr;
+        rh = (_Float16)vr;
+        rl = (_Float16)(vr - (float)rh);
+      } else if (pc >= 0) {
+        qh = (_Float16)1.0f;
+        rh = npc[pc];
+      }
+      qhi[e] = qh;
+      qlo[e] = ql;
+      rhi[e] = rh;
+      rlo[e] = rl;
+    }
+    f16x8* qrow = reinterpret_cast<f16x8*>(Q16) + (size_t)i * ((size_t)KB * 4);
+    qrow[g * 2 + 0] = qhi;
+    qrow[g * 2 + 1] = qlo;
+    if (is_tile) {
+      f16x8* tile = reinterpret_cast<f16x8*>(Rt16) + (size_t)blockIdx.x * ((size_t)KB * 2 * 2 * K16_TS);
+      tile[(size_t)(g * 2 + 0) * K16_TS + r] = rhi;
+      tile[(size_t)(g * 2 + 1) * K16_TS + r] = rlo;
+    }
+  }
+  if (part == 0) {
+    Qn[i] = n;
+    if (is_tile) {
+      float n_orig = 0.0f;
+      if (real) {
+        n_orig = n * scale_info[1];
+        norm2[i] = n_orig;
+      }
+#pragma unroll
+      for (int off = 32; off > 0; off >>= 1) n_orig = fmaxf(n_orig, __shfl_xor(n_orig, off, 64));
+      if (r == 0) atomicMax(reinterpret_cast<int*>(norm2_max), __float_as_int(n_orig));
+    }
+  }
+#undef XS
+  if (is_tile) {
+    const int cnt = (int)min((int64_t)K16_TS, N - row0);
+    k16_tile_sphere(xs_dyn, ld, cnt, d, KB, dA, (int)blockIdx.x, cent16, cent_n, cent_r);
   }
 }
 
@@ -1714,6 +1826,36 @@
                                          float* scale_info, meld_stream_t stream) {
   MELD_CHECK_ARG(col_min && col_max, "meld_knn16_prepare_scaled: null column extremes");
   return k16_prepare_impl(X, N, d, mean, q_begin, q_count, Rt16, Q16, Qn, norm2, norm2_max, scale_info, stream, col_min, col_max);
+}
+
+extern "C" int meld_knn16_prepare_fused(const double* X, int64_t N, int d, const double* mean, const double* col_min, const double* col_max,
+                                        void* Rt16, void* Q16, float* Qn, float* norm2, float* norm2_max, float* scale_info, void* temp,
+                                        meld_stream_t stream) {
+  MELD_CHECK_ARG(X && mean && Rt16 && Q16 && Qn && norm2 && norm2_max && scale_info && temp && N > 0,
+                 "meld_knn16_prepare_fused: null/empty argument");
+  MELD_CHECK_ARG((col_min == nullptr) == (col_max == nullptr), "meld_knn16_prepare_fused: column minima and maxima go together");
+  const int KB = meld_knn16_kblocks(d);
+  if (KB < 0) return KB;
+  hipStream_t st = S(stream);
+  MELD_HIP_CALL(hipMemsetAsync(scale_info, 0, 4 * sizeof(float), st));
+  MELD_HIP_CALL(hipMemsetAsync(norm2_max, 0, sizeof(float), st));
+  if (col_min != nullptr)
+    hipLaunchKernelGGL(absmax_from_extremes_kernel, dim3(1), dim3(256), 0, st, mean, col_min, col_max, d, scale_info);
+  else
+    hipLaunchKernelGGL(absmax_centered_kernel, dim3(2048), dim3(256), 0, st, X, N * (int64_t)d, d, mean, scale_info);
+  hipLaunchKernelGGL(finish_scale_kernel, dim3(1), dim3(1), 0, st, scale_info);
+  const int n_t = (int)ceil_div(N, K16_TS);
+  const size_t n_c = (size_t)ceil_div(n_t, K16_BOUNDS_THREADS) * K16_BOUNDS_THREADS;
+  _Float16* c16 = reinterpret_cast<_Float16*>(temp);
+  float* cn = reinterpret_cast<float*>(reinterpret_cast<char*>(temp) + n_c * (size_t)KB * 64);
+  float* cr = cn + n_c;
+  MELD_HIP_CALL(hipMemsetAsync(temp, 0, n_c * ((size_t)KB * 64 + 2 * sizeof(float)), st));
+  const int64_t q_pad = ceil_div(N, K16_BQ) * K16_BQ;
+  hipLaunchKernelGGL(prepare16_fused_kernel, dim3((unsigned)(q_pad / K16_TS)), dim3(256), sizeof(float) * K16_TS * (size_t)(d | 1), st, X, N, d,
+                     mean, scale_info, KB, reinterpret_cast<_Float16*>(Rt16), reinterpret_cast<_Float16*>(Q16), Qn, norm2, norm2_max, c16, cn, cr,
+                     n_t, k16_dA(d, KB));
+  MELD_LAUNCH_CHECK("meld_knn16_prepare_fused");
+  return MELD_OK;
 }
 
 extern "C" int meld_knn16_prepare_cross(const double* X, int64_t n_refs, int64_t n_total, int d, const double* mean,
@@ -2101,7 +2243,7 @@
 static int k16_step_lists_direct_impl(const double* X, int64_t N, int d, const double* mean, const float* scale_info,
                                       const float* norm2_max, const void* Rt16, const float* thr_seed, const float* q_norm2,
                                       int nprod, void* temp, void* scratch, uint32_t* list, int64_t list_stride, int32_t* cnt,
-                                      int lead_only, meld_stream_t stream) {
+                                      int lead_only, meld_stream_t stream, bool spheres_ready = false) {
   MELD_CHECK_ARG(nprod == 1 || nprod == 3, "meld_knn16_step_lists_direct: nprod must be 1 or 3");
   MELD_CHECK_ARG(X && mean && scale_info && norm2_max && Rt16 && thr_seed && q_norm2 && temp && scratch && list && cnt && N > 0,
                  "meld_knn16_step_lists_direct: bad arguments");
@@ -2119,8 +2261,10 @@
   unsigned long long* bits_a = reinterpret_cast<unsigned long long*>(reinterpret_cast<char*>(scratch) + (((size_t)n_q * sizeof(float) + 255) / 256) * 256);
   unsigned long long* bits_b = bits_a + (size_t)n_q * wpr;
   unsigned long long* live = bits_b + (size_t)n_q * wpr;
-  MELD_HIP_CALL(hipMemsetAsync(temp, 0, n_c * ((size_t)KB * 64 + 2 * sizeof(float)), st));
-  hipLaunchKernelGGL(tile_spheres_kernel, dim3(n_t), dim3(256), sizeof(float) * K16_TS * (size_t)(d | 1), st, X, N, d, mean, scale_info, KB, c16, cn, cr, 0, k16_dA(d, KB));
+  if (!spheres_ready) {
+    MELD_HIP_CALL(hipMemsetAsync(temp, 0, n_c * ((size_t)KB * 64 + 2 * sizeof(float)), st));
+    hipLaunchKernelGGL(tile_spheres_kernel, dim3(n_t), dim3(256), sizeof(float) * K16_TS * (size_t)(d | 1), st, X, N, d, mean, scale_info, KB, c16, cn, cr, 0, k16_dA(d, KB));
+  }
   const float es = (float)meld_knn16_error_coef(nprod, d);
   hipLaunchKernelGGL(knn16_wave_thresholds_kernel, dim3((unsigned)ceil_div(n_q, 4)), dim3(256), 0, st, thr_seed, N, n_q, es, norm2_max,
                      scale_info, wthr);
@@ -2184,6 +2328,14 @@
                                                  int lead_only, meld_stream_t stream) {
   return k16_step_lists_direct_impl(X, N, d, mean, scale_info, norm2_max, Rt16, thr_seed, q_norm2, nprod, temp, scratch, list, list_stride, cnt,
                                     lead_only, stream);
+}
+
+extern "C" int meld_knn16_step_lists_direct_spheres(const double* X, int64_t N, int d, const double* mean, const float* scale_info,
+                                                    const float* norm2_max, const void* Rt16, const float* thr_seed, const float* q_norm2,
+                                                    int nprod, void* temp, void* scratch, uint32_t* list, int64_t list_stride, int32_t* cnt,
+                                                    int lead_only, meld_stream_t stream) {
+  return k16_step_lists_direct_impl(X, N, d, mean, scale_info, norm2_max, Rt16, thr_seed, q_norm2, nprod, temp, scratch, list, list_stride, cnt,
+                                    lead_only, stream, true);
 }
 
 extern "C" int meld_knn16_seed_thresholds_mfma(const void* Q16, const float* Qn, const void* Rt16, const float* scale_info,
diff --git a/meld_amd/graph.py b/meld_amd/graph.py
--- a/meld_amd/graph.py
+++ b/meld_amd/graph.py
@@ -456,7 +456,8 @@
         return out
 
     def directed_kernel_coo(self, X, q_begin, q_count, knn, decay, thresh, ksel, tm=None, force_fallback=False, n_refs=None, assemble=False, comm=None,
-                            bw_scale=1.0, bw_fixed=None, col_stats=None, knn_max=None, symm=(0, 0.0), count_rows_ge=None, frame_axes=None):
+                            bw_scale=1.0, bw_fixed=None, col_stats=None, knn_max=None, symm=(0, 0.0), count_rows_ge=None, frame_axes=None,
+                            anisotropy=None):
         N = int(X.shape[0])
         NR = int(n_refs) if n_refs is not None else N
         if n_refs is not None and not (0 < NR <= q_begin and q_begin + q_count <= N):
@@ -470,7 +471,7 @@
             retry_from, ksel = (ksel, r.n_flag), 128
             r = self._search_and_refine(a, ksel, None)
         s = self._exact_sweep(a, r, count_rows_ge)
-        keys, vals, assembled = self._emit(a, r, s, ksel, assemble, symm)
+        keys, vals, assembled = self._emit(a, r, s, ksel, assemble, symm, anisotropy)
         p, c = r.plan, r.cands
         info = dict(ksel=int(ksel), KP=int(c.KP), search=p.search, nprod=p.nprod, n_flagged_rows=r.n_flag,
                     prune=p.prune, radius_cut=p.radius_cut, seed=p.seed != "none", seeded_bounds=p.seeded_bounds, block_order=p.block_order != "none",
@@ -611,6 +612,10 @@
             check(lib.meld_knn16_prepare_cross(ptr(X), a.NR, N, d, ptr(mean), *tail), "meld_knn16_prepare_cross")
             norm2[a.q_begin : a.q_begin + a.q_count] = o.Qn[: a.q_count]
             nmax = torch.maximum(nmax, o.Qn[: a.q_count].max().reshape(1))
+        elif plan.fused_operands:
+            o.spheres = torch.empty(lib.meld_knn16_bounds_temp_bytes(N, d, a.q_count), dtype=torch.uint8, device=dev)
+            check(lib.meld_knn16_prepare_fused(ptr(o.X_s), N, d, ptr(o.mean_s), ptr(col_min), ptr(col_max), ptr(o.Rt), ptr(o.Q), ptr(o.Qn), ptr(norm2),
+                                               ptr(nmax), ptr(o.scale_info), ptr(o.spheres), st), "meld_knn16_prepare_fused")
         elif col_min is not None:
             check(lib.meld_knn16_prepare_scaled(ptr(o.X_s), N, d, ptr(o.mean_s), ptr(col_min), ptr(col_max), *tail), "meld_knn16_prepare_scaled")
         else:
@@ -642,7 +647,8 @@
             return None, None, None, None
         lib, st, dev, N, d = self.lib, _stream(), a.X.device, a.N, a.d
         X_s, mean_s, n_tiles, n_blocks = o.X_s, o.mean_s, o.n_tiles, o.q_pad // o.BQ
-        tmpb = torch.empty(lib.meld_knn16_bounds_temp_bytes(N, d, a.q_count), dtype=torch.uint8, device=dev)
+        spheres_ready = getattr(o, "spheres", None) is not None
+        tmpb = o.spheres if spheres_ready else torch.empty(lib.meld_knn16_bounds_temp_bytes(N, d, a.q_count), dtype=torch.uint8, device=dev)
         if plan.bounds == "bounds_from_spheres":
             rows_c, row_b = sphere_layout(lib, N, d)
             per = rows_c // comm.world
@@ -659,14 +665,14 @@
             step_list = torch.empty(n_blocks * n_tiles, dtype=torch.int32, device=dev)
             step_cnt = torch.empty(n_blocks, dtype=torch.int32, device=dev)
             scratch = torch.empty(lib.meld_knn16_list_scratch_bytes(N), dtype=torch.uint8, device=dev)
-            check(lib.meld_knn16_step_lists_direct_lead(ptr(X_s), N, d, ptr(mean_s), ptr(o.scale_info), ptr(nmax), ptr(o.Rt), ptr(seeds), ptr(o.Qn), plan.nprod,
-                                                        ptr(tmpb), ptr(scratch), ptr(step_list), n_tiles, ptr(step_cnt), int(plan.lead_bounds), st),
+            check((lib.meld_knn16_step_lists_direct_spheres if spheres_ready else lib.meld_knn16_step_lists_direct_lead)(ptr(X_s), N, d, ptr(mean_s), ptr(o.scale_info), ptr(nmax), ptr(o.Rt), ptr(seeds), ptr(o.Qn), plan.nprod,
+                ptr(tmpb), ptr(scratch), ptr(step_list), n_tiles, ptr(step_cnt), int(plan.lead_bounds), st),
                   "meld_knn16_step_lists_direct")
             del scratch
         else:
             sb = plan.seeded_bounds
             lb2 = torch.empty(lib.meld_knn16_bounds_bytes(N, a.q_count), dtype=torch.uint8, device=dev)
-            check((lib.meld_knn16_bounds_from_spheres if plan.bounds == "bounds_from_spheres" else lib.meld_knn16_bounds)(
+            check((lib.meld_knn16_bounds_from_spheres if plan.bounds == "bounds_from_spheres" or spheres_ready else lib.meld_knn16_bounds)(
                 ptr(X_s), N, d, ptr(mean_s), ptr(o.scale_info), ptr(nmax), ptr(o.Rt), a.q_begin, a.q_count, ptr(seeds) if sb else None,
                 ptr(o.Qn) if sb else None, plan.nprod, ptr(tmpb), ptr(lb2), st), "meld_knn16_bounds")
             if plan.lists == "table":
@@ -856,7 +862,7 @@
             s.rows_at_least = int(((tot + 1) >= int(count_rows_ge)).sum())
         return s
 
-    def _emit(self, a, r, s, ksel, assemble, symm):
+    def _emit(self, a, r, s, ksel, assemble, symm, anisotropy=None):
         lib, st, dev, q_count, n_flag_h, c = self.lib, _stream(), a.X.device, a.q_count, r.n_flag, r.cands
         M = r.m_main + s.fb_total
         assembled = None
@@ -873,9 +879,12 @@
                                                 ptr(s.fb_off), ptr(s.fb_col), ptr(s.fb_val), s.fb_total, ptr(cursor), ptr(tcol), ptr(tval), st),
                       "meld_coo_emit_scatter")
                 a.tm.stop("coo_emit")
-                assembled = self._finish_buckets(cursor, tcol, tval, q_count, sums_diag=1.0, symm=symm)
+                aniso = anisotropy if opt("MELD_ASSEMBLE_FUSED_ANISO", "1") != "0" else None
+                assembled = self._finish_buckets(cursor, tcol, tval, q_count, sums_diag=1.0, symm=symm, anisotropy=aniso)
                 if assembled is not None and self.last_row_sums is not None:
                     assembled = assembled + (self.last_row_sums[1],)
+                    if self.last_degrees is not None:
+                        assembled = assembled + (self.last_degrees,)
                 a.tm.stop("symmetrize")
                 del cursor, tcol, tval
         keys = vals = None
@@ -914,20 +923,31 @@
                                                  int(cap), ptr(counts), ptr(send), _stream()), "meld_coo_partition_remote")
         return send, counts
 
-    def _finish_buckets(self, cursor, tcol, tval, n_rows, sums_diag=None, symm=(0, 0.0)):
+    def _finish_buckets(self, cursor, tcol, tval, n_rows, sums_diag=None, symm=(0, 0.0), anisotropy=None):
         lib, st, dev = self.lib, _stream(), cursor.device
         i32 = dict(dtype=torch.int32, device=dev)
         ucnt = torch.empty(n_rows, **i32)
         flags = torch.empty(1, **i32)
-        check(lib.meld_csr_rows_sort_merge(ptr(cursor), n_rows, ptr(tcol), ptr(tval), ptr(ucnt), ptr(flags), int(symm[0]), float(symm[1]), st), "meld_csr_rows_sort_merge")
+        fused = anisotropy is not None and sums_diag is not None
+        if fused:
+            sums = torch.empty(n_rows, dtype=torch.float64, device=dev)
+            check(lib.meld_csr_rows_sort_merge_sums(ptr(cursor), n_rows, ptr(tcol), ptr(tval), ptr(ucnt), ptr(flags), int(symm[0]), float(symm[1]),
+                                                    float(sums_diag), ptr(sums), st), "meld_csr_rows_sort_merge_sums")
+        else:
+            check(lib.meld_csr_rows_sort_merge(ptr(cursor), n_rows, ptr(tcol), ptr(tval), ptr(ucnt), ptr(flags), int(symm[0]), float(symm[1]), st), "meld_csr_rows_sort_merge")
         rowptr = _scan_i32(lib, ucnt, st)
         nnz, flag = (int(v) for v in torch.stack([rowptr[n_rows], flags[0].to(torch.int64)]).tolist())
         if flag != 0:
             return None
         col = torch.empty(nnz, **i32)
         val = torch.empty(nnz, dtype=torch.float64, device=dev)
-        self.last_row_sums = None
-        if nnz > 0 and sums_diag is not None:
+        self.last_row_sums = self.last_degrees = None
+        if nnz > 0 and fused:
+            dw = torch.empty(n_rows, dtype=torch.float64, device=dev)
+            check(lib.meld_csr_compact_rows_anisotropy(ptr(rowptr), n_rows, ptr(tcol), ptr(tval), ptr(col), ptr(val), ptr(sums), float(anisotropy), ptr(dw), st),
+                  "meld_csr_compact_rows_anisotropy")
+            self.last_row_sums, self.last_degrees = (sums_diag, sums), dw
+        elif nnz > 0 and sums_diag is not None:
             sums = torch.empty(n_rows, dtype=torch.float64, device=dev)
             check(lib.meld_csr_compact_rows_sums(ptr(rowptr), n_rows, ptr(tcol), ptr(tval), ptr(col), ptr(val), float(sums_diag), ptr(sums), st),
                   "meld_csr_compact_rows_sums")
@@ -1366,7 +1386,7 @@
     if knn_max is not None and decay is not None and math.isfinite(decay) and 36 * k1 < min(knn_max + 1, N):
         trial = ops.directed_kernel_coo(X, 0, N, knn, decay, thresh, ksel, tm=tm, force_fallback=force_fallback, assemble=True,
                                         bw_scale=bw_scale, bw_fixed=bw_fixed, col_stats=col_stats, knn_max=None, symm=symm, count_rows_ge=6 * k1,
-                                        frame_axes=frame_axes)
+                                        frame_axes=frame_axes, anisotropy=anisotropy)
         if trial[3]["rows_with_at_least"] <= N // 10 or 36 * k1 >= N / 2:
             keys, vals, bw, info = trial
             info["knn_max_uncapped_as_upstream"] = True
@@ -1375,24 +1395,26 @@
     if info is None:
         keys, vals, bw, info = ops.directed_kernel_coo(X, 0, N, knn, decay, thresh, ksel, tm=tm, force_fallback=force_fallback, assemble=True,
                                                        bw_scale=bw_scale, bw_fixed=bw_fixed, col_stats=col_stats, knn_max=knn_max, symm=symm,
-                                                       frame_axes=frame_axes)
+                                                       frame_axes=frame_axes, anisotropy=anisotropy)
     if bw_scale != 1.0:
         bw = (bw * bw_scale).clamp_(min=float(np.finfo(float).eps))
     if info.get("nnz_directed", 0) == 0:
         raise ValueError("the kernel has no off-diagonal entries; cannot build a graph")
     tm.start()
-    ksum = None
+    ksum = dw = None
     if info.get("assembled") is not None:
         asm = info.pop("assembled")
         rowptr, col, val = asm[:3]
         ksum = asm[3] if len(asm) > 3 else None
+        dw = asm[4] if len(asm) > 4 else None
     else:
         rowptr, col, val = ops.assemble_rows(keys, vals, 0, N, N, symm=symm)
     del keys, vals
     tm.stop("symmetrize")
     if ksum is None:
         ksum = ops.row_sums(rowptr, val, N, 1.0)
-    dw = ops.anisotropy_degrees(rowptr, col, val, N, ksum, 0, anisotropy)
+    if dw is None:
+        dw = ops.anisotropy_degrees(rowptr, col, val, N, ksum, 0, anisotropy)
     tm.stop("anisotropy_degree")
 
     nnz = int(col.shape[0])
diff --git a/meld_amd/knn_plan.py b/meld_amd/knn_plan.py
--- a/meld_amd/knn_plan.py
+++ b/meld_amd/knn_plan.py
@@ -51,6 +51,7 @@
     stage2: bool
     lead_bounds: Optional[bool] = None
     partial_forced: bool = False
+    fused_operands: bool = dataclasses.field(default=False, compare=False)
 
     def __post_init__(self):
         if self.lead_bounds is None:
@@ -110,5 +111,6 @@
     two = opt("MELD_KNN_TWO_PHASE", "1")
     two_pass = lists != "none" and frame and (main_slices == 1 or two == "2") and two != "0" and ee is None
     lead_bounds = lists == "direct" and frame and opt("MELD_KNN16_LEAD_BOUNDS", "1") != "0"
+    fused = prune and bounds != "bounds_from_spheres" and q_begin == 0 and q_count == N and opt("MELD_KNN_FUSED_OPERANDS", "1") != "0"
     return KnnPlan(search, nprod, frame, radius_cut, prune, seed, 0 if seed == "bandwidth" else knn, bounds, seeded_bounds, lists,
-                   block_order, main_slices, two_pass, partial, nprod == 1, lead_bounds, ee is not None)
+                   block_order, main_slices, two_pass, partial, nprod == 1, lead_bounds, ee is not None, fused)
```

Measured after the change: 28.49 million (median of 6 runs). 1.02x the previous value.
